# hhcho/sfgwas

Hardware: AMD Instinct MI355X
Metric: pca_power_iter_ring_macs_per_s (higher is better)
Workload: dtype u64 ring words, exact integers: int8 digits on the matrix core for the MAC of all five moduli, fp64-held integers in the encode and key-switch kernels

## Files before the change

include/sfgwas_hip.h:

```cpp
#ifndef SFGWAS_HIP_H
#define SFGWAS_HIP_H
#include <stdint.h>
#include <stddef.h>
#ifdef __cplusplus
extern "C" {
#endif

typedef struct sfg_ctx sfg_ctx;
typedef struct sfg_geno sfg_geno;

int sfg_ctx_create(sfg_ctx **out, int device, int logN, int nq, int np,
                   const uint64_t *moduli, const uint64_t *psi, double scale);
typedef struct sfg_config {
    uint32_t struct_size;
    int mm_group;
    size_t acc_budget_bytes;
    size_t assoc_rotcache_bytes;
    size_t ksw_budget_bytes;
    int enc_batch;
    int upload_blocking;
    const char *mgpu_transport;
    size_t mgpu_cache_bytes;
    const char *rccl_lib;
} sfg_config;
void sfg_config_default(sfg_config *c);
int sfg_ctx_create_ex(sfg_ctx **out, int device, int logN, int nq, int np,
                      const uint64_t *moduli, const uint64_t *psi, double scale, const sfg_config *config );
int sfg_ctx_fork(sfg_ctx *parent, sfg_ctx **out);
void sfg_ctx_destroy(sfg_ctx *ctx);
const char *sfg_last_error(const sfg_ctx *ctx);
int sfg_ctx_synchronize(sfg_ctx *ctx);
int sfg_ctx_release_scratch(sfg_ctx *ctx);
int sfg_ctx_scratch_bytes(const sfg_ctx *ctx, const char *prefix, size_t *bytes);
int sfg_ctx_set_stream(sfg_ctx *ctx, void *hip_stream);
int sfg_ctx_use_own_stream(sfg_ctx *ctx);

int sfg_ctx_load_rotkey(sfg_ctx *ctx, uint64_t galois_el, const uint64_t *key_host, int montgomery_form);
int sfg_ctx_has_rotkey(const sfg_ctx *ctx, uint64_t galois_el);
int sfg_ctx_export_rotkey(sfg_ctx *ctx, uint64_t galois_el, uint64_t *key_host);
uint64_t sfg_galois_for_rotation(const sfg_ctx *ctx, int k_left);

int sfg_malloc(sfg_ctx *ctx, void **dev_ptr, size_t bytes);
int sfg_free(sfg_ctx *ctx, void *dev_ptr);
int sfg_memcpy_h2d(sfg_ctx *ctx, void *dst_dev, const void *src_host, size_t bytes);
int sfg_memcpy_d2h(sfg_ctx *ctx, void *dst_host, const void *src_dev, size_t bytes);
int sfg_memcpy_d2d(sfg_ctx *ctx, void *dst_dev, const void *src_dev, size_t bytes);

int sfg_ntt_rows(sfg_ctx *ctx, uint64_t *rows_dev, int nrows, const int *mod_idx_host);
int sfg_intt_rows(sfg_ctx *ctx, uint64_t *rows_dev, int nrows, const int *mod_idx_host);

int sfg_mac_dev(sfg_ctx *ctx, const uint64_t *rot_dev, const uint64_t *pt_dev, uint64_t *out_dev,
                int K, int R, int Ncols, int L, int accumulate);

int sfg_mac_i8_dev(sfg_ctx *ctx, const uint64_t *rot_dev, const uint64_t *pt_half_dev, uint64_t *out_dev,
                   int K, int R, int Ncols, int L, int accumulate, int pt_form);

int sfg_encode_diags_dev(sfg_ctx *ctx, const int8_t *block_dev, size_t ld, int r, int c, int transposed,
                         int shift0, int nshift, int L, uint64_t *pt_dev);
int sfg_encode_coeffs_host(sfg_ctx *ctx, const double *values_host, int nvec, int64_t *coeffs_host);
int sfg_ctx_encoder_near_ties(sfg_ctx *ctx, unsigned long long *count, int reset);
int sfg_ctx_encoder_resolved(sfg_ctx *ctx, unsigned long long *count);
int sfg_ctx_encoder_unprovable(sfg_ctx *ctx, unsigned long long *count);
int sfg_ctx_encoder_inject_unsafe_for_test(sfg_ctx *ctx, unsigned long long n);
int sfg_encode_vectors_dev(sfg_ctx *ctx, const double *values_host, int nvec, int level, uint64_t *pt_dev);

int sfg_rotate_right_dev(sfg_ctx *ctx, const uint64_t *ct_in_dev, uint64_t *ct_out_dev, int nct, int level,
                         const int *nrot_host);
int sfg_ct_galois_dev(sfg_ctx *ctx, const uint64_t *ct_in_dev, uint64_t *ct_out_dev, int nct, int level, uint64_t galois_el);
int sfg_ct_add_dev(sfg_ctx *ctx, const uint64_t *a_dev, const uint64_t *b_dev, uint64_t *out_dev, int nct, int level);
int sfg_ct_sub_dev(sfg_ctx *ctx, const uint64_t *a_dev, const uint64_t *b_dev, uint64_t *out_dev, int nct, int level);

int sfg_ct_drop_level_dev(sfg_ctx *ctx, const uint64_t *in_dev, uint64_t *out_dev, int nct, int level_in, int level_out);

int sfg_ct_mul_scalar_dev(sfg_ctx *ctx, const uint64_t *ct_dev, const uint64_t *scalars_host, uint64_t *out_dev, int nct, int level);
int sfg_ct_mul_scalar_add_dev(sfg_ctx *ctx, const uint64_t *ct_dev, const uint64_t *scalars_host, uint64_t *acc_dev, int nct, int level);
int sfg_ct_add_scalar_dev(sfg_ctx *ctx, const uint64_t *ct_dev, const uint64_t *scalars_host, uint64_t *out_dev, int nct, int level);
int sfg_ct_add_plain_dev(sfg_ctx *ctx, const uint64_t *ct_dev, const uint64_t *pt_dev, size_t pt_stride, uint64_t *out_dev,
                         int nct, int level);

int sfg_ctx_load_relinkey(sfg_ctx *ctx, const uint64_t *key_host, int montgomery);
int sfg_ct_mulrelin_dev(sfg_ctx *ctx, const uint64_t *a_dev, const uint64_t *b_dev, uint64_t *out_dev, int nct, int level);
int sfg_ct_mul_plain_dev(sfg_ctx *ctx, const uint64_t *ct_dev, const uint64_t *pt_dev, size_t pt_stride, uint64_t *out_dev,
                         int nct, int level);
int sfg_ct_rescale_dev(sfg_ctx *ctx, const uint64_t *in_dev, uint64_t *out_dev, int nct, int level);
int sfg_ct_innersum_dev(sfg_ctx *ctx, const uint64_t *in_dev, int nct, int level, uint64_t *out_dev);

int sfg_geno_upload(sfg_ctx *ctx, const int8_t *geno_host, size_t nrow, size_t ncol, size_t ld, sfg_geno **out);
int sfg_geno_from_device(sfg_ctx *ctx, const int8_t *geno_dev, size_t nrow, size_t ncol, size_t ld, sfg_geno **out);
void sfg_geno_free(sfg_ctx *ctx, sfg_geno *g);
int sfg_geno_create(sfg_ctx *ctx, size_t nrow, size_t ncol, sfg_geno **out);
int sfg_geno_write_rows(sfg_ctx *ctx, sfg_geno *g, size_t row0, size_t nrows, const int8_t *rows_host, size_t ld);
int sfg_geno_compare_rows(sfg_ctx *ctx, const sfg_geno *g, unsigned flags, size_t row0, size_t nrows, const int8_t *rows_host, size_t ld, uint64_t *ndiff);
int sfg_pinned_alloc(sfg_ctx *ctx, void **host_ptr, size_t bytes);
int sfg_pinned_free(sfg_ctx *ctx, void *host_ptr);
int sfg_geno_set_plaintext_cache(sfg_ctx *ctx, const sfg_geno *g, size_t max_bytes);
int sfg_geno_plaintext_cache_stats(sfg_ctx *ctx, const sfg_geno *g, size_t *blocks, size_t *bytes, size_t *hits, size_t *fills);
int sfg_geno_from_bed(sfg_ctx *ctx, const uint8_t *bed_host, size_t bed_bytes, size_t num_sample, size_t num_snp,
                      const uint8_t *row_filter, const uint8_t *col_filter, sfg_geno **out);
int sfg_pgen_dims(sfg_ctx *ctx, const uint8_t *pgen_host, size_t pgen_bytes, size_t *num_sample, size_t *num_variant);
int sfg_geno_from_pgen(sfg_ctx *ctx, const uint8_t *pgen_host, size_t pgen_bytes, size_t v0, size_t v1,
                       const uint8_t *row_filter, const uint8_t *col_filter, sfg_geno **out);
int sfg_pgen_geno_counts(sfg_ctx *ctx, const uint8_t *pgen_host, size_t pgen_bytes, const uint8_t *row_filter, uint32_t *counts_host);
int sfg_geno_pack(sfg_ctx *ctx, const sfg_geno *g, sfg_geno **out);
int sfg_geno_unpack(sfg_ctx *ctx, const sfg_geno *g, sfg_geno **out);
int sfg_geno_dims(const sfg_geno *g, size_t *nrow, size_t *ncol);
int sfg_geno_download(sfg_ctx *ctx, const sfg_geno *g, int8_t *host);
int sfg_geno_transpose(sfg_ctx *ctx, const sfg_geno *g, sfg_geno **out);
int sfg_geno_concat_cols(sfg_ctx *ctx, const sfg_geno *const *parts, int k, sfg_geno **out);
int sfg_geno_colsums(sfg_ctx *ctx, const sfg_geno *g, double *sum_host, double *sqsum_host);

#define SFG_SQUARE 1u
#define SFG_TRANSPOSE 2u
#define SFG_STREAM_DIRECT 4u
int sfg_matmul_resident_dev(sfg_ctx *ctx, const uint64_t *A_dev, int s, int in_level, int max_level,
                            const sfg_geno *g, unsigned flags, uint64_t *out_dev);
int sfg_matmul_from_cache(sfg_ctx *ctx, const uint64_t *A_dev, int s, int in_level, int max_level, const char *cache_prefix, int nbr, uint64_t *out_dev);
int sfg_diagcache_write(sfg_ctx *ctx, const sfg_geno *g, unsigned flags, int max_level, const char *cache_prefix, int *files_written);
int sfg_diagcache_header(sfg_ctx *ctx, const char *cache_prefix, int block_row, uint64_t hdr[6]);
int sfg_matmul_stream(sfg_ctx *ctx, const uint64_t *A_host, int s, int in_level, int max_level,
                      const int8_t *geno_host, size_t nrow, size_t ncol, size_t ld, unsigned flags,
                      uint64_t *out_host, double *sum_host, double *sqsum_host);
int sfg_assoc_stream_bed(sfg_ctx *ctx, const char *bed_path, size_t num_sample, size_t num_snp, const uint8_t *row_filter, const uint8_t *col_filter,
                         size_t batch_snps, const uint64_t *A_dev, int s, int in_level, int max_level, unsigned flags,
                         uint64_t *out_dev, size_t out_ct_capacity, size_t *out_ct, double *sum_host, double *sqsum_host);
int sfg_assoc_pgen(sfg_ctx *ctx, const uint8_t *pgen_host, size_t pgen_bytes, const uint8_t *row_filter, const uint8_t *col_filter, size_t batch_snps,
                   const uint64_t *A_dev, int s, int in_level, int max_level, unsigned flags,
                   uint64_t *out_dev, size_t out_ct_capacity, size_t *out_ct, double *sum_host, double *sqsum_host);
int sfg_assoc_stream_pgen(sfg_ctx *ctx, const char *pgen_path, const uint8_t *row_filter, const uint8_t *col_filter, size_t batch_snps,
                          const uint64_t *A_dev, int s, int in_level, int max_level, unsigned flags,
                          uint64_t *out_dev, size_t out_ct_capacity, size_t *out_ct, double *sum_host, double *sqsum_host);
int sfg_matmul_resident_range_dev(sfg_ctx *ctx, const uint64_t *A_dev, int s, int in_level, int max_level,
                                  const sfg_geno *g, unsigned flags, int blk0, int blk1, uint64_t *out_dev);
int sfg_matmul_accumulate_dev(sfg_ctx *ctx, const uint64_t *A_dev, int s, int in_level, int max_level,
                              const sfg_geno *g, unsigned flags, int b0, int b1, int j0, int j1,
                              int accumulate, uint64_t *acc_dev);
int sfg_matmul_finalize_dev(sfg_ctx *ctx, const uint64_t *acc_dev, int s, int max_level, int ncolb,
                            int g0, int g1, int accumulate, uint64_t *out_dev);
int sfg_matmul_finalize_slots_dev(sfg_ctx *ctx, const uint64_t *acc_dev, int s, int max_level, int ncolb, int acc_giants, int giant_base,
                                  int g0, int g1, int accumulate, uint64_t *out_dev);
int sfg_rotcache_invalidate(sfg_ctx *ctx);
int sfg_rotcache_layout(sfg_ctx *ctx, int s, int max_level, size_t *job_doubles, size_t *tail_doubles);
int sfg_rotcache_build_jobs_dev(sfg_ctx *ctx, const uint64_t *A_dev, int s, int in_level, int max_level, int nbr, int job0, int job1, double *staged_dev);
int sfg_rotcache_scatter_dev(sfg_ctx *ctx, const double *staged_dev, int s, int max_level, int job0, int job1, int row0, int nrows, double *cache_dev);
int sfg_rotcache_build_rows_dev(sfg_ctx *ctx, const uint64_t *A_dev, int s, int in_level, int max_level, int nbr, int b0, int b1, double *cache_dev);
int sfg_matmul_resident_range_rc_dev(sfg_ctx *ctx, const double *cache_dev, int s, int max_level, const sfg_geno *g, unsigned flags,
                                     int blk0, int blk1, uint64_t *out_dev);
int sfg_matmul_accumulate_rc_dev(sfg_ctx *ctx, const double *cache_dev, int s, int max_level, const sfg_geno *g, unsigned flags,
                                 int b0, int b1, int j0, int j1, int accumulate, uint64_t *acc_dev);
int sfg_reduce_rows_dev(sfg_ctx *ctx, uint64_t *rows_dev, size_t nrows_of_L, int L);

typedef struct sfg_mgpu sfg_mgpu;
typedef struct sfg_mgeno sfg_mgeno;
#define SFG_MGPU_ID_BYTES 128
int sfg_mgpu_unique_id(uint8_t *id128);
int sfg_mgpu_create(sfg_mgpu **out, const int *devices, int n, int logN, int nq, int np, const uint64_t *moduli, const uint64_t *psi, double scale);
int sfg_mgpu_create_rank(sfg_mgpu **out, int device, int rank, int world, const uint8_t *id128, int logN, int nq, int np, const uint64_t *moduli,
                         const uint64_t *psi, double scale);
int sfg_mgpu_create_ex(sfg_mgpu **out, const int *devices, int n, int logN, int nq, int np, const uint64_t *moduli, const uint64_t *psi, double scale,
                       const sfg_config *config);
int sfg_mgpu_create_rank_ex(sfg_mgpu **out, int device, int rank, int world, const uint8_t *id128, int logN, int nq, int np, const uint64_t *moduli,
                            const uint64_t *psi, double scale, const sfg_config *config);
void sfg_mgpu_destroy(sfg_mgpu *mg);
const char *sfg_mgpu_last_error(const sfg_mgpu *mg);
int sfg_mgpu_world(const sfg_mgpu *mg);
int sfg_mgpu_nlocal(const sfg_mgpu *mg);
int sfg_mgpu_rank(const sfg_mgpu *mg, int local);
sfg_ctx *sfg_mgpu_ctx(sfg_mgpu *mg, int local);
const char *sfg_mgpu_transport(const sfg_mgpu *mg);
int sfg_mgpu_synchronize(sfg_mgpu *mg);
int sfg_mgpu_comm_info(sfg_mgpu *mg, int local, int *nranks, int *rank);
int sfg_mgpu_preflight(sfg_mgpu *mg, size_t count_per_rank);
int sfg_mgpu_load_rotkey(sfg_mgpu *mg, uint64_t galois_el, const uint64_t *key_host, int montgomery_form);
int sfg_mgpu_load_relinkey(sfg_mgpu *mg, const uint64_t *key_host, int montgomery_form);
int sfg_mgpu_fill_rotkeys_synthetic(sfg_mgpu *mg, const int *rot_left, int nrot, uint64_t seed);
int sfg_mgpu_shard(int world, size_t ncol, int rank, size_t *blk0, size_t *blk1, size_t *col0, size_t *col1);
int sfg_mgpu_geno_upload(sfg_mgpu *mg, const int8_t *geno_host, size_t nrow, size_t ncol, size_t ld, sfg_mgeno **out);
int sfg_mgpu_geno_adopt(sfg_mgpu *mg, size_t nrow, size_t ncol, sfg_geno *const *shards, sfg_mgeno **out);
int sfg_mgpu_geno_synthetic(sfg_mgpu *mg, size_t nrow, size_t ncol, uint64_t seed, int packed, sfg_mgeno **out);
void sfg_mgpu_geno_free(sfg_mgpu *mg, sfg_mgeno *g);
const sfg_geno *sfg_mgpu_geno_shard(const sfg_mgeno *g, int local);
int sfg_mgpu_geno_dims(const sfg_mgeno *g, size_t *nrow, size_t *ncol);
int sfg_mgpu_geno_blocks(const sfg_mgeno *g, int local, size_t *blk0, size_t *blk1);
int sfg_mgpu_geno_set_plaintext_cache(sfg_mgpu *mg, const sfg_mgeno *g, size_t max_bytes_per_rank);
int sfg_mgpu_geno_create(sfg_mgpu *mg, size_t nrow, size_t ncol, sfg_mgeno **out);
int sfg_mgpu_geno_write_rows(sfg_mgpu *mg, sfg_mgeno *g, size_t row0, size_t nrows, const int8_t *rows_host, size_t ld);
int sfg_mgpu_geno_compare_rows(sfg_mgpu *mg, const sfg_mgeno *g, unsigned flags, size_t row0, size_t nrows, const int8_t *rows_host, size_t ld, uint64_t *ndiff);
int sfg_mgpu_matmul_dev(sfg_mgpu *mg, const uint64_t *const *A_dev, int s, int in_level, int max_level, const sfg_mgeno *g, unsigned flags,
                        uint64_t *const *out_dev);
int sfg_mgpu_matmul(sfg_mgpu *mg, const uint64_t *A_host, int s, int in_level, int max_level, const sfg_mgeno *g, unsigned flags, uint64_t *out_host);
int sfg_mgpu_inject_failure_for_test(sfg_mgpu *mg, int local, int phase);
int sfg_mgpu_assoc_stream_bed(sfg_mgpu *mg, const char *bed_path, size_t num_sample, size_t num_snp, const uint8_t *row_filter, const uint8_t *col_filter,
                              size_t batch_snps, const uint64_t *A_host, int s, int in_level, int max_level, unsigned flags,
                              uint64_t *out_host, size_t out_ct_capacity, size_t *out_ct, double *sum_host, double *sqsum_host);
int sfg_mgpu_assoc_stream_pgen(sfg_mgpu *mg, const char *pgen_path, const uint8_t *row_filter, const uint8_t *col_filter, size_t kept_samples,
                               size_t batch_snps, const uint64_t *A_host, int s, int in_level, int max_level, unsigned flags,
                               uint64_t *out_host, size_t out_ct_capacity, size_t *out_ct, double *sum_host, double *sqsum_host);

int sfg_ctx_load_secret_key(sfg_ctx *ctx, const uint64_t *sk_host, int montgomery_form);
int sfg_refresh_gen_shares_dev(sfg_ctx *ctx, const uint64_t *ct_dev, int nct, int level, const uint64_t *crs_dev, const uint64_t *mask_dev, int mask_limbs,
                               const int32_t *e0_dev, const int32_t *e1_dev, uint64_t *h0_dev, uint64_t *h1_dev);
int sfg_refresh_finish_dev(sfg_ctx *ctx, const uint64_t *ct_dev, int nct, int level, const uint64_t *h0agg_dev, const uint64_t *h1agg_dev,
                           const uint64_t *crs_dev, uint64_t *out_dev);

int sfg_refresh_gen_shares_scaled_dev(sfg_ctx *ctx, const uint64_t *ct_dev, int nct, int level, double ct_scale, double target_scale, const uint64_t *crs_dev,
                                      const uint64_t *mask_dev, int mask_limbs, const int32_t *e0_dev, const int32_t *e1_dev, uint64_t *h0_dev, uint64_t *h1_dev);
int sfg_refresh_finish_scaled_dev(sfg_ctx *ctx, const uint64_t *ct_dev, int nct, int level, double ct_scale, double target_scale, const uint64_t *h0agg_dev,
                                  const uint64_t *h1agg_dev, const uint64_t *crs_dev, uint64_t *out_dev);

int sfg_ckks_to_ss_share_dev(sfg_ctx *ctx, const uint64_t *ct_dev, int nct, int level, const uint64_t *mask_dev, int mask_limbs, const int32_t *e0_dev,
                             uint64_t *h0_dev, uint64_t *mask_ntt_dev);

int sfg_ss_mask_dev(sfg_ctx *ctx, int limbs, const uint64_t *modulus_host, const uint64_t *bound_host, const uint64_t *rm_dev, const uint64_t *rand_dev,
                    uint64_t *rm_masked_dev, uint64_t *mask_dev, size_t n);
int sfg_ss_hub_share_dev(sfg_ctx *ctx, int limbs, const uint64_t *modulus_host, const uint64_t *revealed_dev, const uint64_t *mask_dev, uint64_t *share_dev, size_t n);

int sfg_ctx_load_public_key(sfg_ctx *ctx, const uint64_t *pk_host, int montgomery_form);
int sfg_ctx_has_public_key(const sfg_ctx *ctx);
int sfg_encrypt_explicit_dev(sfg_ctx *ctx, const uint64_t *pt_dev, int nct, int level, const int8_t *u_dev, const int32_t *e0_dev, const int32_t *e1_dev,
                             uint64_t *out_dev);
int sfg_ctx_seed_encryptor(sfg_ctx *ctx, const uint8_t *key32);
int sfg_ctx_encryptor_next_index(const sfg_ctx *ctx, uint64_t *next_index);
int sfg_ct_add_fresh_zero_dev(sfg_ctx *ctx, uint64_t *ct_dev, int nct, int level);
int sfg_encrypt_vectors_dev(sfg_ctx *ctx, const double *values_host, int nct, int level, uint64_t *out_dev);
int sfg_encrypt_transcript_for_test(sfg_ctx *ctx, uint64_t first_index, int nct, int8_t *u_dev, int32_t *e0_dev, int32_t *e1_dev);

int sfg_pcks_gen_share_dev(sfg_ctx *ctx, const uint64_t *ct_dev, int nct, int level, const int32_t *e0_dev, const int32_t *e1_dev, uint64_t *h0_dev, uint64_t *h1_dev);
int sfg_pcks_finish_dev(sfg_ctx *ctx, const uint64_t *ct_dev, int nct, int level, const uint64_t *h0agg_dev, uint64_t *pt_dev);
int sfg_decode_vectors(sfg_ctx *ctx, const uint64_t *pt_dev, size_t pt_stride, int nct, int level, double scale, double *re_host, double *im_host);
int sfg_decode_vectors_dev(sfg_ctx *ctx, const uint64_t *pt_dev, size_t pt_stride, int nct, int level, double scale, double *re_dev, double *im_dev);
int sfg_decode_coeffs(sfg_ctx *ctx, const uint64_t *pt_dev, size_t pt_stride, int nct, int level, double scale, double *coeffs_host);
int sfg_pcks_finish_decode(sfg_ctx *ctx, const uint64_t *ct_dev, int nct, int level, double scale, const uint64_t *h0agg_dev, double *re_host, double *im_host);
int sfg_decrypt_vectors(sfg_ctx *ctx, const uint64_t *ct_dev, int nct, int level, double scale, double *re_host, double *im_host);

int sfg_beaver_elem_dev(sfg_ctx *ctx, int pid, int limbs, const uint64_t *modulus_host,
                        const uint64_t *ar_dev, const uint64_t *am_dev, const uint64_t *br_dev, const uint64_t *bm_dev,
                        uint64_t *out_dev, size_t n);
int sfg_beaver_elem(sfg_ctx *ctx, int pid, int limbs, const uint64_t *modulus_host,
                    const uint64_t *ar_host, const uint64_t *am_host, const uint64_t *br_host, const uint64_t *bm_host,
                    uint64_t *out_host, size_t n);
int sfg_beaver_matmul(sfg_ctx *ctx, int pid, int limbs, const uint64_t *modulus_host,
                      const uint64_t *ar_host, const uint64_t *am_host, const uint64_t *br_host, const uint64_t *bm_host,
                      uint64_t *out_host, int m, int k, int n);

int sfg_sketch(sfg_ctx *ctx, const sfg_geno *g, const int32_t *bucket_host, const int8_t *sgn_host, int kp,
               double *sketch_host, uint64_t *xsum_host, uint64_t *x2sum_host);

int sfg_fill_uniform_ct_dev(sfg_ctx *ctx, uint64_t *ct_dev, int nct, int level, uint64_t seed);
int sfg_fill_geno_dev(sfg_ctx *ctx, int8_t *geno_dev, size_t nrow, size_t ncol, uint64_t seed);
int sfg_fill_geno_window_dev(sfg_ctx *ctx, int8_t *geno_dev, size_t nrow, size_t ncol, size_t ld, size_t col0, size_t ncol_global, uint64_t seed);
int sfg_fill_rotkeys_synthetic(sfg_ctx *ctx, const int *rot_left, int nrot, uint64_t seed);

int sfg_ctx_clear_phases(sfg_ctx *ctx);
double sfg_last_phase_ms(const sfg_ctx *ctx, const char *phase);
int sfg_last_phase_launches(const sfg_ctx *ctx, const char *phase);
double sfg_last_phase_bytes(const sfg_ctx *ctx, const char *phase);

#ifdef __cplusplus
}
#endif
#endif
```

sfgwas_amd/capi.py:

```python
import ctypes as C
import os
import numpy as np

_HERE = os.path.dirname(os.path.abspath(__file__))
LIB_PATH = os.environ.get("SFG_LIB_PATH") or os.path.join(_HERE, "lib", "libsfgwas_hip.so")
AB_LIB_PATH = os.path.join(_HERE, "lib_ab", "libsfgwas_hip.so")
DEPLOYMENT_SWITCHES = {"SFG_MM_GROUP", "SFG_MM_ACC_BUDGET_MB", "SFG_ASSOC_ROTCACHE_MB", "SFG_KSW_BUDGET_MB", "SFG_ENC_BATCH", "SFG_UPLOAD_BLOCKING",
                       "SFG_MGPU_TRANSPORT", "SFG_MGPU_CACHE_GB", "SFG_RCCL_LIB", "SFG_ENABLE_TEST_HOOKS",
                       "SFG_TEST_SCRATCH_OOM", "SFG_TEST_TIE_BAND_LOG2", "SFG_MGPU_FORCE_COLLECTIVES"}


def ab_lib():
    import subprocess
    subprocess.check_call(["make", "-C", os.path.join(_HERE, "csrc"), "ab", "-j8"], stdout=subprocess.DEVNULL)
    return AB_LIB_PATH


def env_for(switches):
    e = {k: str(v) for k, v in switches.items()}
    if any(k.startswith("SFG_") and k not in DEPLOYMENT_SWITCHES for k in e):
        e["SFG_LIB_PATH"] = ab_lib()
    return e


class SfgConfig(C.Structure):
    _fields_ = [("struct_size", C.c_uint32), ("mm_group", C.c_int), ("acc_budget_bytes", C.c_size_t), ("assoc_rotcache_bytes", C.c_size_t),
                ("ksw_budget_bytes", C.c_size_t), ("enc_batch", C.c_int), ("upload_blocking", C.c_int), ("mgpu_transport", C.c_char_p),
                ("mgpu_cache_bytes", C.c_size_t), ("rccl_lib", C.c_char_p)]

    def __init__(self, **kw):
        super().__init__()
        self.struct_size = C.sizeof(SfgConfig)
        for k, v in kw.items():
            setattr(self, k, v)

u64p = C.POINTER(C.c_uint64)
_lib = None

SFG_SQUARE = 1
SFG_TRANSPOSE = 2
SFG_STREAM_DIRECT = 4


class SfgError(RuntimeError):
    pass


def _sig(L):
    vp, i, u64, d, sz = C.c_void_p, C.c_int, C.c_uint64, C.c_double, C.c_size_t
    S = {
        "sfg_ctx_create": (i, [C.POINTER(vp), i, i, i, i, u64p, u64p, d]),
        "sfg_ctx_create_ex": (i, [C.POINTER(vp), i, i, i, i, u64p, u64p, d, vp]),
        "sfg_config_default": (None, [vp]),
        "sfg_mgpu_create_ex": (i, [C.POINTER(vp), C.POINTER(i), i, i, i, i, u64p, u64p, d, vp]),
        "sfg_mgpu_create_rank_ex": (i, [C.POINTER(vp), i, i, i, vp, i, i, i, u64p, u64p, d, vp]),
        "sfg_ctx_fork": (i, [vp, C.POINTER(vp)]),
        "sfg_ctx_destroy": (None, [vp]),
        "sfg_last_error": (C.c_char_p, [vp]),
        "sfg_ctx_synchronize": (i, [vp]),
        "sfg_ctx_set_stream": (i, [vp, vp]),
        "sfg_ctx_release_scratch": (i, [vp]),
        "sfg_ctx_scratch_bytes": (i, [vp, C.c_char_p, C.POINTER(C.c_size_t)]),
        "sfg_rotcache_invalidate": (i, [vp]),
        "sfg_ctx_use_own_stream": (i, [vp]),
        "sfg_ctx_encoder_inject_unsafe_for_test": (i, [vp, C.c_ulonglong]),
        "sfg_ctx_encoder_resolved": (i, [vp, C.POINTER(C.c_ulonglong)]),
        "sfg_ctx_encoder_unprovable": (i, [vp, C.POINTER(C.c_ulonglong)]),
        "sfg_ctx_load_rotkey": (i, [vp, u64, u64p, i]),
        "sfg_ctx_load_secret_key": (i, [vp, u64p, i]),
        "sfg_ctx_load_public_key": (i, [vp, u64p, i]),
        "sfg_ctx_has_public_key": (i, [vp]),
        "sfg_ctx_seed_encryptor": (i, [vp, C.c_char_p]),
        "sfg_ctx_encryptor_next_index": (i, [vp, C.POINTER(u64)]),
        "sfg_encrypt_explicit_dev": (i, [vp, vp, i, i, vp, vp, vp, vp]),
        "sfg_ct_add_fresh_zero_dev": (i, [vp, vp, i, i]),
        "sfg_encrypt_vectors_dev": (i, [vp, C.POINTER(d), i, i, vp]),
        "sfg_encrypt_transcript_for_test": (i, [vp, u64, i, vp, vp, vp]),
        "sfg_pcks_gen_share_dev": (i, [vp, vp, i, i, vp, vp, vp, vp]),
        "sfg_pcks_finish_dev": (i, [vp, vp, i, i, vp, vp]),
        "sfg_decode_vectors": (i, [vp, vp, sz, i, i, d, vp, vp]),
        "sfg_decode_vectors_dev": (i, [vp, vp, sz, i, i, d, vp, vp]),
        "sfg_decode_coeffs": (i, [vp, vp, sz, i, i, d, vp]),
        "sfg_pcks_finish_decode": (i, [vp, vp, i, i, d, vp, vp, vp]),
        "sfg_decrypt_vectors": (i, [vp, vp, i, i, d, vp, vp]),
        "sfg_ct_galois_dev": (i, [vp, vp, vp, i, i, u64]),
        "sfg_ct_mul_scalar_add_dev": (i, [vp, vp, u64p, vp, i, i]),
        "sfg_refresh_gen_shares_dev": (i, [vp, vp, i, i, vp, vp, i, vp, vp, vp, vp]),
        "sfg_refresh_finish_dev": (i, [vp, vp, i, i, vp, vp, vp, vp]),
        "sfg_refresh_gen_shares_scaled_dev": (i, [vp, vp, i, i, d, d, vp, vp, i, vp, vp, vp, vp]),
        "sfg_refresh_finish_scaled_dev": (i, [vp, vp, i, i, d, d, vp, vp, vp, vp]),
        "sfg_ckks_to_ss_share_dev": (i, [vp, vp, i, i, vp, i, vp, vp, vp]),
        "sfg_geno_pack": (i, [vp, vp, C.POINTER(vp)]),
        "sfg_geno_unpack": (i, [vp, vp, C.POINTER(vp)]),
        "sfg_assoc_stream_bed": (i, [vp, C.c_char_p, sz, sz, vp, vp, sz, vp, i, i, i, C.c_uint, vp, sz, C.POINTER(sz), vp, vp]),
        "sfg_assoc_stream_pgen": (i, [vp, C.c_char_p, vp, vp, sz, vp, i, i, i, C.c_uint, vp, sz, C.POINTER(sz), vp, vp]),
        "sfg_assoc_pgen": (i, [vp, vp, sz, vp, vp, sz, vp, i, i, i, C.c_uint, vp, sz, C.POINTER(sz), vp, vp]),
        "sfg_ctx_has_rotkey": (i, [vp, u64]),
        "sfg_ctx_export_rotkey": (i, [vp, u64, u64p]),
        "sfg_galois_for_rotation": (u64, [vp, i]),
        "sfg_malloc": (i, [vp, C.POINTER(vp), sz]),
        "sfg_free": (i, [vp, vp]),
        "sfg_memcpy_h2d": (i, [vp, vp, vp, sz]),
        "sfg_memcpy_d2h": (i, [vp, vp, vp, sz]),
        "sfg_memcpy_d2d": (i, [vp, vp, vp, sz]),
        "sfg_ct_drop_level_dev": (i, [vp, vp, vp, i, i, i]),
        "sfg_ntt_rows": (i, [vp, vp, i, C.POINTER(i)]),
        "sfg_intt_rows": (i, [vp, vp, i, C.POINTER(i)]),
        "sfg_mac_dev": (i, [vp, vp, vp, vp, i, i, i, i, i]),
        "sfg_mac_i8_dev": (i, [vp, vp, vp, vp, i, i, i, i, i, i]),
        "sfg_encode_diags_dev": (i, [vp, vp, sz, i, i, i, i, i, i, vp]),
        "sfg_encode_coeffs_host": (i, [vp, C.POINTER(d), i, C.POINTER(C.c_int64)]),
        "sfg_encode_vectors_dev": (i, [vp, C.POINTER(d), i, i, vp]),
        "sfg_ctx_encoder_near_ties": (i, [vp, C.POINTER(C.c_ulonglong), i]),
        "sfg_rotate_right_dev": (i, [vp, vp, vp, i, i, C.POINTER(i)]),
        "sfg_ct_add_dev": (i, [vp, vp, vp, vp, i, i]),
        "sfg_ct_sub_dev": (i, [vp, vp, vp, vp, i, i]),
        "sfg_ct_mul_scalar_dev": (i, [vp, vp, u64p, vp, i, i]),
        "sfg_ct_add_scalar_dev": (i, [vp, vp, u64p, vp, i, i]),
        "sfg_ct_add_plain_dev": (i, [vp, vp, vp, sz, vp, i, i]),
        "sfg_ctx_load_relinkey": (i, [vp, u64p, i]),
        "sfg_ct_mulrelin_dev": (i, [vp, vp, vp, vp, i, i]),
        "sfg_ct_mul_plain_dev": (i, [vp, vp, vp, sz, vp, i, i]),
        "sfg_ct_rescale_dev": (i, [vp, vp, vp, i, i]),
        "sfg_ct_innersum_dev": (i, [vp, vp, i, i, vp]),
        "sfg_geno_upload": (i, [vp, vp, sz, sz, sz, C.POINTER(vp)]),
        "sfg_geno_from_device": (i, [vp, vp, sz, sz, sz, C.POINTER(vp)]),
        "sfg_geno_free": (None, [vp, vp]),
        "sfg_geno_create": (i, [vp, sz, sz, C.POINTER(vp)]),
        "sfg_geno_write_rows": (i, [vp, vp, sz, sz, vp, sz]),
        "sfg_geno_compare_rows": (i, [vp, vp, C.c_uint, sz, sz, vp, sz, u64p]),
        "sfg_pinned_alloc": (i, [vp, C.POINTER(vp), sz]),
        "sfg_pinned_free": (i, [vp, vp]),
        "sfg_geno_set_plaintext_cache": (i, [vp, vp, C.c_size_t]),
        "sfg_geno_plaintext_cache_stats": (i, [vp, vp, C.POINTER(C.c_size_t), C.POINTER(C.c_size_t), C.POINTER(C.c_size_t), C.POINTER(C.c_size_t)]),
        "sfg_geno_from_bed": (i, [vp, vp, sz, sz, sz, vp, vp, C.POINTER(vp)]),
        "sfg_geno_dims": (i, [vp, C.POINTER(sz), C.POINTER(sz)]),
        "sfg_pgen_dims": (i, [vp, vp, sz, C.POINTER(sz), C.POINTER(sz)]),
        "sfg_geno_from_pgen": (i, [vp, vp, sz, sz, sz, vp, vp, C.POINTER(vp)]),
        "sfg_pgen_geno_counts": (i, [vp, vp, sz, vp, vp]),
        "sfg_geno_download": (i, [vp, vp, vp]),
        "sfg_geno_transpose": (i, [vp, vp, C.POINTER(vp)]),
        "sfg_geno_concat_cols": (i, [vp, C.POINTER(vp), i, C.POINTER(vp)]),
        "sfg_geno_colsums": (i, [vp, vp, C.POINTER(d), C.POINTER(d)]),
        "sfg_matmul_resident_dev": (i, [vp, vp, i, i, i, vp, C.c_uint, vp]),
        "sfg_matmul_from_cache": (i, [vp, vp, i, i, i, C.c_char_p, i, vp]),
        "sfg_diagcache_header": (i, [vp, C.c_char_p, i, u64p]),
        "sfg_diagcache_write": (i, [vp, vp, C.c_uint, i, C.c_char_p, C.POINTER(C.c_int)]),
        "sfg_matmul_stream": (i, [vp, u64p, i, i, i, vp, sz, sz, sz, C.c_uint, u64p, C.POINTER(d), C.POINTER(d)]),
        "sfg_matmul_resident_range_dev": (i, [vp, vp, i, i, i, vp, C.c_uint, i, i, vp]),
        "sfg_matmul_accumulate_dev": (i, [vp, vp, i, i, i, vp, C.c_uint, i, i, i, i, i, vp]),
        "sfg_matmul_finalize_dev": (i, [vp, vp, i, i, i, i, i, i, vp]),
        "sfg_matmul_finalize_slots_dev": (i, [vp, vp, i, i, i, i, i, i, i, i, vp]),
        "sfg_reduce_rows_dev": (i, [vp, vp, sz, i]),
        "sfg_rotcache_layout": (i, [vp, i, i, C.POINTER(sz), C.POINTER(sz)]),
        "sfg_rotcache_build_jobs_dev": (i, [vp, vp, i, i, i, i, i, i, vp]),
        "sfg_rotcache_scatter_dev": (i, [vp, vp, i, i, i, i, i, i, vp]),
        "sfg_rotcache_build_rows_dev": (i, [vp, vp, i, i, i, i, i, i, vp]),
        "sfg_matmul_resident_range_rc_dev": (i, [vp, vp, i, i, vp, C.c_uint, i, i, vp]),
        "sfg_matmul_accumulate_rc_dev": (i, [vp, vp, i, i, vp, C.c_uint, i, i, i, i, i, vp]),
        "sfg_beaver_elem_dev": (i, [vp, i, i, u64p, vp, vp, vp, vp, vp, sz]),
        "sfg_ss_mask_dev": (i, [vp, i, u64p, u64p, vp, vp, vp, vp, sz]),
        "sfg_ss_hub_share_dev": (i, [vp, i, u64p, vp, vp, vp, sz]),
        "sfg_beaver_elem": (i, [vp, i, i, u64p, u64p, u64p, u64p, u64p, u64p, sz]),
        "sfg_beaver_matmul": (i, [vp, i, i, u64p, u64p, u64p, u64p, u64p, u64p, i, i, i]),
        "sfg_sketch": (i, [vp, vp, C.POINTER(C.c_int32), C.POINTER(C.c_int8), i, C.POINTER(d), u64p, u64p]),
        "sfg_fill_uniform_ct_dev": (i, [vp, vp, i, i, u64]),
        "sfg_fill_geno_dev": (i, [vp, vp, sz, sz, u64]),
        "sfg_fill_geno_window_dev": (i, [vp, vp, sz, sz, sz, sz, sz, u64]),
        "sfg_fill_rotkeys_synthetic": (i, [vp, C.POINTER(i), i, u64]),
        "sfg_mgpu_unique_id": (i, [vp]),
        "sfg_mgpu_create": (i, [C.POINTER(vp), C.POINTER(i), i, i, i, i, u64p, u64p, d]),
        "sfg_mgpu_create_rank": (i, [C.POINTER(vp), i, i, i, vp, i, i, i, u64p, u64p, d]),
        "sfg_mgpu_destroy": (None, [vp]),
        "sfg_mgpu_last_error": (C.c_char_p, [vp]),
        "sfg_mgpu_world": (i, [vp]),
        "sfg_mgpu_nlocal": (i, [vp]),
        "sfg_mgpu_rank": (i, [vp, i]),
        "sfg_mgpu_ctx": (vp, [vp, i]),
        "sfg_mgpu_transport": (C.c_char_p, [vp]),
        "sfg_mgpu_synchronize": (i, [vp]),
        "sfg_mgpu_load_rotkey": (i, [vp, u64, u64p, i]),
        "sfg_mgpu_load_relinkey": (i, [vp, u64p, i]),
        "sfg_mgpu_fill_rotkeys_synthetic": (i, [vp, C.POINTER(i), i, u64]),
        "sfg_mgpu_shard": (i, [i, sz, i, C.POINTER(sz), C.POINTER(sz), C.POINTER(sz), C.POINTER(sz)]),
        "sfg_mgpu_geno_upload": (i, [vp, vp, sz, sz, sz, C.POINTER(vp)]),
        "sfg_mgpu_geno_adopt": (i, [vp, sz, sz, C.POINTER(vp), C.POINTER(vp)]),
        "sfg_mgpu_geno_create": (i, [vp, sz, sz, C.POINTER(vp)]),
        "sfg_mgpu_geno_write_rows": (i, [vp, vp, sz, sz, vp, sz]),
        "sfg_mgpu_geno_compare_rows": (i, [vp, vp, C.c_uint, sz, sz, vp, sz, u64p]),
        "sfg_mgpu_comm_info": (i, [vp, i, C.POINTER(i), C.POINTER(i)]),
        "sfg_mgpu_preflight": (i, [vp, sz]),
        "sfg_mgpu_geno_synthetic": (i, [vp, sz, sz, u64, i, C.POINTER(vp)]),
        "sfg_mgpu_geno_free": (None, [vp, vp]),
        "sfg_mgpu_geno_shard": (vp, [vp, i]),
        "sfg_mgpu_geno_dims": (i, [vp, C.POINTER(sz), C.POINTER(sz)]),
        "sfg_mgpu_geno_blocks": (i, [vp, i, C.POINTER(sz), C.POINTER(sz)]),
        "sfg_mgpu_geno_set_plaintext_cache": (i, [vp, vp, sz]),
        "sfg_mgpu_matmul_dev": (i, [vp, C.POINTER(vp), i, i, i, vp, C.c_uint, C.POINTER(vp)]),
        "sfg_mgpu_matmul": (i, [vp, u64p, i, i, i, vp, C.c_uint, u64p]),
        "sfg_mgpu_inject_failure_for_test": (i, [vp, i, i]),
        "sfg_mgpu_assoc_stream_bed": (i, [vp, C.c_char_p, sz, sz, vp, vp, sz, u64p, i, i, i, C.c_uint, u64p, sz, C.POINTER(sz), vp, vp]),
        "sfg_mgpu_assoc_stream_pgen": (i, [vp, C.c_char_p, vp, vp, sz, sz, u64p, i, i, i, C.c_uint, u64p, sz, C.POINTER(sz), vp, vp]),
        "sfg_ctx_clear_phases": (i, [vp]),
        "sfg_last_phase_ms": (d, [vp, C.c_char_p]),
        "sfg_last_phase_launches": (i, [vp, C.c_char_p]),
        "sfg_last_phase_bytes": (d, [vp, C.c_char_p]),
    }
    for name, (res, args) in S.items():
        fn = getattr(L, name)
        fn.restype, fn.argtypes = res, args
    return list(S.keys())


EXPORTS = []


def lib():
    global _lib, EXPORTS
    if _lib is None:
        if not os.path.exists(LIB_PATH):
            raise SfgError(f"{LIB_PATH} is missing: run `python -c 'import __graft_entry__ as g; g.build()'` "
                           "(there is no CPU fallback for the HIP path)")
        _lib = C.CDLL(LIB_PATH)
        EXPORTS = _sig(_lib)
    return _lib


def p64(a):
    assert a.dtype == np.uint64 and a.flags.c_contiguous
    return a.ctypes.data_as(u64p)


class Context:

    def __init__(self, q, p, scale=2.0 ** 34, logN=14, device=0, psi=None, config=None):
        L = lib()
        self.q, self.p = list(q), list(p)
        self.nq, self.np_ = len(q), len(p)
        self.N, self.slots = 1 << logN, (1 << logN) // 2
        mods = np.array(self.q + self.p, dtype=np.uint64)
        h = C.c_void_p()
        ps = None if psi is None else p64(np.array(psi, dtype=np.uint64))
        if config is None:
            rc = L.sfg_ctx_create(C.byref(h), device, logN, self.nq, self.np_, p64(mods), ps, float(scale))
        else:
            rc = L.sfg_ctx_create_ex(C.byref(h), device, logN, self.nq, self.np_, p64(mods), ps, float(scale), C.byref(config))
        if rc:
            raise SfgError("sfg_ctx_create: " + L.sfg_last_error(None).decode())
        self.h = h
        self.beta = (self.nq + self.np_ - 1) // self.np_

    def close(self):
        if getattr(self, "h", None):
            lib().sfg_ctx_destroy(self.h)
            self.h = None

    def __del__(self):
        try:
            self.close()
        except Exception:
            pass

    def check(self, rc, what):
        if rc:
            raise SfgError(f"{what}: {lib().sfg_last_error(self.h).decode()}")

    def malloc(self, nbytes):
        p = C.c_void_p()
        self.check(lib().sfg_malloc(self.h, C.byref(p), nbytes), "sfg_malloc")
        return p

    def free(self, p):
        self.check(lib().sfg_free(self.h, p), "sfg_free")

    def to_device(self, arr):
        arr = np.ascontiguousarray(arr)
        p = self.malloc(arr.nbytes)
        self.check(lib().sfg_memcpy_h2d(self.h, p, arr.ctypes.data_as(C.c_void_p), arr.nbytes), "h2d")
        return p

    def to_host(self, p, shape, dtype):
        out = np.empty(shape, dtype=dtype)
        self.check(lib().sfg_memcpy_d2h(self.h, out.ctypes.data_as(C.c_void_p), p, out.nbytes), "d2h")
        return out

    def sync(self):
        self.check(lib().sfg_ctx_synchronize(self.h), "sync")

    def ntt_rows(self, rows, mod_idx, inverse=False):
        rows = np.ascontiguousarray(rows, dtype=np.uint64)
        n = rows.shape[0]
        mi = (C.c_int * n)(*[int(x) for x in mod_idx])
        d = self.to_device(rows)
        fn = lib().sfg_intt_rows if inverse else lib().sfg_ntt_rows
        self.check(fn(self.h, d, n, mi), "ntt_rows")
        out = self.to_host(d, rows.shape, np.uint64)
        self.free(d)
        return out

    def load_rotkey(self, galois, key, montgomery=False):
        key = np.ascontiguousarray(key, dtype=np.uint64)
        self.check(lib().sfg_ctx_load_rotkey(self.h, int(galois), p64(key), int(montgomery)), "load_rotkey")

    def export_rotkey(self, galois):
        key = np.zeros((self.beta, 2, self.nq + self.np_, self.N), dtype=np.uint64)
        self.check(lib().sfg_ctx_export_rotkey(self.h, int(galois), p64(key)), "export_rotkey")
        return key

    def load_secret_key(self, sk_rows, montgomery=False):
        sk_rows = np.ascontiguousarray(sk_rows, dtype=np.uint64)
        assert sk_rows.shape == (self.nq, self.N)
        self.check(lib().sfg_ctx_load_secret_key(self.h, p64(sk_rows), int(montgomery)), "load_secret_key")

    def refresh_gen_shares(self, cts, level, crs, mask_limbs, e0, e1, scales=None):
        nct, W = cts.shape[0], mask_limbs.shape[-1]
        d = [self.to_device(np.ascontiguousarray(a)) for a in (cts, crs, mask_limbs, e0.astype(np.int32), e1.astype(np.int32))]
        h0, h1 = self.malloc(nct * (level + 1) * self.N * 8), self.malloc(nct * self.nq * self.N * 8)
        if scales is None:
            self.check(lib().sfg_refresh_gen_shares_dev(self.h, d[0], nct, level, d[1], d[2], W, d[3], d[4], h0, h1), "refresh_gen_shares")
        else:
            self.check(lib().sfg_refresh_gen_shares_scaled_dev(self.h, d[0], nct, level, float(scales[0]), float(scales[1]), d[1], d[2], W, d[3], d[4], h0, h1),
                       "refresh_gen_shares_scaled")
        out = self.to_host(h0, (nct, level + 1, self.N), np.uint64), self.to_host(h1, (nct, self.nq, self.N), np.uint64)
        for p_ in d + [h0, h1]:
            self.free(p_)
        return out

    def ckks_to_ss_share(self, cts, level, mask_limbs, e0):
        nct, W = cts.shape[0], mask_limbs.shape[-1]
        d = [self.to_device(np.ascontiguousarray(a)) for a in (cts, mask_limbs, e0.astype(np.int32))]
        h0, mk = self.malloc(nct * (level + 1) * self.N * 8), self.malloc(nct * (level + 1) * self.N * 8)
        self.check(lib().sfg_ckks_to_ss_share_dev(self.h, d[0], nct, level, d[1], W, d[2], h0, mk), "ckks_to_ss_share")
        out = self.to_host(h0, (nct, level + 1, self.N), np.uint64), self.to_host(mk, (nct, level + 1, self.N), np.uint64)
        for p_ in d + [h0, mk]:
            self.free(p_)
        return out

    def refresh_finish(self, cts, level, h0agg, h1agg, crs, scales=None):
        nct = cts.shape[0]
        d = [self.to_device(np.ascontiguousarray(a)) for a in (cts, h0agg, h1agg, crs)]
        o = self.malloc(nct * 2 * self.nq * self.N * 8)
        if scales is None:
            self.check(lib().sfg_refresh_finish_dev(self.h, d[0], nct, level, d[1], d[2], d[3], o), "refresh_finish")
        else:
            self.check(lib().sfg_refresh_finish_scaled_dev(self.h, d[0], nct, level, float(scales[0]), float(scales[1]), d[1], d[2], d[3], o), "refresh_finish_scaled")
        out = self.to_host(o, (nct, 2, self.nq, self.N), np.uint64)
        for p_ in d + [o]:
            self.free(p_)
        return out

    def fork(self):
        h = C.c_void_p()
        self.check(lib().sfg_ctx_fork(self.h, C.byref(h)), "sfg_ctx_fork")
        child = Context.__new__(Context)
        child.__dict__.update({k: v for k, v in self.__dict__.items()})
        child.h = h
        return child

    def encoder_near_ties(self, reset=False):
        n = C.c_ulonglong()
        self.check(lib().sfg_ctx_encoder_near_ties(self.h, C.byref(n), int(reset)), "encoder_near_ties")
        return n.value

    def galois(self, k):
        return lib().sfg_galois_for_rotation(self.h, k)

    def phase_ms(self, name):
        return lib().sfg_last_phase_ms(self.h, name.encode())


def _ctx_mac(self, rot, pt, L, out_init=None):
    rot = np.ascontiguousarray(rot, dtype=np.uint64)
    pt = np.ascontiguousarray(pt, dtype=np.uint64)
    K, R = rot.shape[0], rot.shape[1]
    Ncols = pt.shape[1]
    assert rot.shape[2] == L and pt.shape[2] == L and pt.shape[0] == K
    d_rot, d_pt = self.to_device(rot), self.to_device(pt)
    if out_init is not None:
        d_out = self.to_device(np.ascontiguousarray(out_init, dtype=np.uint64))
    else:
        d_out = self.malloc(Ncols * R * L * self.N * 8)
    self.check(lib().sfg_mac_dev(self.h, d_rot, d_pt, d_out, K, R, Ncols, L, int(out_init is not None)), "sfg_mac_dev")
    out = self.to_host(d_out, (Ncols, R, L, self.N), np.uint64)
    for p in (d_rot, d_pt, d_out):
        self.free(p)
    return out


Context.mac = _ctx_mac


def _ctx_mac_i8(self, rot, pt_half, L, K=None, out_init=None, pt_form=0):
    rot = np.ascontiguousarray(rot, dtype=np.uint64)
    pt_half = np.ascontiguousarray(pt_half, dtype=np.uint64)
    P, R = rot.shape[0], rot.shape[1]
    Ncols = pt_half.shape[1]
    K = P if K is None else K
    assert rot.shape[2] == L and pt_half.shape[2] == L and pt_half.shape[0] == P and pt_half.shape[3] == self.N // 2 and K >= P
    bufs = []
    for arr in (rot, pt_half):
        sl = arr.nbytes // P
        d = self.malloc(sl * K)
        self.check(lib().sfg_memcpy_h2d(self.h, d, arr.ctypes.data_as(C.c_void_p), arr.nbytes), "h2d")
        filled = P
        while filled < K:
            n = min(filled, K - filled)
            self.check(lib().sfg_memcpy_d2d(self.h, C.c_void_p(d.value + filled * sl), d, n * sl), "d2d")
            filled += n
        bufs.append(d)
    if out_init is not None:
        d_out = self.to_device(np.ascontiguousarray(out_init, dtype=np.uint64))
    else:
        d_out = self.malloc(Ncols * R * L * self.N * 8)
    try:
        self.check(lib().sfg_mac_i8_dev(self.h, bufs[0], bufs[1], d_out, K, R, Ncols, L, int(out_init is not None), pt_form), "sfg_mac_i8_dev")
        out = self.to_host(d_out, (Ncols, R, L, self.N), np.uint64)
    finally:
        for p_ in bufs + [d_out]:
            self.free(p_)
    return out


Context.mac_i8 = _ctx_mac_i8


def _ctx_encode_diags(self, block, shift0, nshift, L, transposed=False):
    block = np.ascontiguousarray(block, dtype=np.int8)
    r, c = block.shape
    if transposed:
        r, c = c, r
    d_blk = self.to_device(block)
    d_pt = self.malloc(nshift * L * self.N * 8)
    self.check(lib().sfg_encode_diags_dev(self.h, d_blk, block.shape[1], r, c, int(transposed), shift0, nshift, L, d_pt), "sfg_encode_diags_dev")
    out = self.to_host(d_pt, (nshift, L, self.N), np.uint64)
    self.free(d_blk)
    self.free(d_pt)
    return out


Context.encode_diags = _ctx_encode_diags


def _ctx_rotate_right(self, cts, level, nrots):
    cts = np.ascontiguousarray(cts, dtype=np.uint64)
    nct = cts.shape[0]
    d_in = self.to_device(cts)
    d_out = self.malloc(cts.nbytes)
    arr = (C.c_int * nct)(*[int(x) for x in nrots])
    self.check(lib().sfg_rotate_right_dev(self.h, d_in, d_out, nct, level, arr), "sfg_rotate_right_dev")
    out = self.to_host(d_out, cts.shape, np.uint64)
    self.free(d_in)
    self.free(d_out)
    return out


Context.rotate_right = _ctx_rotate_right


def _ctx_matmul_stream(self, A, in_level, max_level, geno, flags=0, want_sums=False):
    A = np.ascontiguousarray(A, dtype=np.uint64)
    geno = np.ascontiguousarray(geno, dtype=np.int8)
    s = A.shape[0]
    nrow, ncol = geno.shape
    lrow, lcol = (ncol, nrow) if flags & SFG_TRANSPOSE else (nrow, ncol)
    nbr, m_ct = (lrow - 1) // self.slots + 1, (lcol - 1) // self.slots + 1
    assert A.shape[1] == nbr, (A.shape, nbr)
    out = np.zeros((s, m_ct, 2, max_level, self.N), dtype=np.uint64)
    sm = np.zeros(ncol) if want_sums else None
    sq = np.zeros(ncol) if want_sums else None
    dp = C.POINTER(C.c_double)
    self.check(lib().sfg_matmul_stream(self.h, p64(A), s, in_level, max_level, geno.ctypes.data_as(C.c_void_p), nrow, ncol, ncol, flags,
                                       p64(out), sm.ctypes.data_as(dp) if want_sums else None, sq.ctypes.data_as(dp) if want_sums else None),
               "sfg_matmul_stream")
    return out, sm, sq


Context.matmul_stream = _ctx_matmul_stream


def random_rotkey(ctx_or_ring_moduli, beta, N, seed):
    rnd = np.random.default_rng(seed)
    mods = ctx_or_ring_moduli
    k = np.zeros((beta, 2, len(mods), N), dtype=np.uint64)
    for m, q in enumerate(mods):
        k[:, :, m, :] = rnd.integers(0, q, (beta, 2, N), dtype=np.uint64)
    return k


def _ctx_evalop(self, name, level, *arrays, out_level=None, extra=()):
    devs = [self.to_device(np.ascontiguousarray(a, dtype=np.uint64)) for a in arrays]
    nct = arrays[0].shape[0]
    ol_ = level if out_level is None else out_level
    out = self.malloc(nct * 2 * (ol_ + 1) * self.N * 8)
    fn = getattr(lib(), name)
    if name in ("sfg_ct_mul_plain_dev", "sfg_ct_add_plain_dev"):
        self.check(fn(self.h, devs[0], devs[1], extra[0], out, nct, level), name)
    elif name in ("sfg_ct_mul_scalar_dev", "sfg_ct_add_scalar_dev"):
        self.check(fn(self.h, devs[0], p64(np.ascontiguousarray(extra[0], dtype=np.uint64)), out, nct, level), name)
    elif name == "sfg_ct_rescale_dev":
        self.check(fn(self.h, devs[0], out, nct, level), name)
    else:
        self.check(fn(self.h, devs[0], devs[1], out, nct, level), name)
    res = self.to_host(out, (nct, 2, ol_ + 1, self.N), np.uint64)
    for d_ in devs + [out]:
        self.free(d_)
    return res


def _ctx_innersum(self, cts, level):
    cts = np.ascontiguousarray(cts, dtype=np.uint64)
    d_in = self.to_device(cts)
    out = self.malloc(2 * (level + 1) * self.N * 8)
    self.check(lib().sfg_ct_innersum_dev(self.h, d_in, cts.shape[0], level, out), "innersum")
    res = self.to_host(out, (2, level + 1, self.N), np.uint64)
    self.free(d_in); self.free(out)
    return res


def _ctx_load_relinkey(self, key, montgomery=False):
    key = np.ascontiguousarray(key, dtype=np.uint64)
    self.check(lib().sfg_ctx_load_relinkey(self.h, p64(key), int(montgomery)), "load_relinkey")


Context.evalop = _ctx_evalop
Context.innersum = _ctx_innersum
Context.load_relinkey = _ctx_load_relinkey


def _ctx_geno_to_host(self, g):
    nr, nc = C.c_size_t(), C.c_size_t()
    lib().sfg_geno_dims(g, C.byref(nr), C.byref(nc))
    out = np.empty((nr.value, nc.value), dtype=np.int8)
    self.check(lib().sfg_geno_download(self.h, g, out.ctypes.data_as(C.c_void_p)), "geno_download")
    return out


def _ctx_geno_from_bed(self, bed, num_sample, num_snp, row_filter=None, col_filter=None):
    bed = np.ascontiguousarray(bed, dtype=np.uint8)
    rf = None if row_filter is None else np.ascontiguousarray(row_filter, dtype=np.uint8)
    cf = None if col_filter is None else np.ascontiguousarray(col_filter, dtype=np.uint8)
    g = C.c_void_p()
    self.check(lib().sfg_geno_from_bed(self.h, bed.ctypes.data_as(C.c_void_p), bed.size, num_sample, num_snp,
                                       None if rf is None else rf.ctypes.data_as(C.c_void_p),
                                       None if cf is None else cf.ctypes.data_as(C.c_void_p), C.byref(g)), "geno_from_bed")
    return g


def _ctx_geno_from_pgen(self, img, v0=0, v1=0, row_filter=None, col_filter=None):
    img = np.ascontiguousarray(img, dtype=np.uint8)
    rf = None if row_filter is None else np.ascontiguousarray(row_filter, dtype=np.uint8)
    cf = None if col_filter is None else np.ascontiguousarray(col_filter, dtype=np.uint8)
    g = C.c_void_p()
    self.check(lib().sfg_geno_from_pgen(self.h, img.ctypes.data_as(C.c_void_p), img.size, v0, v1,
                                        None if rf is None else rf.ctypes.data_as(C.c_void_p),
                                        None if cf is None else cf.ctypes.data_as(C.c_void_p), C.byref(g)), "geno_from_pgen")
    return g


def _ctx_pgen_geno_counts(self, img, row_filter=None):
    img = np.ascontiguousarray(img, dtype=np.uint8)
    ns, nv = C.c_size_t(), C.c_size_t()
    self.check(lib().sfg_pgen_dims(self.h, img.ctypes.data_as(C.c_void_p), img.size, C.byref(ns), C.byref(nv)), "pgen_dims")
    rf = None if row_filter is None else np.ascontiguousarray(row_filter, dtype=np.uint8)
    out = np.empty((6, nv.value), dtype=np.uint32)
    self.check(lib().sfg_pgen_geno_counts(self.h, img.ctypes.data_as(C.c_void_p), img.size, None if rf is None else rf.ctypes.data_as(C.c_void_p),
                                          out.ctypes.data_as(C.c_void_p)), "pgen_geno_counts")
    return out


Context.geno_to_host = _ctx_geno_to_host
Context.geno_from_bed = _ctx_geno_from_bed
Context.geno_from_pgen = _ctx_geno_from_pgen
Context.pgen_geno_counts = _ctx_pgen_geno_counts


def _ctx_encode_vectors(self, values, level):
    values = np.ascontiguousarray(values, dtype=np.float64)
    nvec = values.shape[0]
    out = self.malloc(nvec * (level + 1) * self.N * 8)
    self.check(lib().sfg_encode_vectors_dev(self.h, values.ctypes.data_as(C.POINTER(C.c_double)), nvec, level, out), "encode_vectors")
    res = self.to_host(out, (nvec, level + 1, self.N), np.uint64)
    self.free(out)
    return res


Context.encode_vectors = _ctx_encode_vectors


def _ctx_load_public_key(self, pk_rows, montgomery=False):
    pk_rows = np.ascontiguousarray(pk_rows, dtype=np.uint64)
    assert pk_rows.shape == (2, self.nq + self.np_, self.N)
    self.check(lib().sfg_ctx_load_public_key(self.h, p64(pk_rows), int(montgomery)), "load_public_key")


def _ctx_has_public_key(self):
    return bool(lib().sfg_ctx_has_public_key(self.h))


def _ctx_seed_encryptor(self, key32):
    key32 = bytes(key32)
    if len(key32) != 32:
        raise ValueError("the encryptor key is 32 bytes")
    self.check(lib().sfg_ctx_seed_encryptor(self.h, key32), "seed_encryptor")


def _ctx_encryptor_next_index(self):
    n = C.c_uint64()
    self.check(lib().sfg_ctx_encryptor_next_index(self.h, C.byref(n)), "encryptor_next_index")
    return n.value


def _ctx_encrypt_explicit(self, pt, level, u, e0, e1):
    u, e0, e1 = (np.ascontiguousarray(u, dtype=np.int8), np.ascontiguousarray(e0, dtype=np.int32), np.ascontiguousarray(e1, dtype=np.int32))
    nct = u.shape[0]
    assert u.shape == e0.shape == e1.shape == (nct, self.N)
    d = [DevArray.from_host(self, a) for a in (u, e0, e1)]
    dpt = None
    if pt is not None:
        pt = np.ascontiguousarray(pt, dtype=np.uint64)
        assert pt.shape == (nct, level + 1, self.N)
        dpt = DevArray.from_host(self, pt)
    out = DevArray(self, (nct, 2, level + 1, self.N))
    try:
        self.check(lib().sfg_encrypt_explicit_dev(self.h, None if dpt is None else dpt.p, nct, level, d[0].p, d[1].p, d[2].p, out.p), "encrypt_explicit")
        return out.host()
    finally:
        for a in d + [out] + ([dpt] if dpt is not None else []):
            a.free()


def _ctx_add_fresh_zero(self, ct_dev, level):
    nct = int(np.prod(ct_dev.shape[:-3])) if len(ct_dev.shape) > 3 else 1
    assert ct_dev.shape[-3:] == (2, level + 1, self.N)
    self.check(lib().sfg_ct_add_fresh_zero_dev(self.h, ct_dev.p, nct, level), "add_fresh_zero")
    return ct_dev


def _ctx_encrypt_vectors(self, values, level):
    values = np.ascontiguousarray(values, dtype=np.float64)
    nct = values.shape[0]
    out = DevArray(self, (max(nct, 1), 2, level + 1, self.N))
    rc = lib().sfg_encrypt_vectors_dev(self.h, values.ctypes.data_as(C.POINTER(C.c_double)), nct, level, out.p)
    if rc:
        out.free()
    self.check(rc, "encrypt_vectors")
    return out


def _ctx_encrypt_transcript(self, first_index, nct):
    d = [DevArray(self, (max(nct, 1), self.N), t) for t in (np.int8, np.int32, np.int32)]
    try:
        self.check(lib().sfg_encrypt_transcript_for_test(self.h, int(first_index), nct, d[0].p, d[1].p, d[2].p), "encrypt_transcript")
        return tuple(a.host() for a in d)
    finally:
        for a in d:
            a.free()


Context.load_public_key = _ctx_load_public_key
Context.has_public_key = _ctx_has_public_key
Context.seed_encryptor = _ctx_seed_encryptor
Context.encryptor_next_index = _ctx_encryptor_next_index
Context.encrypt_explicit = _ctx_encrypt_explicit
Context.add_fresh_zero = _ctx_add_fresh_zero
Context.encrypt_vectors = _ctx_encrypt_vectors
Context.encrypt_transcript = _ctx_encrypt_transcript


def _dev_ptr(self, a, dtype, shape=None):
    if isinstance(a, DevArray):
        return a.p, None
    a = np.ascontiguousarray(a, dtype=dtype)
    assert shape is None or a.shape == shape, (a.shape, shape)
    d = DevArray.from_host(self, a)
    return d.p, d


def _ctx_pcks_gen_share(self, cts, level, e0, e1=None):
    nct = int(cts.shape[0])
    keep = []
    try:
        pc, t = _dev_ptr(self, cts, np.uint64, (nct, 2, level + 1, self.N)); keep.append(t)
        p0, t = _dev_ptr(self, e0, np.int32, (nct, self.N)); keep.append(t)
        p1 = None
        if e1 is not None:
            p1, t = _dev_ptr(self, e1, np.int32, (nct, self.N)); keep.append(t)
        h0 = DevArray(self, (nct, level + 1, self.N)); keep.append(h0)
        h1 = None
        if e1 is not None:
            h1 = DevArray(self, (nct, level + 1, self.N)); keep.append(h1)
        self.check(lib().sfg_pcks_gen_share_dev(self.h, pc, nct, level, p0, p1, h0.p, None if h1 is None else h1.p), "pcks_gen_share")
        return h0.host(), (None if h1 is None else h1.host())
    finally:
        for a in keep:
            if a is not None:
                a.free()


def _ctx_pcks_finish(self, cts, level, h0agg, scale=None, want_imag=False):
    nct = int(cts.shape[0])
    keep = []
    try:
        pc, t = _dev_ptr(self, cts, np.uint64, (nct, 2, level + 1, self.N)); keep.append(t)
        ph, t = _dev_ptr(self, h0agg, np.uint64, (nct, level + 1, self.N)); keep.append(t)
        if scale is None:
            pt = DevArray(self, (nct, level + 1, self.N)); keep.append(pt)
            self.check(lib().sfg_pcks_finish_dev(self.h, pc, nct, level, ph, pt.p), "pcks_finish")
            return pt.host()
        re = np.empty((nct, self.slots)); im = np.empty((nct, self.slots)) if want_imag else None
        self.check(lib().sfg_pcks_finish_decode(self.h, pc, nct, level, float(scale), ph, re.ctypes.data_as(C.c_void_p),
                                                None if im is None else im.ctypes.data_as(C.c_void_p)), "pcks_finish_decode")
        return (re, im) if want_imag else re
    finally:
        for a in keep:
            if a is not None:
                a.free()


def _ctx_decode_vectors(self, pt, level, scale, want_imag=False, stride=None):
    nct = int(pt.shape[0])
    p, t = _dev_ptr(self, pt, np.uint64)
    try:
        re = np.empty((nct, self.slots)); im = np.empty((nct, self.slots)) if want_imag else None
        self.check(lib().sfg_decode_vectors(self.h, p, (level + 1) * self.N if stride is None else int(stride), nct, level, float(scale),
                                            re.ctypes.data_as(C.c_void_p), None if im is None else im.ctypes.data_as(C.c_void_p)), "decode_vectors")
        return (re, im) if want_imag else re
    finally:
        if t is not None:
            t.free()


def _ctx_decode_coeffs(self, pt, level, scale, stride=None):
    nct = int(pt.shape[0])
    p, t = _dev_ptr(self, pt, np.uint64)
    try:
        out = np.empty((nct, self.N))
        self.check(lib().sfg_decode_coeffs(self.h, p, (level + 1) * self.N if stride is None else int(stride), nct, level, float(scale),
                                           out.ctypes.data_as(C.c_void_p)), "decode_coeffs")
        return out
    finally:
        if t is not None:
            t.free()


def _ctx_decrypt_vectors(self, cts, level, scale, want_imag=False):
    nct = int(np.prod(cts.shape[:-3]))
    p, t = _dev_ptr(self, cts, np.uint64)
    try:
        re = np.empty((nct, self.slots)); im = np.empty((nct, self.slots)) if want_imag else None
        self.check(lib().sfg_decrypt_vectors(self.h, p, nct, level, float(scale), re.ctypes.data_as(C.c_void_p),
                                             None if im is None else im.ctypes.data_as(C.c_void_p)), "decrypt_vectors")
        return (re, im) if want_imag else re
    finally:
        if t is not None:
            t.free()


Context.pcks_gen_share = _ctx_pcks_gen_share
Context.pcks_finish = _ctx_pcks_finish
Context.decode_vectors = _ctx_decode_vectors
Context.decode_coeffs = _ctx_decode_coeffs
Context.decrypt_vectors = _ctx_decrypt_vectors


class DevArray:

    def __init__(self, ctx, shape, dtype=np.uint64):
        self.ctx, self.shape, self.dtype = ctx, tuple(int(x) for x in shape), np.dtype(dtype)
        self.nbytes = int(np.prod(self.shape)) * self.dtype.itemsize
        self.p = ctx.malloc(max(self.nbytes, 8))

    @classmethod
    def from_host(cls, ctx, arr):
        arr = np.ascontiguousarray(arr)
        d = cls(ctx, arr.shape, arr.dtype)
        ctx.check(lib().sfg_memcpy_h2d(ctx.h, d.p, arr.ctypes.data_as(C.c_void_p), arr.nbytes), "h2d")
        return d

    def host(self):
        return self.ctx.to_host(self.p, self.shape, self.dtype)

    def host_slice(self, index):
        index = index if isinstance(index, tuple) else (index,)
        sub = self.shape[len(index):]
        off = 0
        for k, i in enumerate(index):
            off += int(i) * int(np.prod(self.shape[k + 1:]))
        out = np.empty(sub, dtype=self.dtype)
        src = C.c_void_p(self.p.value + off * self.dtype.itemsize)
        self.ctx.check(lib().sfg_memcpy_d2h(self.ctx.h, out.ctypes.data_as(C.c_void_p), src, out.nbytes), "d2h")
        return out

    def free(self):
        if self.p is not None:
            self.ctx.free(self.p)
            self.p = None


def _ctx_geno_upload(self, geno):
    geno = np.ascontiguousarray(geno, dtype=np.int8)
    g = C.c_void_p()
    self.check(lib().sfg_geno_upload(self.h, geno.ctypes.data_as(C.c_void_p), geno.shape[0], geno.shape[1], geno.shape[1], C.byref(g)), "geno_upload")
    return g


def _ctx_geno_free(self, g):
    lib().sfg_geno_free(self.h, g)


def _ctx_geno_create(self, nrow, ncol):
    g = C.c_void_p()
    self.check(lib().sfg_geno_create(self.h, nrow, ncol, C.byref(g)), "geno_create")
    return g


def _ctx_geno_write_rows(self, g, row0, rows, ld=None):
    rows = np.ascontiguousarray(rows, dtype=np.int8)
    self.check(lib().sfg_geno_write_rows(self.h, g, row0, rows.shape[0], rows.ctypes.data_as(C.c_void_p), ld or rows.shape[1]), "geno_write_rows")


def _ctx_geno_compare_rows(self, g, flags, row0, rows):
    rows = np.ascontiguousarray(rows, dtype=np.int8)
    nd = np.zeros(1, dtype=np.uint64)
    self.check(lib().sfg_geno_compare_rows(self.h, g, flags, row0, rows.shape[0], rows.ctypes.data_as(C.c_void_p), rows.shape[1], p64(nd)), "geno_compare_rows")
    return int(nd[0])


def _ctx_fill_uniform_cts(self, nct, level, seed):
    d = DevArray(self, (nct, 2, level + 1, self.N))
    self.check(lib().sfg_fill_uniform_ct_dev(self.h, d.p, nct, level, seed), "fill_uniform_ct")
    return d


def _ctx_fill_geno(self, nrow, ncol, seed):
    d = DevArray(self, (nrow, ncol), np.int8)
    self.check(lib().sfg_fill_geno_dev(self.h, d.p, nrow, ncol, seed), "fill_geno")
    g = C.c_void_p()
    self.check(lib().sfg_geno_from_device(self.h, d.p, nrow, ncol, ncol, C.byref(g)), "geno_from_device")
    return d, g


def _ctx_matmul_resident(self, A_dev, s, in_level, max_level, g, flags=0, blk=None):
    nr, nc = C.c_size_t(), C.c_size_t()
    lib().sfg_geno_dims(g, C.byref(nr), C.byref(nc))
    lcol = nr.value if flags & SFG_TRANSPOSE else nc.value
    m_ct = (lcol - 1) // self.slots + 1
    if blk is None:
        out = DevArray(self, (s, m_ct, 2, max_level, self.N))
        self.check(lib().sfg_matmul_resident_dev(self.h, A_dev.p, s, in_level, max_level, g, flags, out.p), "matmul_resident")
    else:
        m_out = m_ct if flags & SFG_TRANSPOSE else blk[1] - blk[0]
        out = DevArray(self, (s, m_out, 2, max_level, self.N))
        self.check(lib().sfg_matmul_resident_range_dev(self.h, A_dev.p, s, in_level, max_level, g, flags, blk[0], blk[1], out.p), "matmul_resident_range")
    return out


def _ctx_matmul_accumulate(self, A_dev, s, in_level, max_level, g, flags, b0, b1, j0, j1, acc=None):
    d = 91
    accumulate = acc is not None
    if acc is None:
        acc = DevArray(self, (j1 - j0, d, s, 2, max_level, self.N))
    self.check(lib().sfg_matmul_accumulate_dev(self.h, A_dev.p, s, in_level, max_level, g, flags, b0, b1, j0, j1, int(accumulate), acc.p), "matmul_accumulate")
    return acc


def _ctx_matmul_finalize(self, acc, s, max_level, ncolb, g0, g1, out=None):
    accumulate = out is not None
    if out is None:
        out = DevArray(self, (s, ncolb, 2, max_level, self.N))
    self.check(lib().sfg_matmul_finalize_dev(self.h, acc.p, s, max_level, ncolb, g0, g1, int(accumulate), out.p), "matmul_finalize")
    return out


Context.geno_upload = _ctx_geno_upload
Context.geno_free = _ctx_geno_free
Context.geno_create = _ctx_geno_create
Context.geno_write_rows = _ctx_geno_write_rows
Context.geno_compare_rows = _ctx_geno_compare_rows
Context.fill_uniform_cts = _ctx_fill_uniform_cts
Context.fill_geno = _ctx_fill_geno
Context.matmul_resident = _ctx_matmul_resident
Context.matmul_accumulate = _ctx_matmul_accumulate
Context.matmul_finalize = _ctx_matmul_finalize


class MultiGpu:

    def __init__(self, q, p, devices=None, scale=2.0 ** 34, logN=14, rank=None, world=None, uid=None, device=0, config=None):
        L = lib()
        self.q, self.p = list(q), list(p)
        self.nq, self.np_ = len(q), len(p)
        self.N, self.slots = 1 << logN, (1 << logN) // 2
        mods = np.array(self.q + self.p, dtype=np.uint64)
        h = C.c_void_p()
        cfgp = None if config is None else C.byref(config)
        if uid is None:
            devs = (C.c_int * len(devices))(*devices)
            rc = L.sfg_mgpu_create_ex(C.byref(h), devs, len(devices), logN, self.nq, self.np_, p64(mods), None, float(scale), cfgp)
        else:
            buf = (C.c_uint8 * 128).from_buffer_copy(bytes(uid))
            rc = L.sfg_mgpu_create_rank_ex(C.byref(h), device, rank, world, buf, logN, self.nq, self.np_, p64(mods), None, float(scale), cfgp)
        if rc:
            raise SfgError("sfg_mgpu_create: " + L.sfg_mgpu_last_error(None).decode())
        self.h = h
        self.world, self.nlocal = L.sfg_mgpu_world(h), L.sfg_mgpu_nlocal(h)
        self.transport = L.sfg_mgpu_transport(h).decode()
        self.ctx = []
        for i in range(self.nlocal):
            c = Context.__new__(Context)
            c.__dict__.update(q=self.q, p=self.p, nq=self.nq, np_=self.np_, N=self.N, slots=self.slots, beta=(self.nq + self.np_ - 1) // self.np_)
            c.h = C.c_void_p(L.sfg_mgpu_ctx(h, i))
            c.close = lambda: None
            self.ctx.append(c)
        self.ranks = [L.sfg_mgpu_rank(h, i) for i in range(self.nlocal)]

    @staticmethod
    def unique_id():
        buf = (C.c_uint8 * 128)()
        if lib().sfg_mgpu_unique_id(buf):
            raise SfgError("sfg_mgpu_unique_id: " + lib().sfg_mgpu_last_error(None).decode())
        return bytes(buf)

    def check(self, rc, what):
        if rc:
            raise SfgError(f"{what}: {lib().sfg_mgpu_last_error(self.h).decode()}")

    def close(self):
        if getattr(self, "h", None):
            for c in self.ctx:
                c.h = None
            lib().sfg_mgpu_destroy(self.h)
            self.h = None

    def sync(self):
        self.check(lib().sfg_mgpu_synchronize(self.h), "sfg_mgpu_synchronize")

    def fill_rotkeys_synthetic(self, rots_left, seed):
        arr = (C.c_int * len(rots_left))(*rots_left)
        self.check(lib().sfg_mgpu_fill_rotkeys_synthetic(self.h, arr, len(rots_left), seed), "sfg_mgpu_fill_rotkeys_synthetic")

    def load_rotkey(self, galois, key, montgomery=False):
        key = np.ascontiguousarray(key, dtype=np.uint64)
        self.check(lib().sfg_mgpu_load_rotkey(self.h, int(galois), p64(key), int(montgomery)), "sfg_mgpu_load_rotkey")

    def geno_upload(self, geno):
        geno = np.ascontiguousarray(geno, dtype=np.int8)
        g = C.c_void_p()
        self.check(lib().sfg_mgpu_geno_upload(self.h, geno.ctypes.data_as(C.c_void_p), geno.shape[0], geno.shape[1], geno.shape[1], C.byref(g)), "sfg_mgpu_geno_upload")
        return g

    def geno_create(self, nrow, ncol):
        g = C.c_void_p()
        self.check(lib().sfg_mgpu_geno_create(self.h, nrow, ncol, C.byref(g)), "sfg_mgpu_geno_create")
        return g

    def geno_write_rows(self, g, row0, rows):
        rows = np.ascontiguousarray(rows, dtype=np.int8)
        self.check(lib().sfg_mgpu_geno_write_rows(self.h, g, row0, rows.shape[0], rows.ctypes.data_as(C.c_void_p), rows.shape[1]), "sfg_mgpu_geno_write_rows")

    def geno_compare_rows(self, g, flags, row0, rows):
        rows = np.ascontiguousarray(rows, dtype=np.int8)
        nd = np.zeros(1, dtype=np.uint64)
        self.check(lib().sfg_mgpu_geno_compare_rows(self.h, g, flags, row0, rows.shape[0], rows.ctypes.data_as(C.c_void_p), rows.shape[1], p64(nd)), "sfg_mgpu_geno_compare_rows")
        return int(nd[0])

    def preflight(self, count_per_rank=4096):
        self.check(lib().sfg_mgpu_preflight(self.h, count_per_rank), "sfg_mgpu_preflight")

    def comm_info(self, local=0):
        n, r = C.c_int(), C.c_int()
        self.check(lib().sfg_mgpu_comm_info(self.h, local, C.byref(n), C.byref(r)), "sfg_mgpu_comm_info")
        return n.value, r.value

    def geno_synthetic(self, nrow, ncol, seed, packed=False):
        g = C.c_void_p()
        self.check(lib().sfg_mgpu_geno_synthetic(self.h, nrow, ncol, seed, int(packed), C.byref(g)), "sfg_mgpu_geno_synthetic")
        return g

    def geno_free(self, g):
        lib().sfg_mgpu_geno_free(self.h, g)

    def geno_blocks(self, g, local):
        b0, b1 = C.c_size_t(), C.c_size_t()
        lib().sfg_mgpu_geno_blocks(g, local, C.byref(b0), C.byref(b1))
        return b0.value, b1.value

    def matmul_dev(self, A, s, in_level, max_level, g, flags, out):
        n = self.nlocal
        pa = (C.c_void_p * n)(*[a.p for a in A])
        po = (C.c_void_p * n)(*[o.p for o in out])
        self.check(lib().sfg_mgpu_matmul_dev(self.h, pa, s, in_level, max_level, g, flags, po), "sfg_mgpu_matmul_dev")

    def inject_failure_for_test(self, local, phase):
        self.check(lib().sfg_mgpu_inject_failure_for_test(self.h, local, phase), "sfg_mgpu_inject_failure_for_test")

    def matmul(self, A_host, s, in_level, max_level, g, flags=0):
        A_host = np.ascontiguousarray(A_host, dtype=np.uint64)
        nr, nc = C.c_size_t(), C.c_size_t()
        lib().sfg_mgpu_geno_dims(g, C.byref(nr), C.byref(nc))
        ncols = ((nr.value if flags & SFG_TRANSPOSE else nc.value) - 1) // self.slots + 1
        out = np.zeros((s, ncols, 2, max_level, self.N), dtype=np.uint64)
        self.check(lib().sfg_mgpu_matmul(self.h, p64(A_host), s, in_level, max_level, g, flags, p64(out)), "sfg_mgpu_matmul")
        return out
```

sfgwas_amd/csrc/common.hpp:

```cpp
#pragma once
#include <hip/hip_runtime.h>
#include <cstdint>
#include <cstdio>
#include <cstring>
#include <string>
#include <vector>
#include <map>
#include <set>
#include "../../include/sfgwas_hip.h"

typedef unsigned long long u64;
typedef unsigned __int128 u128;

constexpr int SFG_LOGN = 14;
constexpr int SFG_N = 1 << SFG_LOGN;
constexpr int SFG_SLOTS = SFG_N / 2;
constexpr int SFG_D = 91;
constexpr int SFG_MAXMOD = 16;
constexpr unsigned long long SFG_I8_BIG_QMAX = 0x7F7F7F7F7F80ULL;

struct ModConst {
    double q, qinv;
    double ninv, ninv_q;
    u64 qi;
};

struct RotKey {
    u64 *key_dev = nullptr;
    uint16_t *index_dev = nullptr;
};

struct PhaseStat { double ms = 0; int launches = 0; double bytes = 0; };
struct PendingEvent { hipEvent_t e0, e1; std::string name; int launches; double bytes; };

struct sfg_geno {
    const int8_t *dev = nullptr;
    size_t nrow = 0, ncol = 0, ld = 0;
    bool owned = false;
    bool packed = false;
    struct PtcEntry { double *slot; bool transposed; };
    mutable std::map<uint64_t, PtcEntry> ptc;
    mutable size_t ptc_budget = 0, ptc_used = 0;
    mutable double *ptc_arena = nullptr;
    mutable uint32_t *ptc_perm = nullptr;
    mutable const void *ptc_owner = nullptr;
    mutable size_t ptc_hits = 0, ptc_fills = 0;
};

struct SfgConfig {
    int mm_group = 8;
    bool mm_group_auto = true;
    size_t acc_budget = 24ULL << 30;
    size_t assoc_cache_budget = 160ULL << 30;
    size_t ksw_budget = 4ULL << 30;
    int enc_batch = 2048;
    bool upload_blocking = false;
    bool test_hooks = false;
    std::string test_scratch_oom;
    double tie_band = 0x1p-50;
    bool mac_i8_big = true;
    bool mac_reg = false;
    bool mac_bc = true;
    bool mac_i8 = true;
    bool mac_i8_nolds = true;
    bool mac_i8_ring = true;
    int mac_i8_waves = 12;
    bool mac_i8_wg1 = false;
    int mac_wc = 1;
    bool no_overlap = true;
    bool ntt_fwd_full = false;
    bool ntt_half_full = false;
    bool pt_compact = true;
    bool pt_kmajor = true;
    int pt_ride = 192;
    int i8_mover_depth_ride = 1, i8_mover_nt_ride = 1;
    bool mac_plain_pt = false;
    bool assoc_trace = false;
};
constexpr size_t SFG_I8_KEEP_RESERVE = 80ULL << 30;

struct SfgShared {
    int device = 0;
    int logN = SFG_LOGN, N = SFG_N, nq = 0, np = 0, nmod = 0, beta = 0;
    double scale = 0;
    u64 q[SFG_MAXMOD] = {0}, psi[SFG_MAXMOD] = {0};
    double *tw_fwd = nullptr;
    double *tw_inv = nullptr;
    double2 *pack_fwd = nullptr;
    double2 *pack_inv = nullptr;
    ModConst *modc = nullptr;
    ModConst modc_host[SFG_MAXMOD];
    void *enc_tables = nullptr;
    void *zeros_dev = nullptr;
    u64 *sk_dev = nullptr;
    u64 *pk_dev = nullptr;
    uint32_t enc_key[8] = {0, 0, 0, 0, 0, 0, 0, 0}; uint32_t *enc_key_dev = nullptr; bool enc_seeded = false;
    u64 enc_next = 0;
    std::map<u64, RotKey> rotkeys;
    SfgConfig cfg;
    int refs = 1;
};

struct sfg_ctx {
    SfgShared *sh = nullptr;
    bool is_fork = false;
    int device = 0;
    int logN = SFG_LOGN, N = SFG_N, nq = 0, np = 0, nmod = 0, beta = 0;
    double scale = 0;
    u64 q[SFG_MAXMOD] = {0}, psi[SFG_MAXMOD] = {0};
    double *tw_fwd = nullptr, *tw_inv = nullptr;
    double2 *pack_fwd = nullptr, *pack_inv = nullptr;
    ModConst *modc = nullptr;
    ModConst modc_host[SFG_MAXMOD];
    SfgConfig cfg;
    unsigned ntt_plain_seq = 0;
    struct I8Slot { const void *src = nullptr; u64 sig[8] = {0, 0, 0, 0, 0, 0, 0, 0}; u64 last_use = 0; };
    static constexpr int I8_SLOTS = 16;
    u64 i8_gen = 1, i8_clock = 0; I8Slot i8_slot[2][I8_SLOTS];
    hipStream_t own_stream = nullptr, stream = nullptr;
    hipStream_t user_stream = nullptr;
    hipStream_t aux_stream = nullptr;
    unsigned char *pin = nullptr; size_t pin_bytes = 0, pin_head = 0;
    hipStream_t coll_stream = nullptr;
    hipEvent_t ev_pipe[4] = {nullptr, nullptr, nullptr, nullptr};
    std::vector<hipEvent_t> ev_pool; size_t ev_next = 0;
    std::map<int, void *> ksw_cache;
    void *ws = nullptr; size_t ws_bytes = 0;
    std::map<std::string, std::pair<void *, size_t>> pool;
    std::map<std::string, std::pair<void *, size_t>> host_pool;
    std::map<std::string, unsigned long long> pool_epoch;
    unsigned long long api_epoch = 0; int api_depth = 0;
    int scratch_oom_seen = 0;
    std::vector<PendingEvent> pending;
    std::string err;
    std::map<std::string, PhaseStat> phases;
    std::set<const sfg_geno *> ptc_genos;
    bool test_hooks = false;
    void *tie_count_dev = nullptr;
    hipStream_t main_stream() const { return user_stream ? user_stream : own_stream; }
    std::map<u64, RotKey> &rotkeys() { return sh->rotkeys; }
    const std::map<u64, RotKey> &rotkeys() const { return sh->rotkeys; }
    void *enc_tables() const { return sh->enc_tables; }
    void *zeros_dev() const { return sh->zeros_dev; }
};

int sfg_sync_all(sfg_ctx *ctx);
int sfg_encoder_check(sfg_ctx *ctx);
void sfg_ptc_detach_all(sfg_ctx *ctx);
void sfg_ptc_invalidate_all(sfg_ctx *ctx);

int encrypt_set_attrs(sfg_ctx *ctx);
int sfg_rows_from_montgomery(sfg_ctx *ctx, unsigned long long *rows_dev, size_t nrows, int nmod);
void sfg_encrypt_destroy(SfgShared *sh);

extern thread_local std::string g_create_error;

#define SFG_FAIL(ctx, ...) do { char _b[512]; snprintf(_b, sizeof _b, __VA_ARGS__); (ctx)->err = _b; return 1; } while (0)
#ifdef SFG_AB
#include "ab/ab.hpp"
#endif
#define SFG_HIP(ctx, call) do { hipError_t _e = (call); if (_e != hipSuccess) { char _b[512]; \
    snprintf(_b, sizeof _b, "HIP call failed: %s (%s:%d)", hipGetErrorString(_e), __FILE__, __LINE__); (ctx)->err = _b; return 1; } } while (0)
#define SFG_TRY(expr) do { int _rc = (expr); if (_rc) return _rc; } while (0)

int sfg_ws_reserve(sfg_ctx *ctx, size_t bytes);

static inline u64 h_mulmod(u64 a, u64 b, u64 q) { return (u64)(((u128)a * b) % q); }
static inline u64 h_powmod(u64 a, u64 e, u64 q) { u64 r = 1 % q; a %= q; while (e) { if (e & 1) r = h_mulmod(r, a, q); a = h_mulmod(a, a, q); e >>= 1; } return r; }
static inline u64 h_invmod(u64 a, u64 q) { return h_powmod(a, q - 2, q); }
static inline uint32_t h_brev(uint32_t x, int bits) { uint32_t r = 0; for (int i = 0; i < bits; i++) { r = (r << 1) | (x & 1); x >>= 1; } return r; }

int sfg_upload_small(sfg_ctx *ctx, void *dst_dev, const void *src_host, size_t bytes);
struct ApiScope {
    sfg_ctx *c;
    explicit ApiScope(sfg_ctx *c_) : c(c_) { if (c->api_depth++ == 0) c->api_epoch++; }
    ~ApiScope() { c->api_depth--; }
};
struct AuxScope {
    sfg_ctx *c; hipStream_t saved;
    explicit AuxScope(sfg_ctx *c_, bool on = true) : c(c_), saved(c_->stream) { if (on) c->stream = c->aux_stream; }
    ~AuxScope() { c->stream = saved; }
};
int sfg_stream_after(sfg_ctx *ctx, hipStream_t waiter, hipStream_t signaller);
int sfg_scratch(sfg_ctx *ctx, const char *name, size_t bytes, void **out);
int sfg_host_scratch(sfg_ctx *ctx, const char *name, size_t bytes, void **out);
void sfg_phases_resolve(sfg_ctx *ctx);

struct PhaseTimer {
    sfg_ctx *ctx; const char *name; hipEvent_t e0, e1; bool on;
    PhaseTimer(sfg_ctx *c, const char *n, bool enable = true) : ctx(c), name(n), on(enable) {
        if (on) { (void)hipEventCreate(&e0); (void)hipEventCreate(&e1); (void)hipEventRecord(e0, ctx->stream); }
    }
    void stop(int launches = 1, double bytes = 0) {
        if (!on) return;
        (void)hipEventRecord(e1, ctx->stream);
        ctx->pending.push_back(PendingEvent{e0, e1, name, launches, bytes});
        on = false;
        if (ctx->pending.size() > 4096) sfg_phases_resolve(ctx);
    }
    ~PhaseTimer() { stop(0); }
};

constexpr u64 PACKED_ZERO = 0ULL;
#ifdef __HIPCC__
__device__ __host__ __forceinline__ u64 pack_limbs(u64 w) {
    return (w & 0xFFF) | (((w >> 12) & 0xFFF) << 16) | ((w >> 24) << 32);
}

__device__ __forceinline__ double mulmod_lazy(double x, double w, double wq, double q) {
    double qh = __builtin_rint(x * wq);
    double h = x * w;
    double l = __builtin_fma(x, w, -h);
    double r = __builtin_fma(-qh, q, h);
    return r + l;
}
__device__ __forceinline__ double mulmod_lazy_q(double x, double w, double q, double qinv) {
    double h = x * w;
    double qh = __builtin_rint(h * qinv);
    double l = __builtin_fma(x, w, -h);
    double r = __builtin_fma(-qh, q, h);
    return r + l;
}
__device__ __forceinline__ double canon(double x, double q, double qinv) {
    const double r = __builtin_fma(-__builtin_floor(x * qinv), q, x);
    return r == q ? 0.0 : r;
}
__device__ __forceinline__ double canon_le(double x, double q, double qinv) {
    return __builtin_fma(-__builtin_floor(x * qinv), q, x);
}
__device__ __forceinline__ double pred(double x, double q, double qinv) {
    double qh = __builtin_rint(x * qinv);
    return __builtin_fma(-qh, q, x);
}
__device__ __forceinline__ double u64_to_f64(u64 x) {
    return __longlong_as_double((long long)(x | 0x4330000000000000ULL)) - 4503599627370496.0;
}
__device__ __forceinline__ u64 f64_to_u64(double x) {
    return (u64)__double_as_longlong(x + 4503599627370496.0) & 0x000FFFFFFFFFFFFFULL;
}
__device__ __forceinline__ void bytes_tr4(unsigned w0, unsigned w1, unsigned w2, unsigned w3, unsigned (&o)[4]) {
    const unsigned p0 = __builtin_amdgcn_perm(w1, w0, 0x05010400u), p1 = __builtin_amdgcn_perm(w1, w0, 0x07030602u);
    const unsigned q0 = __builtin_amdgcn_perm(w3, w2, 0x05010400u), q1 = __builtin_amdgcn_perm(w3, w2, 0x07030602u);
    o[0] = __builtin_amdgcn_perm(q0, p0, 0x05040100u); o[1] = __builtin_amdgcn_perm(q0, p0, 0x07060302u);
    o[2] = __builtin_amdgcn_perm(q1, p1, 0x05040100u); o[3] = __builtin_amdgcn_perm(q1, p1, 0x07060302u);
}
__device__ __forceinline__ int sq_sum4_i8(int w) {
    const int sq = __builtin_amdgcn_sdot4(w, w, 0, false);
    if (sq < 128) return sq;
    int s = 0;
#pragma unroll
    for (int k = 0; k < 4; k++) { const int x = (int)(int8_t)(w >> (8 * k)); s += (int)(int8_t)(x * x); }
    return s;
}
__device__ __forceinline__ u64 pack_limbs_f64(double x) {
    const u64 b = (u64)__double_as_longlong(x + 4503599627370496.0);
    const unsigned lo = (unsigned)b, hi = (unsigned)(b >> 32);
    const unsigned x01 = ((lo << 4) & 0x0FFF0000u) | (lo & 0xFFFu);
    const unsigned x2 = __builtin_amdgcn_alignbit(hi, lo, 24) & 0xFFFu;
    return ((u64)x2 << 32) | x01;
}
__device__ __forceinline__ u64 d_mulmod_u64(u64 a, u64 b, u64 q) {
    u64 hi = __umul64hi(a, b), lo = a * b;
    u64 r = hi % q;
    for (int i = 63; i >= 0; i--) { u64 top = r >> 63; r = (r << 1) | ((lo >> i) & 1); if (top || r >= q) r -= q; }
    return r;
}
__device__ __forceinline__ u64 splitmix_at(u64 seed, u64 idx) {
    u64 z = seed + 0x9E3779B97F4A7C15ULL * (idx + 1);
    z = (z ^ (z >> 30)) * 0xBF58476D1CE4E5B9ULL;
    z = (z ^ (z >> 27)) * 0x94D049BB133111EBULL;
    return z ^ (z >> 31);
}
#endif
```

sfgwas_amd/csrc/ctx.hip:

```cpp
#include "common.hpp"

thread_local std::string g_create_error;

static u64 derive_psi(u64 q, int logN) {
    u64 phi = q - 1, n = phi; std::vector<u64> fac;
    for (u64 p = 2; p * p <= n; p += (p == 2 ? 1 : 2)) if (n % p == 0) { fac.push_back(p); while (n % p == 0) n /= p; }
    if (n > 1) fac.push_back(n);
    for (u64 g = 2;; g++) {
        bool ok = true;
        for (u64 f : fac) if (h_powmod(g, phi / f, q) == 1) { ok = false; break; }
        if (ok) return h_powmod(g, phi >> (logN + 1), q);
    }
}

int sfg_encoder_init(sfg_ctx *ctx);
void sfg_encoder_destroy(SfgShared *sh);
int sfg_kernel_attrs_init(sfg_ctx *ctx);
int mac_bc_set_attrs(sfg_ctx *ctx);
int ntt_set_attrs(sfg_ctx *ctx);
int encode_set_attrs(sfg_ctx *ctx);
int decrypt_set_attrs(sfg_ctx *ctx);
int mac_i8_set_attrs(sfg_ctx *ctx);

static void apply_public_config(SfgConfig &c, const sfg_config *pc) {
    if (!pc || pc->struct_size < sizeof(uint32_t) * 2) return;
    const size_t have = pc->struct_size;
#define SFG_CFG_HAS(f) (have >= offsetof(sfg_config, f) + sizeof(pc->f))
    if (SFG_CFG_HAS(mm_group) && pc->mm_group > 0) { c.mm_group = pc->mm_group; c.mm_group_auto = false; }
    if (SFG_CFG_HAS(acc_budget_bytes) && pc->acc_budget_bytes) c.acc_budget = pc->acc_budget_bytes;
    if (SFG_CFG_HAS(assoc_rotcache_bytes) && pc->assoc_rotcache_bytes) c.assoc_cache_budget = pc->assoc_rotcache_bytes == SIZE_MAX ? 0 : pc->assoc_rotcache_bytes;
    if (SFG_CFG_HAS(ksw_budget_bytes) && pc->ksw_budget_bytes) c.ksw_budget = std::max<size_t>(pc->ksw_budget_bytes, 16ULL << 20);
    if (SFG_CFG_HAS(enc_batch) && pc->enc_batch > 0) c.enc_batch = std::min(std::max(pc->enc_batch, 64), 8192);
    if (SFG_CFG_HAS(upload_blocking) && pc->upload_blocking) c.upload_blocking = true;
#undef SFG_CFG_HAS
}
static void read_config(SfgConfig &c, const sfg_config *pc) {
    auto env = [](const char *n) { return getenv(n); };
    apply_public_config(c, pc);
    if (const char *e = env("SFG_MM_GROUP")) { c.mm_group = atoi(e); if (c.mm_group < 1) c.mm_group = 1; c.mm_group_auto = false; }
    if (const char *e = env("SFG_MM_ACC_BUDGET_MB")) c.acc_budget = (size_t)atoll(e) << 20;
    if (const char *e = env("SFG_ASSOC_ROTCACHE_MB")) c.assoc_cache_budget = (size_t)atoll(e) << 20;
    if (const char *e = env("SFG_KSW_BUDGET_MB")) { c.ksw_budget = (size_t)atoll(e) << 20; if (c.ksw_budget < (16ULL << 20)) c.ksw_budget = 16ULL << 20; }
    if (const char *e = env("SFG_ENC_BATCH")) { c.enc_batch = atoi(e); if (c.enc_batch < 64) c.enc_batch = 64; if (c.enc_batch > 8192) c.enc_batch = 8192; }
    if (env("SFG_UPLOAD_BLOCKING")) c.upload_blocking = true;
    if (const char *e = env("SFG_ENABLE_TEST_HOOKS")) c.test_hooks = atoi(e) == 1;
    if (c.test_hooks) {
        if (const char *e = env("SFG_TEST_SCRATCH_OOM")) c.test_scratch_oom = e;
        if (const char *e = env("SFG_TEST_TIE_BAND_LOG2")) c.tie_band = ldexp(1.0, atoi(e));
    }
#ifdef SFG_AB
    ab_read_config(c);
#endif
}

static void ctx_bind_shared(sfg_ctx *ctx, SfgShared *sh) {
    ctx->sh = sh; ctx->device = sh->device; ctx->logN = sh->logN; ctx->N = sh->N; ctx->nq = sh->nq; ctx->np = sh->np; ctx->nmod = sh->nmod;
    ctx->beta = sh->beta; ctx->scale = sh->scale; ctx->cfg = sh->cfg; ctx->test_hooks = sh->cfg.test_hooks;
    memcpy(ctx->q, sh->q, sizeof sh->q); memcpy(ctx->psi, sh->psi, sizeof sh->psi); memcpy(ctx->modc_host, sh->modc_host, sizeof sh->modc_host);
    ctx->tw_fwd = sh->tw_fwd; ctx->tw_inv = sh->tw_inv; ctx->pack_fwd = sh->pack_fwd; ctx->pack_inv = sh->pack_inv; ctx->modc = sh->modc;
}
static const char *ctx_exec_init(sfg_ctx *ctx) {
    if (hipSetDevice(ctx->device) != hipSuccess) return "hipSetDevice failed";
    if (hipStreamCreateWithFlags(&ctx->own_stream, hipStreamNonBlocking) != hipSuccess) return "hipStreamCreate failed";
    ctx->stream = ctx->own_stream;
    {
        int lo = 0, hi = 0; (void)hipDeviceGetStreamPriorityRange(&lo, &hi);
        if (hipStreamCreateWithPriority(&ctx->aux_stream, hipStreamNonBlocking, lo) != hipSuccess) return "hipStreamCreate failed";
    }
    if (hipStreamCreateWithFlags(&ctx->coll_stream, hipStreamNonBlocking) != hipSuccess) return "hipStreamCreate failed";
    for (int i = 0; i < 4; i++) if (hipEventCreateWithFlags(&ctx->ev_pipe[i], hipEventDisableTiming) != hipSuccess) return "hipEventCreate failed";
    ctx->pin_bytes = 64u << 20;
    if (hipHostMalloc((void **)&ctx->pin, ctx->pin_bytes, hipHostMallocDefault) != hipSuccess) return "hipHostMalloc failed";
    if (hipMalloc(&ctx->tie_count_dev, 32) != hipSuccess || hipMemset(ctx->tie_count_dev, 0, 32) != hipSuccess) return "hipMalloc failed";
    return nullptr;
}

extern "C" void sfg_config_default(sfg_config *c) { if (c) { memset(c, 0, sizeof *c); c->struct_size = (uint32_t)sizeof *c; } }
extern "C" int sfg_ctx_create(sfg_ctx **out, int device, int logN, int nq, int np,
                              const uint64_t *moduli, const uint64_t *psi, double scale) {
    return sfg_ctx_create_ex(out, device, logN, nq, np, moduli, psi, scale, nullptr);
}
extern "C" int sfg_ctx_create_ex(sfg_ctx **out, int device, int logN, int nq, int np,
                                 const uint64_t *moduli, const uint64_t *psi, double scale, const sfg_config *config) {
    if (!out) { g_create_error = "null result pointer"; return 1; }
    *out = nullptr;
    if (logN != SFG_LOGN) { g_create_error = "only logN = 14 (PN14QP438) is built into this library"; return 1; }
    if (nq < 1 || np < 1 || nq + np > SFG_MAXMOD) { g_create_error = "bad modulus counts"; return 1; }
    int ndev = 0;
    if (hipGetDeviceCount(&ndev) != hipSuccess || ndev == 0) { g_create_error = "no HIP device: libsfgwas_hip has no CPU fallback"; return 1; }
    if (device < 0 || device >= ndev) { g_create_error = "bad device index"; return 1; }
    sfg_ctx *ctx = new sfg_ctx();
    SfgShared *sh = new SfgShared();
    ctx->sh = sh; ctx->device = device;
    sh->device = device; sh->nq = nq; sh->np = np; sh->nmod = nq + np; sh->beta = (nq + np - 1) / np; sh->scale = scale;
    read_config(sh->cfg, config);
    auto fail = [&](const char *m) { std::string msg = m; sfg_ctx_destroy(ctx); g_create_error = msg; return 1; };
    if (const char *e = ctx_exec_init(ctx)) return fail(e);
    const int N = SFG_N;
    std::vector<double> twf((size_t)sh->nmod * N), twi((size_t)sh->nmod * N);
    for (int m = 0; m < sh->nmod; m++) {
        u64 q = moduli[m];
        if (q >= (1ULL << 47) || (q - 1) % (2ULL * N)) return fail("modulus must be < 2^47 (exact fp64 arithmetic: 14 lazy NTT stages stay below 2^51) and == 1 mod 2N");
        sh->q[m] = q;
        if (m < nq && q > SFG_I8_BIG_QMAX) sh->cfg.mac_i8_big = false;
        sh->psi[m] = psi ? psi[m] : derive_psi(q, logN);
        if (h_powmod(sh->psi[m], N, q) != q - 1) return fail("psi is not a primitive 2N-th root of unity");
        u64 psi_inv = h_invmod(sh->psi[m], q), p = 1, pi = 1;
        for (int k = 0; k < N; k++) {
            uint32_t b = h_brev((uint32_t)k, logN);
            twf[(size_t)m * N + b] = (double)p;
            twi[(size_t)m * N + b] = (double)pi;
            p = h_mulmod(p, sh->psi[m], q); pi = h_mulmod(pi, psi_inv, q);
        }
        ModConst &mc = sh->modc_host[m];
        mc.q = (double)q; mc.qinv = 1.0 / (double)q; mc.qi = q;
        u64 ninv = h_invmod((u64)N, q);
        mc.ninv = (double)ninv; mc.ninv_q = (double)ninv / (double)q;
    }
    auto build_pack = [&](const std::vector<double> &tw, std::vector<double2> &pk) {
        pk.assign((size_t)sh->nmod * (N / 2), make_double2(0, 0));
        for (int m = 0; m < sh->nmod; m++) {
            const double *t = tw.data() + (size_t)m * N;
            for (int p = 0; p < N / 16; p++) {
                double e[16]; int k = 0;
                e[k++] = t[1024 + p];
                for (int g = 0; g < 2; g++) e[k++] = t[2048 + 2 * p + g];
                for (int g = 0; g < 4; g++) e[k++] = t[4096 + 4 * p + g];
                for (int g = 0; g < 8; g++) e[k++] = t[8192 + 8 * p + g];
                e[k++] = 0.0;
                for (int i = 0; i < 8; i++) pk[(size_t)m * (N / 2) + (size_t)(p >> 6) * 512 + (size_t)i * 64 + (p & 63)] = make_double2(e[2 * i], e[2 * i + 1]);
            }
        }
    };
    std::vector<double2> pkf, pki; build_pack(twf, pkf); build_pack(twi, pki);
    if (hipMalloc(&sh->tw_fwd, twf.size() * sizeof(double)) != hipSuccess || hipMalloc(&sh->tw_inv, twi.size() * sizeof(double)) != hipSuccess ||
        hipMalloc(&sh->pack_fwd, pkf.size() * sizeof(double2)) != hipSuccess || hipMalloc(&sh->pack_inv, pki.size() * sizeof(double2)) != hipSuccess ||
        hipMalloc(&sh->modc, sizeof(ModConst) * SFG_MAXMOD) != hipSuccess || hipMalloc(&sh->zeros_dev, 512) != hipSuccess) return fail("hipMalloc of tables failed");
    if (hipMemcpy(sh->tw_fwd, twf.data(), twf.size() * sizeof(double), hipMemcpyHostToDevice) != hipSuccess ||
        hipMemcpy(sh->tw_inv, twi.data(), twi.size() * sizeof(double), hipMemcpyHostToDevice) != hipSuccess ||
        hipMemcpy(sh->pack_fwd, pkf.data(), pkf.size() * sizeof(double2), hipMemcpyHostToDevice) != hipSuccess ||
        hipMemcpy(sh->pack_inv, pki.data(), pki.size() * sizeof(double2), hipMemcpyHostToDevice) != hipSuccess ||
        hipMemcpy(sh->modc, sh->modc_host, sizeof(ModConst) * SFG_MAXMOD, hipMemcpyHostToDevice) != hipSuccess ||
        hipMemset(sh->zeros_dev, 0, 512) != hipSuccess) return fail("table upload failed");
    {
        u64 pz[32]; for (int i = 0; i < 32; i++) pz[i] = PACKED_ZERO;
        if (hipMemcpy((char *)sh->zeros_dev + 256, pz, 256, hipMemcpyHostToDevice) != hipSuccess) return fail("table upload failed");
    }
    ctx_bind_shared(ctx, sh);
    if (sfg_encoder_init(ctx)) { std::string e = ctx->err; return fail(e.c_str()); }
    if (mac_bc_set_attrs(ctx) || ntt_set_attrs(ctx) || encode_set_attrs(ctx) || mac_i8_set_attrs(ctx) || encrypt_set_attrs(ctx) || decrypt_set_attrs(ctx)) { std::string e = ctx->err; return fail(e.c_str()); }
    *out = ctx;
    return 0;
}

extern "C" int sfg_ctx_fork(sfg_ctx *parent, sfg_ctx **out) {
    *out = nullptr;
    sfg_ctx *ctx = new sfg_ctx();
    ctx->is_fork = true;
    ctx_bind_shared(ctx, parent->sh);
    __atomic_add_fetch(&parent->sh->refs, 1, __ATOMIC_ACQ_REL);
    if (const char *e = ctx_exec_init(ctx)) { parent->err = std::string("sfg_ctx_fork: ") + e; sfg_ctx_destroy(ctx); return 1; }
    *out = ctx;
    return 0;
}

extern "C" void sfg_ctx_destroy(sfg_ctx *ctx) {
    if (!ctx) return;
    (void)hipSetDevice(ctx->device);
    if (ctx->own_stream) (void)hipStreamSynchronize(ctx->own_stream);
    if (ctx->aux_stream) (void)hipStreamSynchronize(ctx->aux_stream);
    if (ctx->coll_stream) (void)hipStreamSynchronize(ctx->coll_stream);
    if (ctx->user_stream) (void)hipStreamSynchronize(ctx->user_stream);
    sfg_phases_resolve(ctx);
    sfg_ptc_detach_all(ctx);
    for (auto &kv : ctx->ksw_cache) (void)hipFree(kv.second);
    for (auto &kv : ctx->host_pool) (void)hipHostFree(kv.second.first);
    for (auto &kv : ctx->pool) (void)hipFree(kv.second.first);
    (void)hipFree(ctx->ws); (void)hipFree(ctx->tie_count_dev);
    if (ctx->own_stream) (void)hipStreamDestroy(ctx->own_stream);
    if (ctx->aux_stream) (void)hipStreamDestroy(ctx->aux_stream);
    if (ctx->coll_stream) (void)hipStreamDestroy(ctx->coll_stream);
    if (ctx->pin) (void)hipHostFree(ctx->pin);
    for (hipEvent_t e : ctx->ev_pool) (void)hipEventDestroy(e);
    for (int i = 0; i < 4; i++) if (ctx->ev_pipe[i]) (void)hipEventDestroy(ctx->ev_pipe[i]);
    SfgShared *sh = ctx->sh;
    if (sh && __atomic_sub_fetch(&sh->refs, 1, __ATOMIC_ACQ_REL) == 0) {
        for (auto &kv : sh->rotkeys) { (void)hipFree(kv.second.key_dev); (void)hipFree(kv.second.index_dev); }
        sfg_encoder_destroy(sh);
        sfg_encrypt_destroy(sh);
        (void)hipFree(sh->tw_fwd); (void)hipFree(sh->tw_inv); (void)hipFree(sh->pack_fwd); (void)hipFree(sh->pack_inv); (void)hipFree(sh->modc); (void)hipFree(sh->zeros_dev); (void)hipFree(sh->sk_dev);
        delete sh;
    }
    delete ctx;
}

extern "C" const char *sfg_last_error(const sfg_ctx *ctx) { return ctx ? ctx->err.c_str() : g_create_error.c_str(); }

extern "C" int sfg_ctx_synchronize(sfg_ctx *ctx) {
    SFG_HIP(ctx, hipSetDevice(ctx->device));
    SFG_TRY(sfg_sync_all(ctx));
    return sfg_encoder_check(ctx);
}
extern "C" int sfg_ctx_set_stream(sfg_ctx *ctx, void *s) {
    if (!s) SFG_FAIL(ctx, "sfg_ctx_set_stream: a NULL handle is HIP's default stream - create an explicit (non-default) stream, or call sfg_ctx_use_own_stream");
    ctx->user_stream = (hipStream_t)s; ctx->stream = ctx->main_stream(); return 0;
}
extern "C" int sfg_ctx_use_own_stream(sfg_ctx *ctx) { ctx->user_stream = nullptr; ctx->stream = ctx->main_stream(); return 0; }
int sfg_sync_all(sfg_ctx *ctx) {
    SFG_HIP(ctx, hipStreamSynchronize(ctx->stream));
    if (ctx->user_stream && ctx->user_stream != ctx->stream) SFG_HIP(ctx, hipStreamSynchronize(ctx->user_stream));
    if (ctx->own_stream && ctx->own_stream != ctx->stream) SFG_HIP(ctx, hipStreamSynchronize(ctx->own_stream));
    if (ctx->aux_stream && ctx->aux_stream != ctx->stream) SFG_HIP(ctx, hipStreamSynchronize(ctx->aux_stream));
    if (ctx->coll_stream && ctx->coll_stream != ctx->stream) SFG_HIP(ctx, hipStreamSynchronize(ctx->coll_stream));
    return 0;
}

int sfg_upload_small(sfg_ctx *ctx, void *dst_dev, const void *src_host, size_t bytes) {
    if (!bytes) return 0;
    const size_t need = (bytes + 255) & ~(size_t)255;
    if (ctx->cfg.upload_blocking || need > ctx->pin_bytes / 4) {
        SFG_HIP(ctx, hipStreamSynchronize(ctx->stream));
        SFG_HIP(ctx, hipMemcpy(dst_dev, src_host, bytes, hipMemcpyHostToDevice));
        return 0;
    }
    if (ctx->pin_head + need > ctx->pin_bytes) {
        SFG_TRY(sfg_sync_all(ctx));
        ctx->pin_head = 0;
    }
    unsigned char *slot = ctx->pin + ctx->pin_head; ctx->pin_head += need;
    memcpy(slot, src_host, bytes);
    SFG_HIP(ctx, hipMemcpyAsync(dst_dev, slot, bytes, hipMemcpyHostToDevice, ctx->stream));
    return 0;
}
int sfg_stream_after(sfg_ctx *ctx, hipStream_t waiter, hipStream_t signaller) {
    if (waiter == signaller) return 0;
    if (ctx->ev_pool.size() < 64) { hipEvent_t e; SFG_HIP(ctx, hipEventCreateWithFlags(&e, hipEventDisableTiming)); ctx->ev_pool.push_back(e); ctx->ev_next = ctx->ev_pool.size() - 1; }
    hipEvent_t e = ctx->ev_pool[ctx->ev_next]; ctx->ev_next = (ctx->ev_next + 1) % ctx->ev_pool.size();
    SFG_HIP(ctx, hipEventRecord(e, signaller));
    SFG_HIP(ctx, hipStreamWaitEvent(waiter, e, 0));
    return 0;
}

int sfg_ws_reserve(sfg_ctx *ctx, size_t bytes) {
    if (bytes <= ctx->ws_bytes) return 0;
    SFG_TRY(sfg_sync_all(ctx));
    if (ctx->ws) SFG_HIP(ctx, hipFree(ctx->ws));
    ctx->ws = nullptr; ctx->ws_bytes = 0;
    SFG_HIP(ctx, hipMalloc(&ctx->ws, bytes));
    ctx->ws_bytes = bytes;
    return 0;
}

extern "C" int sfg_ctx_release_scratch(sfg_ctx *ctx);
extern "C" int sfg_malloc(sfg_ctx *ctx, void **p, size_t bytes) {
    SFG_HIP(ctx, hipSetDevice(ctx->device));
    hipError_t err = hipMalloc(p, bytes);
    if (err == hipErrorOutOfMemory && ctx->api_depth == 0 && !ctx->pool.empty()) {
        (void)hipGetLastError();
        SFG_TRY(sfg_ctx_release_scratch(ctx));
        err = hipMalloc(p, bytes);
    }
    SFG_HIP(ctx, err);
    return 0;
}
extern "C" int sfg_free(sfg_ctx *ctx, void *p) { SFG_HIP(ctx, hipSetDevice(ctx->device)); SFG_HIP(ctx, hipStreamSynchronize(ctx->stream)); SFG_HIP(ctx, hipFree(p)); return 0; }
extern "C" int sfg_memcpy_h2d(sfg_ctx *ctx, void *d, const void *s, size_t n) {
    SFG_HIP(ctx, hipSetDevice(ctx->device)); SFG_HIP(ctx, hipMemcpyAsync(d, s, n, hipMemcpyHostToDevice, ctx->stream)); SFG_HIP(ctx, hipStreamSynchronize(ctx->stream)); return 0;
}
extern "C" int sfg_memcpy_d2h(sfg_ctx *ctx, void *d, const void *s, size_t n) {
    SFG_HIP(ctx, hipSetDevice(ctx->device)); SFG_HIP(ctx, hipMemcpyAsync(d, s, n, hipMemcpyDeviceToHost, ctx->stream)); SFG_HIP(ctx, hipStreamSynchronize(ctx->stream));
    return sfg_encoder_check(ctx);
}

void sfg_phases_resolve(sfg_ctx *ctx) {
    if (ctx->pending.empty()) return;
    (void)hipEventSynchronize(ctx->pending.back().e1);
    for (auto &p : ctx->pending) {
        float ms = 0; (void)hipEventSynchronize(p.e1); (void)hipEventElapsedTime(&ms, p.e0, p.e1);
        auto &st = ctx->phases[p.name]; st.ms += ms; st.launches += p.launches; st.bytes += p.bytes;
        (void)hipEventDestroy(p.e0); (void)hipEventDestroy(p.e1);
    }
    ctx->pending.clear();
}
int sfg_scratch(sfg_ctx *ctx, const char *name, size_t bytes, void **out) {
    auto &e = ctx->pool[name];
    ctx->pool_epoch[name] = ctx->api_epoch;
    bool inject = false;
    if (ctx->test_hooks && !ctx->cfg.test_scratch_oom.empty() && ctx->api_depth > 0) {
        const std::string &t = ctx->cfg.test_scratch_oom; const size_t c = t.rfind(':');
        if (t.compare(0, c, name) == 0 && strlen(name) == (c == std::string::npos ? t.size() : c))
            inject = ++ctx->scratch_oom_seen == (c == std::string::npos ? 1 : atoi(t.c_str() + c + 1));
    }
    if (e.second < bytes || inject) {
        SFG_TRY(sfg_sync_all(ctx));
        if (e.first) SFG_HIP(ctx, hipFree(e.first));
        e.first = nullptr; e.second = 0;
        hipError_t err = inject ? hipErrorOutOfMemory : hipMalloc(&e.first, bytes);
        if (err != hipSuccess && ctx->api_depth > 0) {
            (void)hipGetLastError();
            bool freed_rot_copy = false;
            for (auto it = ctx->pool.begin(); it != ctx->pool.end();) {
                if (it->first != name && it->second.first && ctx->pool_epoch[it->first] < ctx->api_epoch) {
                    if (it->first.rfind("mi8.A", 0) == 0) freed_rot_copy = true;
                    (void)hipFree(it->second.first); ctx->pool_epoch.erase(it->first); it = ctx->pool.erase(it);
                } else ++it;
            }
            if (freed_rot_copy) { for (int b = 0; b < 2; b++) for (int i = 0; i < sfg_ctx::I8_SLOTS; i++) ctx->i8_slot[b][i] = sfg_ctx::I8Slot(); ctx->i8_gen++; }
            auto &e2 = ctx->pool[name];
            err = hipMalloc(&e2.first, bytes);
            if (err != hipSuccess) { e2.first = nullptr; e2.second = 0; SFG_FAIL(ctx, "out of device memory: %zu bytes for scratch buffer '%s' (after returning the buffers of earlier calls)", bytes, name); }
            e2.second = bytes; *out = e2.first;
            return 0;
        }
        if (err != hipSuccess) { e.first = nullptr; SFG_FAIL(ctx, "out of device memory: %zu bytes for scratch buffer '%s' (sfg_ctx_release_scratch returns the grown pools)", bytes, name); }
        e.second = bytes;
    }
    *out = e.first;
    return 0;
}
extern "C" int sfg_ctx_release_scratch(sfg_ctx *ctx) {
    SFG_HIP(ctx, hipSetDevice(ctx->device));
    SFG_TRY(sfg_sync_all(ctx));
    for (auto &kv : ctx->pool) (void)hipFree(kv.second.first);
    ctx->pool.clear(); ctx->pool_epoch.clear();
    for (auto &kv : ctx->host_pool) (void)hipHostFree(kv.second.first);
    ctx->host_pool.clear();
    for (int b = 0; b < 2; b++) for (int i = 0; i < sfg_ctx::I8_SLOTS; i++) ctx->i8_slot[b][i] = sfg_ctx::I8Slot();
    ctx->i8_gen++;
    return 0;
}
int sfg_host_scratch(sfg_ctx *ctx, const char *name, size_t bytes, void **out) {
    auto &e = ctx->host_pool[name];
    if (e.second < bytes) {
        if (e.first) { SFG_TRY(sfg_sync_all(ctx)); SFG_HIP(ctx, hipHostFree(e.first)); }
        e.first = nullptr; e.second = 0;
        SFG_HIP(ctx, hipHostMalloc(&e.first, bytes, hipHostMallocDefault));
        e.second = bytes;
    }
    *out = e.first;
    return 0;
}
extern "C" int sfg_ctx_scratch_bytes(const sfg_ctx *ctx, const char *prefix, size_t *bytes) {
    size_t n = 0; const std::string pre = prefix ? prefix : "";
    for (const auto &kv : ctx->pool) if (kv.second.first && kv.first.rfind(pre, 0) == 0) n += kv.second.second;
    if (bytes) *bytes = n;
    return 0;
}
extern "C" int sfg_rotcache_invalidate(sfg_ctx *ctx) { ctx->i8_gen++; return 0; }
extern "C" int sfg_ctx_clear_phases(sfg_ctx *ctx) { sfg_phases_resolve(ctx); ctx->phases.clear(); return 0; }
extern "C" double sfg_last_phase_ms(const sfg_ctx *ctx, const char *phase) {
    sfg_phases_resolve(const_cast<sfg_ctx *>(ctx));
    auto it = ctx->phases.find(phase); return it == ctx->phases.end() ? -1.0 : it->second.ms;
}
extern "C" double sfg_last_phase_bytes(const sfg_ctx *ctx, const char *phase) {
    sfg_phases_resolve(const_cast<sfg_ctx *>(ctx));
    auto it = ctx->phases.find(phase); return it == ctx->phases.end() ? -1.0 : it->second.bytes;
}
extern "C" int sfg_last_phase_launches(const sfg_ctx *ctx, const char *phase) {
    sfg_phases_resolve(const_cast<sfg_ctx *>(ctx));
    auto it = ctx->phases.find(phase); return it == ctx->phases.end() ? -1 : it->second.launches;
}

extern "C" uint64_t sfg_galois_for_rotation(const sfg_ctx *ctx, int k) {
    const u64 M = 2ULL * SFG_N; int n = SFG_SLOTS; k %= n; if (k < 0) k += n;
    u64 g = 1; for (int i = 0; i < k; i++) g = (g * 5) % M; return g;
}
extern "C" int sfg_ctx_has_rotkey(const sfg_ctx *ctx, uint64_t g) { return ctx->rotkeys().count(g) ? 1 : 0; }

extern "C" int sfg_ctx_export_rotkey(sfg_ctx *ctx, uint64_t g, uint64_t *key_host) {
    SFG_HIP(ctx, hipSetDevice(ctx->device));
    auto it = ctx->rotkeys().find(g);
    if (it == ctx->rotkeys().end()) SFG_FAIL(ctx, "export_rotkey: no key loaded for galois element %llu", (unsigned long long)g);
    const size_t words = (size_t)ctx->beta * 2 * ctx->nmod * SFG_N;
    SFG_HIP(ctx, hipMemcpyAsync(key_host, it->second.key_dev, words * 8, hipMemcpyDeviceToHost, ctx->stream));
    SFG_HIP(ctx, hipStreamSynchronize(ctx->stream));
    return 0;
}

__global__ void k_from_montgomery(u64 *rows, int nmod, const ModConst *modc, size_t total_rows) {
    size_t row = blockIdx.y; int m = (int)(row % nmod); u64 q = modc[m].qi;
    __shared__ u64 r64inv;
    if (threadIdx.x == 0) {
        u64 r = ((~0ULL) % q + 1) % q;
        u64 e = q - 2, base = r, acc = 1;
        while (e) { if (e & 1) acc = d_mulmod_u64(acc, base, q); base = d_mulmod_u64(base, base, q); e >>= 1; }
        r64inv = acc;
    }
    __syncthreads();
    u64 *p = rows + row * SFG_N;
    for (int x = blockIdx.x * blockDim.x + threadIdx.x; x < SFG_N; x += gridDim.x * blockDim.x) p[x] = d_mulmod_u64(p[x], r64inv, q);
}

int sfg_rows_from_montgomery(sfg_ctx *ctx, u64 *rows_dev, size_t nrows, int nmod) {
    dim3 grid(8, (unsigned)nrows);
    hipLaunchKernelGGL(k_from_montgomery, grid, dim3(256), 0, ctx->stream, rows_dev, nmod, ctx->modc, nrows);
    SFG_HIP(ctx, hipGetLastError());
    return 0;
}
extern "C" int sfg_ctx_load_secret_key(sfg_ctx *ctx, const uint64_t *sk_host, int mont) {
    SFG_HIP(ctx, hipSetDevice(ctx->device));
    const size_t words = (size_t)ctx->nq * SFG_N;
    if (!ctx->sh->sk_dev) SFG_HIP(ctx, hipMalloc(&ctx->sh->sk_dev, words * 8));
    SFG_HIP(ctx, hipMemcpyAsync(ctx->sh->sk_dev, sk_host, words * 8, hipMemcpyHostToDevice, ctx->stream));
    if (mont) {
        dim3 grid(8, (unsigned)ctx->nq);
        hipLaunchKernelGGL(k_from_montgomery, grid, dim3(256), 0, ctx->stream, ctx->sh->sk_dev, ctx->nq, ctx->modc, (size_t)grid.y);
    }
    SFG_HIP(ctx, hipStreamSynchronize(ctx->stream));
    return 0;
}

extern "C" int sfg_ctx_load_rotkey(sfg_ctx *ctx, uint64_t g, const uint64_t *key_host, int mont) {
    SFG_HIP(ctx, hipSetDevice(ctx->device));
    const int N = SFG_N; size_t words = (size_t)ctx->beta * 2 * ctx->nmod * N;
    RotKey rk;
    auto it = ctx->rotkeys().find(g);
    if (it != ctx->rotkeys().end()) rk = it->second;
    else { SFG_HIP(ctx, hipMalloc(&rk.key_dev, words * 8)); SFG_HIP(ctx, hipMalloc(&rk.index_dev, N * sizeof(uint16_t))); }
    SFG_HIP(ctx, hipMemcpyAsync(rk.key_dev, key_host, words * 8, hipMemcpyHostToDevice, ctx->stream));
    if (mont) {
        dim3 grid(8, (unsigned)((size_t)ctx->beta * 2 * ctx->nmod));
        hipLaunchKernelGGL(k_from_montgomery, grid, dim3(256), 0, ctx->stream, rk.key_dev, ctx->nmod, ctx->modc, (size_t)grid.y);
    }
    std::vector<uint16_t> idx(N); u64 mask = 2ULL * N - 1;
    for (int i = 0; i < N; i++) { u64 t1 = 2ULL * h_brev((uint32_t)i, SFG_LOGN) + 1; u64 t2 = ((g * t1 & mask) - 1) >> 1; idx[i] = (uint16_t)h_brev((uint32_t)t2, SFG_LOGN); }
    SFG_HIP(ctx, hipMemcpyAsync(rk.index_dev, idx.data(), N * sizeof(uint16_t), hipMemcpyHostToDevice, ctx->stream));
    SFG_HIP(ctx, hipStreamSynchronize(ctx->stream));
    ctx->rotkeys()[g] = rk;
    return 0;
}
```

sfgwas_amd/csrc/ddfft.hpp:

```cpp
#pragma once
#include "common.hpp"
#include <cmath>
#include <type_traits>

struct dd { double hi, lo; };
__host__ __device__ static inline dd dd_make(double h, double l) { dd r; r.hi = h; r.lo = l; return r; }
__host__ __device__ static inline dd dd_quick(double a, double b) { double s = a + b; return dd_make(s, b - (s - a)); }
__host__ __device__ static inline dd dd_two_sum(double a, double b) { double s = a + b, bb = s - a; return dd_make(s, (a - (s - bb)) + (b - bb)); }
__host__ __device__ static inline dd dd_add(dd a, dd b) { dd s = dd_two_sum(a.hi, b.hi); s.lo += a.lo + b.lo; return dd_quick(s.hi, s.lo); }
__host__ __device__ static inline dd dd_neg(dd a) { return dd_make(-a.hi, -a.lo); }
__host__ __device__ static inline dd dd_add_lazy(dd a, dd b) { dd s = dd_two_sum(a.hi, b.hi); s.lo += a.lo + b.lo; return s; }
__host__ __device__ static inline dd dd_sub_lazy(dd a, dd b) { dd s = dd_two_sum(a.hi, -b.hi); s.lo += a.lo - b.lo; return s; }
__host__ __device__ static inline dd dd_sub(dd a, dd b) { return dd_add(a, dd_neg(b)); }
__host__ __device__ static inline dd dd_mul(dd a, dd b) {
    double p = a.hi * b.hi, e = fma(a.hi, b.hi, -p);
    e = fma(a.hi, b.lo, e); e = fma(a.lo, b.hi, e);
    return dd_quick(p, e);
}
__host__ __device__ static inline dd dd_mul_d(dd a, double b) {
    double p = a.hi * b, e = fma(a.hi, b, -p);
    e = fma(a.lo, b, e);
    return dd_quick(p, e);
}
static inline dd dd_add_acc(dd a, dd b) {
    dd s = dd_two_sum(a.hi, b.hi), t = dd_two_sum(a.lo, b.lo);
    s.lo += t.hi; s = dd_quick(s.hi, s.lo); s.lo += t.lo; return dd_quick(s.hi, s.lo);
}
struct cdd { dd re, im; };
__host__ __device__ static inline cdd cdd_mul(cdd a, cdd b) {
    cdd r; r.re = dd_sub(dd_mul(a.re, b.re), dd_mul(a.im, b.im)); r.im = dd_add(dd_mul(a.re, b.im), dd_mul(a.im, b.re)); return r;
}

constexpr int ENC_H = SFG_SLOTS / 2;
constexpr int ENC_TW = 16384;
constexpr int ENC_TB_P512 = 0, ENC_TB_P64 = ENC_TB_P512 + 7 * 512, ENC_TB_P8 = ENC_TB_P64 + 7 * 64;
constexpr int ENC_TB_RLEN = ENC_H / 2 + 1;
constexpr int ENC_TB_RW = ENC_TB_P8 + 7 * 8, ENC_TB_RZ = ENC_TB_RW + ENC_TB_RLEN, ENC_TB_RZ2 = ENC_TB_RZ + ENC_TB_RLEN;
constexpr int ENC_TB_SIZE = ENC_TB_RZ2 + ENC_TB_RLEN;

struct EncTables {
    double4 *tb = nullptr;
    uint16_t *tinv = nullptr;
    double2 *costab = nullptr;
    int sexp = -1;
    double4 *dec = nullptr;
};

static inline void dd_sincos_small(dd theta, dd &s, dd &c) {
    dd t2 = dd_mul(theta, theta);
    dd term = theta; s = theta;
    for (int k = 1; k < 14; k++) {
        term = dd_mul(term, t2); term = dd_mul_d(term, -1.0);
        double den = (double)(2 * k) * (double)(2 * k + 1);
        dd q; q.hi = term.hi / den; double rem = fma(-q.hi, den, term.hi); q.lo = (rem + term.lo) / den; term = dd_quick(q.hi, q.lo);
        s = dd_add_acc(s, term);
    }
    term = dd_make(1.0, 0.0); c = term;
    for (int k = 1; k < 14; k++) {
        term = dd_mul(term, t2); term = dd_mul_d(term, -1.0);
        double den = (double)(2 * k - 1) * (double)(2 * k);
        dd q; q.hi = term.hi / den; double rem = fma(-q.hi, den, term.hi); q.lo = (rem + term.lo) / den; term = dd_quick(q.hi, q.lo);
        c = dd_add_acc(c, term);
    }
}

__device__ __forceinline__ int padj(int j) { return j ^ ((j >> 3) & 31); }
__device__ __forceinline__ int padj_fin(int j) { return j ^ ((j >> 5) & 15); }

__device__ __forceinline__ dd dd_dot2(dd a, dd w, dd b, dd x, double sgn) {
    const double p1 = a.hi * w.hi, e1 = fma(a.hi, w.hi, -p1);
    const double bh = sgn * b.hi, bl = sgn * b.lo;
    const double p2 = bh * x.hi, e2 = fma(bh, x.hi, -p2);
    dd s = dd_two_sum(p1, p2);
    double lo = e1 + e2;
    lo = fma(a.hi, w.lo, lo); lo = fma(a.lo, w.hi, lo);
    lo = fma(bh, x.lo, lo); lo = fma(bl, x.hi, lo);
    return dd_quick(s.hi, s.lo + lo);
}
constexpr double GRID_M = 3145728.0;
__device__ __forceinline__ dd grid_split(double p, double e) { const double h = (p + GRID_M) - GRID_M; return dd_make(h, (p - h) + e); }
template <bool GRID> __device__ __forceinline__ dd fx_add(dd a, dd b) { return GRID ? dd_make(a.hi + b.hi, a.lo + b.lo) : dd_add_lazy(a, b); }
template <bool GRID> __device__ __forceinline__ dd fx_sub(dd a, dd b) { return GRID ? dd_make(a.hi - b.hi, a.lo - b.lo) : dd_sub_lazy(a, b); }
template <bool GRID> __device__ __forceinline__ dd fx_mul(dd a, dd b) {
    double p = a.hi * b.hi, e = fma(a.hi, b.hi, -p);
    e = fma(a.hi, b.lo, e); e = fma(a.lo, b.hi, e);
    return GRID ? grid_split(p, e) : dd_quick(p, e);
}
template <bool GRID> __device__ __forceinline__ dd fx_dot2(dd a, dd w, dd b, dd x, double sgn) {
    const double p1 = a.hi * w.hi, e1 = fma(a.hi, w.hi, -p1);
    const double bh = sgn * b.hi, bl = sgn * b.lo;
    const double p2 = bh * x.hi, e2 = fma(bh, x.hi, -p2);
    if (GRID) {
        const double h1 = (p1 + GRID_M) - GRID_M, h2 = (p2 + GRID_M) - GRID_M;
        double lo = (p1 - h1) + (p2 - h2);
        lo += e1 + e2;
        lo = fma(a.hi, w.lo, lo); lo = fma(a.lo, w.hi, lo);
        lo = fma(bh, x.lo, lo); lo = fma(bl, x.hi, lo);
        return dd_make(h1 + h2, lo);
    }
    dd s = dd_two_sum(p1, p2);
    double lo = e1 + e2;
    lo = fma(a.hi, w.lo, lo); lo = fma(a.lo, w.hi, lo);
    lo = fma(bh, x.lo, lo); lo = fma(bl, x.hi, lo);
    return dd_quick(s.hi, s.lo + lo);
}
#ifndef SFG_ENC_DIAG
#define SFG_ENC_DIAG 0
#endif
__device__ __forceinline__ void tw_at(const double4 *tab, int idx, dd &wr, dd &wi) {
    if (SFG_ENC_DIAG & 1) { wr = dd_make(0.7 + idx * 1e-9, 1e-18); wi = dd_make(0.3 - idx * 1e-9, 2e-18); return; }
    const double4 w = tab[idx];
    wr = dd_make(w.x, w.y); wi = dd_make(w.z, w.w);
}
template <int S, bool GRID>
__device__ __forceinline__ void dif_radix8(dd (&xr)[8], dd (&xi)[8], const double4 *tab, int t) {
    const dd rs = dd_make(7.071067811865475727e-01, -4.833646656726456726e-17);
    dd ur[4], ui[4], dr[4], di[4];
#pragma unroll
    for (int i = 0; i < 4; i++) {
        ur[i] = fx_add<GRID>(xr[i], xr[i + 4]); ui[i] = fx_add<GRID>(xi[i], xi[i + 4]);
        dr[i] = fx_sub<GRID>(xr[i], xr[i + 4]); di[i] = fx_sub<GRID>(xi[i], xi[i + 4]);
    }
    {
        dd a = dr[1], b = di[1];
        dr[1] = fx_mul<GRID>(fx_add<GRID>(a, b), rs); di[1] = fx_mul<GRID>(fx_sub<GRID>(b, a), rs);
    }
    {
        dd a = dr[2]; dr[2] = di[2]; di[2] = dd_neg(a);
    }
    {
        dd a = dr[3], b = di[3];
        dr[3] = fx_mul<GRID>(fx_sub<GRID>(b, a), rs); di[3] = dd_neg(fx_mul<GRID>(fx_add<GRID>(a, b), rs));
    }
    auto quad = [&](dd (&hr)[4], dd (&hi)[4], int o) {
        dd p0r = fx_add<GRID>(hr[0], hr[2]), p0i = fx_add<GRID>(hi[0], hi[2]);
        dd p1r = fx_add<GRID>(hr[1], hr[3]), p1i = fx_add<GRID>(hi[1], hi[3]);
        dd q0r = fx_sub<GRID>(hr[0], hr[2]), q0i = fx_sub<GRID>(hi[0], hi[2]);
        dd t1r = fx_sub<GRID>(hr[1], hr[3]), t1i = fx_sub<GRID>(hi[1], hi[3]);
        dd q1r = t1i, q1i = dd_neg(t1r);
        xr[o + 0] = fx_add<GRID>(p0r, p1r); xi[o + 0] = fx_add<GRID>(p0i, p1i);
        xr[o + 1] = fx_sub<GRID>(p0r, p1r); xi[o + 1] = fx_sub<GRID>(p0i, p1i);
        xr[o + 2] = fx_add<GRID>(q0r, q1r); xi[o + 2] = fx_add<GRID>(q0i, q1i);
        xr[o + 3] = fx_sub<GRID>(q0r, q1r); xi[o + 3] = fx_sub<GRID>(q0i, q1i);
    };
    quad(ur, ui, 0);
    quad(dr, di, 4);
    if (S > 1) {
#pragma unroll
        for (int r = 1; r < 8; r++) {
            if (SFG_ENC_DIAG & 8) continue;
            dd wr, wi; tw_at(tab, (r - 1) * S + t, wr, wi);
            const dd pr = fx_dot2<GRID>(xr[r], wr, xi[r], wi, -1.0), pi = fx_dot2<GRID>(xr[r], wi, xi[r], wr, 1.0);
            xr[r] = pr; xi[r] = pi;
        }
    }
}
```

sfgwas_amd/csrc/encode.hip:

```cpp
#include "common.hpp"
#include "kernels.hpp"
#include "i8_move.hpp"
#include "ddfft.hpp"



int sfg_encoder_init(sfg_ctx *ctx) {
    EncTables *et = new EncTables();
    ctx->sh->enc_tables = et;
    const int n = SFG_SLOTS; const u64 M = 2ULL * SFG_N;
    dd pi = dd_make(3.141592653589793116e+00, 1.224646799147353207e-16);
    dd theta = dd_make(pi.hi / 16384.0, pi.lo / 16384.0);
    dd s1, c1; dd_sincos_small(theta, s1, c1);
    std::vector<cdd> z(ENC_TW + 1);
    z[0].re = dd_make(1, 0); z[0].im = dd_make(0, 0);
    z[1].re = c1; z[1].im = dd_neg(s1);
    for (int k = 2; k <= ENC_TW; k++) z[k] = (k & 1) ? cdd_mul(z[k - 1], z[1]) : cdd_mul(z[k / 2], z[k / 2]);
    z[ENC_TW].re = dd_make(-1, 0); z[ENC_TW].im = dd_make(0, 0);
    z[ENC_TW / 2].re = dd_make(0, 0); z[ENC_TW / 2].im = dd_make(-1, 0);
    auto zat = [&](int idx) {
        const bool neg = idx > ENC_TW; const cdd w = z[neg ? idx - ENC_TW : idx]; const double sg = neg ? -1.0 : 1.0;
        return make_double4(sg * w.re.hi, sg * w.re.lo, sg * w.im.hi, sg * w.im.lo);
    };
    std::vector<double4> tb(ENC_TB_SIZE);
    {
        const int E[8] = {0, 4, 2, 6, 1, 5, 3, 7};
        const int S3[3] = {512, 64, 8}, off[3] = {ENC_TB_P512, ENC_TB_P64, ENC_TB_P8};
        for (int k = 0; k < 3; k++) for (int r = 1; r < 8; r++) for (int t = 0; t < S3[k]; t++) tb[off[k] + (r - 1) * S3[k] + t] = zat(E[r] * t * (4096 / S3[k]));
        const double son = ctx->sh->scale / (double)n;
        auto scaled = [&](int idx) {
            const double4 w = zat(idx); const dd re = dd_mul_d(dd_make(w.x, w.y), son), im = dd_mul_d(dd_make(w.z, w.w), son);
            return make_double4(re.hi, re.lo, im.hi, im.lo);
        };
        for (int c = 0; c < ENC_TB_RLEN; c++) { { const double4 w = zat(4 * c); tb[ENC_TB_RW + c] = make_double4(0.5 * w.x, 0.5 * w.y, 0.5 * w.z, 0.5 * w.w); } tb[ENC_TB_RZ + c] = scaled(c); tb[ENC_TB_RZ2 + c] = scaled(ENC_H - c); }
    }
    {
        std::vector<double4> dt(2 * ENC_H);
        for (int c = 0; c < ENC_H; c++) {
            const double4 a = zat(c), b = zat(4 * c);
            dt[c] = make_double4(0.5 * a.x, 0.5 * a.y, -0.5 * a.z, -0.5 * a.w); dt[ENC_H + c] = make_double4(b.x, b.y, -b.z, -b.w);
        }
        SFG_HIP(ctx, hipMalloc(&et->dec, dt.size() * sizeof(double4)));
        SFG_HIP(ctx, hipMemcpy(et->dec, dt.data(), dt.size() * sizeof(double4), hipMemcpyHostToDevice));
    }
    std::vector<uint16_t> tinv(n);
    u64 g = 1;
    for (int t = 0; t < n; t++) { tinv[((g - 1) / 4) % n] = (uint16_t)t; g = (g * 5) % M; }
    {
        std::vector<double2> ct(ENC_TW / 2 + 1);
        for (int k = 0; k <= ENC_TW / 2; k++) ct[k] = make_double2(z[k].re.hi, z[k].re.lo);
        SFG_HIP(ctx, hipMalloc(&et->costab, ct.size() * sizeof(double2)));
        SFG_HIP(ctx, hipMemcpy(et->costab, ct.data(), ct.size() * sizeof(double2), hipMemcpyHostToDevice));
        int e = 0; const double son = std::frexp(ctx->sh->scale / (double)n, &e);
        et->sexp = (son == 0.5 && e - 1 >= 0 && e - 1 <= 40) ? e - 1 : -1;
    }
    SFG_HIP(ctx, hipMalloc(&et->tb, tb.size() * sizeof(double4)));
    SFG_HIP(ctx, hipMalloc(&et->tinv, n * sizeof(uint16_t)));
    SFG_HIP(ctx, hipMemcpy(et->tb, tb.data(), tb.size() * sizeof(double4), hipMemcpyHostToDevice));
    SFG_HIP(ctx, hipMemcpy(et->tinv, tinv.data(), n * sizeof(uint16_t), hipMemcpyHostToDevice));
    return 0;
}
void sfg_encoder_destroy(SfgShared *sh) {
    EncTables *et = (EncTables *)sh->enc_tables;
    if (!et) return;
    (void)hipFree(et->tb); (void)hipFree(et->tinv); (void)hipFree(et->costab); (void)hipFree(et->dec);
    delete et; sh->enc_tables = nullptr;
}

constexpr int SK_T = 128, SK_U = 2 * SK_T - 1, SK_PITCH = 144, SK_PITCH_T = 272;
constexpr int SK_LDS = SK_U * SK_PITCH > SK_T * SK_PITCH_T ? SK_U * SK_PITCH : SK_T * SK_PITCH_T;
__device__ __forceinline__ unsigned sk_clean(unsigned w, int square) {
    const unsigned t = w & 0x80808080u;
    w &= ~((t << 1) - (t >> 7));
    if (square) {
        unsigned o = 0;
#pragma unroll
        for (int k = 0; k < 4; k++) { const unsigned v = (w >> (8 * k)) & 0xFFu; o |= ((v * v) & 0xFFu) << (8 * k); }
        w = o;
    }
    return w;
}
template <bool TR>
__global__ void __launch_bounds__(256) k_skew(const int8_t *blk, size_t ld, int r, int c, int square, int8_t *D) {
    __shared__ __attribute__((aligned(16))) int8_t tile[SK_LDS];
    const int n = SFG_SLOTS, tid = threadIdx.x;
    const int J0 = blockIdx.x * SK_T, S0 = blockIdx.y * SK_T;
    auto load4 = [&](const int8_t *src, int nvalid) -> unsigned {
        if (nvalid >= 4 && ((uintptr_t)src & 3) == 0) return *reinterpret_cast<const unsigned *>(src);
        unsigned w = 0;
#pragma unroll
        for (int k = 0; k < 4; k++) if (k < nvalid) w |= (unsigned)(uint8_t)src[k] << (8 * k);
        return w;
    };
    auto load16 = [&](const int8_t *src, int nvalid) -> uint4 {
        if (nvalid >= 16 && ((uintptr_t)src & 15) == 0) return *reinterpret_cast<const uint4 *>(src);
        return make_uint4(load4(src, nvalid), load4(src + 4, nvalid - 4), load4(src + 8, nvalid - 8), load4(src + 12, nvalid - 12));
    };
    if (!TR) {
        const int x = tid & 7;
        for (int u = tid >> 3; u < SK_U; u += 32) {
            int i = S0 + J0 + u; if (i >= n) i -= n;
            const int j = J0 + 16 * x;
            const uint4 w = i < r ? load16(blk + (size_t)i * ld + j, c - j) : make_uint4(0, 0, 0, 0);
            *reinterpret_cast<uint4 *>(tile + u * SK_PITCH + 16 * x) = w;
        }
    } else {
        const int x = tid & 15;
        for (int jj = tid >> 4; jj < SK_T; jj += 16) {
            const int u = 16 * x;
            int i = S0 + J0 + u; if (i >= n) i -= n;
            const int j = J0 + jj;
            const uint4 w = j < c ? load16(blk + (size_t)j * ld + i, r - i) : make_uint4(0, 0, 0, 0);
            *reinterpret_cast<uint4 *>(tile + jj * SK_PITCH_T + u) = w;
        }
    }
    __syncthreads();
    const int q = tid & 31;
#pragma unroll
    for (int it = 0; it < 4; it++) {
        const int s0 = 4 * ((tid >> 5) + 8 * it);
        unsigned out[4];
        if (!TR) {
            unsigned W[7], E[6];
#pragma unroll
            for (int k = 0; k < 7; k++) W[k] = *reinterpret_cast<const unsigned *>(tile + (s0 + 4 * q + k) * SK_PITCH + 4 * q);
#pragma unroll
            for (int k = 0; k < 6; k++) E[k] = __builtin_amdgcn_perm(W[k + 1], W[k], 0x07020500u);
#pragma unroll
            for (int m = 0; m < 4; m++) out[m] = __builtin_amdgcn_perm(E[m + 2], E[m], 0x07060100u);
        } else {
            unsigned V[4];
#pragma unroll
            for (int t = 0; t < 4; t++) {
                const unsigned *rowp = reinterpret_cast<const unsigned *>(tile + (4 * q + t) * SK_PITCH_T + s0 + 4 * q);
                V[t] = t ? __builtin_amdgcn_alignbyte(rowp[1], rowp[0], (unsigned)t) : rowp[0];
            }
            const unsigned P0 = __builtin_amdgcn_perm(V[1], V[0], 0x05010400u), P1 = __builtin_amdgcn_perm(V[1], V[0], 0x07030602u);
            const unsigned Q0 = __builtin_amdgcn_perm(V[3], V[2], 0x05010400u), Q1 = __builtin_amdgcn_perm(V[3], V[2], 0x07030602u);
            out[0] = __builtin_amdgcn_perm(Q0, P0, 0x05040100u); out[1] = __builtin_amdgcn_perm(Q0, P0, 0x07060302u);
            out[2] = __builtin_amdgcn_perm(Q1, P1, 0x05040100u); out[3] = __builtin_amdgcn_perm(Q1, P1, 0x07060302u);
        }
#pragma unroll
        for (int m = 0; m < 4; m++) *reinterpret_cast<unsigned *>(D + (size_t)(S0 + s0 + m) * n + J0 + 4 * q) = sk_clean(out[m], square);
    }
}

__device__ __forceinline__ dd dd_dot2_raw(dd a, dd w, dd b, dd x, double sgn) {
    const double p1 = a.hi * w.hi, e1 = fma(a.hi, w.hi, -p1);
    const double bh = sgn * b.hi, bl = sgn * b.lo;
    const double p2 = bh * x.hi, e2 = fma(bh, x.hi, -p2);
    dd s = dd_two_sum(p1, p2);
    double lo = e1 + e2;
    lo = fma(a.hi, w.lo, lo); lo = fma(a.lo, w.hi, lo);
    lo = fma(bh, x.lo, lo); lo = fma(bl, x.hi, lo);
    return dd_make(s.hi, s.lo + lo);
}
__device__ __forceinline__ void cdd_mul_ip(dd &re, dd &im, dd wr, dd wi) {
    const dd r = dd_dot2(re, wr, im, wi, -1.0), i = dd_dot2(re, wi, im, wr, 1.0);
    re = r; im = i;
}

template <bool EXACT_TIES>
__device__ __forceinline__ double dd_round_away(dd x, unsigned &near_tie, double band, bool &inside) {
    double nn = __builtin_rint(x.hi);
    double diff = (x.hi - nn) + x.lo;
    if (!EXACT_TIES) {
        const double tie_dist = __builtin_fabs(__builtin_fabs(diff) - 0.5);
        inside = tie_dist < band;
        near_tie += (tie_dist < 0x1p-40 ? 1u : 0u);
        return nn + __builtin_rint(diff);
    }
    const double k = __builtin_rint(diff), e = diff - k, b = nn + k;
    const double tie_dist = __builtin_fabs(__builtin_fabs(e) - 0.5);
    inside = tie_dist < band;
    near_tie += (tie_dist < 0x1p-40 ? 1u : 0u);
    const bool up = (e == 0.5) & (b >= 0), dn = (e == -0.5) & (b <= 0);
    return b + (up ? 1.0 : 0.0) - (dn ? 1.0 : 0.0);
}

__device__ __noinline__ bool enc_tie_resolve(const int8_t *row, const uint16_t *tinv, int nrot, const double2 *costab, int sexp, int j, double *out) {
    const int n = SFG_SLOTS;
    __int128 sa = 0, sb = 0, sc = 0;
    for (int m = 0; m < n; m++) {
        int t = (int)tinv[m] - nrot; t += t < 0 ? n : 0;
        const int v = (int)row[t];
        if (!v) continue;
        unsigned k = ((4u * (unsigned)m + 1u) * (unsigned)j) & 32767u;
        if (k > 16384u) k = 32768u - k;
        const bool neg = k > 8192u; if (neg) k = 16384u - k;
        const double2 cv = costab[k];
        const double x = cv.x * 0x1p20, a = __builtin_rint(x), r1 = x - a;
        const double y = r1 * 0x1p40, bq = __builtin_rint(y), r2 = y - bq;
        const double cq = __builtin_rint(r2 * 0x1p40 + cv.y * 0x1p100);
        const long long sv = neg ? -(long long)v : (long long)v;
        sa += (__int128)(sv * (long long)a); sb += (__int128)(sv * (long long)bq); sc += (__int128)(sv * (long long)cq);
    }
    const __int128 T = (sa << 80) + (sb << 40) + sc;
    const int sh = 100 - sexp;
    const __int128 q = T >> sh, rem = T - (q << sh), half = (__int128)1 << (sh - 1);
    const __int128 dist = rem > half ? rem - half : half - rem;
    if (dist <= ((__int128)1 << (sh - 62))) return false;
    *out = (double)((long long)q + (rem > half ? 1 : 0));
    return true;
}

constexpr unsigned long long ENC_DOM_NONFINITE = 1, ENC_DOM_RANGE = 2;
constexpr size_t ENC_LDS_BYTES = (size_t)2 * ENC_H * 8;
template <bool F64IN>
__global__ void __launch_bounds__(512, 4) k_fft_encode(const void *Dv, int shift0, const double4 *tb, const uint16_t *tinv,
                                                      double *pc_out, unsigned long long *tie_count, const double2 *costab, int sexp, double band, double band_rel) {
    unsigned near_tie = 0;
    extern __shared__ double lds[];
    double *RE = lds, *IM = lds + ENC_H;
    const int n = SFG_SLOTS, h = ENC_H, tid = threadIdx.x;
    const int shift = shift0 + blockIdx.x;
    const int nrot = F64IN ? 0 : SFG_D * (shift / SFG_D);
    const int8_t *row = (const int8_t *)Dv + (size_t)shift * n;
    const double *rowd = (const double *)Dv + (size_t)shift * n;
    int8_t *rowl = reinterpret_cast<int8_t *>(lds);
    if (!F64IN) reinterpret_cast<uint4 *>(rowl)[tid] = reinterpret_cast<const uint4 *>(row)[tid];
    __syncthreads();
    dd xr[8], xi[8], yr[8], yi[8];
    auto exchange = [&](dd (&sr)[8], dd (&si)[8], dd (&dr)[8], dd (&di)[8], auto widx, auto ridx, auto wave, bool entry_barrier) {
        constexpr bool WAVE = decltype(wave)::value;
        auto sync = [&]() { if (WAVE) __builtin_amdgcn_fence(__ATOMIC_ACQ_REL, "wavefront"); else __syncthreads(); };
        if (SFG_ENC_DIAG & 4) { for (int k = 0; k < 8; k++) { dr[k] = sr[k]; di[k] = si[k]; } return; }
        if (entry_barrier) __syncthreads(); else sync();
#pragma unroll
        for (int k = 0; k < 8; k++) { const int p = padj(widx(k)); RE[p] = sr[k].hi; IM[p] = si[k].hi; }
        sync();
#pragma unroll
        for (int k = 0; k < 8; k++) { const int p = padj(ridx(k)); dr[k].hi = RE[p]; di[k].hi = IM[p]; }
        sync();
#pragma unroll
        for (int k = 0; k < 8; k++) { const int p = padj(widx(k)); RE[p] = sr[k].lo; IM[p] = si[k].lo; }
        sync();
#pragma unroll
        for (int k = 0; k < 8; k++) { const int p = padj(ridx(k)); dr[k].lo = RE[p]; di[k].lo = IM[p]; }
    };
    const std::false_type wg_wide; const std::true_type wave_local;
#pragma unroll
    for (int a = 0; a < 8; a++) {
        const int m = a * 512 + tid;
        int t0 = (int)tinv[2 * m] - nrot, t1 = (int)tinv[2 * m + 1] - nrot;
        t0 += t0 < 0 ? n : 0; t1 += t1 < 0 ? n : 0;
        if (F64IN) { xr[a] = dd_make(rowd[t0], 0.0); xi[a] = dd_make(rowd[t1], 0.0); }
        else { xr[a] = dd_make((double)rowl[t0], 0.0); xi[a] = dd_make((double)rowl[t1], 0.0); }
    }
    bool out_of_domain = false;
    if (F64IN) {
        double s = 0.0;
#pragma unroll
        for (int a = 0; a < 8; a++) s += __builtin_fabs(xr[a].hi) + __builtin_fabs(xi[a].hi);
#pragma unroll
        for (int o = 32; o > 0; o >>= 1) s += __shfl_xor(s, o);
        if ((tid & 63) == 0) lds[tid >> 6] = s;
        __syncthreads();
        s = 0.0;
#pragma unroll
        for (int w = 0; w < 8; w++) s += lds[w];
        if (!__builtin_isfinite(s)) { if (tid == 0) atomicOr(tie_count + 3, ENC_DOM_NONFINITE); }
        else band = __builtin_fmax(band, s * band_rel);
    }
    dif_radix8<512, !F64IN>(xr, xi, tb + ENC_TB_P512, tid);
    {
        const int cd = tid & 63, ar = tid >> 6;
        exchange(xr, xi, yr, yi, [&](int a) { return a * 512 + tid; }, [&](int b) { return ar * 512 + b * 64 + cd; }, wg_wide, true);
        dif_radix8<64, !F64IN>(yr, yi, tb + ENC_TB_P64, cd);
        const int d = tid & 7, ab = tid >> 3;
        exchange(yr, yi, xr, xi, [&](int b) { return ar * 512 + b * 64 + cd; }, [&](int c) { return ab * 64 + c * 8 + d; }, wave_local, true);
        dif_radix8<8, !F64IN>(xr, xi, tb + ENC_TB_P8, d);
        exchange(xr, xi, yr, yi, [&](int c) { return ab * 64 + c * 8 + d; }, [&](int d4) { return tid * 8 + d4; }, wave_local, false);
        dif_radix8<1, !F64IN>(yr, yi, tb, 0);
    }
    double *pc = pc_out + (size_t)blockIdx.x * n;
    const int cbase = (int)(__brev((unsigned)tid) >> 23);
    dd Ar[5], Ai[5], Br[5], Bi[5];
    const int npair = tid == 0 ? 5 : 4;
    __syncthreads();
#pragma unroll
    for (int d4 = 0; d4 < 8; d4++) { const int p = padj_fin((int)((__brev((unsigned)d4) >> 29) << 9) | cbase); RE[p] = yr[d4].hi; IM[p] = yi[d4].hi; }
    __syncthreads();
#pragma unroll
    for (int i = 0; i < 5; i++) if (i < npair) {
        const int c = tid + 512 * i, pa = padj_fin(c), pb = padj_fin((h - c) & (h - 1));
        Ar[i].hi = RE[pa]; Ai[i].hi = IM[pa]; Br[i].hi = RE[pb]; Bi[i].hi = -IM[pb];
    }
    __syncthreads();
#pragma unroll
    for (int d4 = 0; d4 < 8; d4++) { const int p = padj_fin((int)((__brev((unsigned)d4) >> 29) << 9) | cbase); RE[p] = yr[d4].lo; IM[p] = yi[d4].lo; }
    __syncthreads();
#pragma unroll
    for (int i = 0; i < 5; i++) if (i < npair) {
        const int c = tid + 512 * i, pa = padj_fin(c), pb = padj_fin((h - c) & (h - 1));
        Ar[i].lo = RE[pa]; Ai[i].lo = IM[pa]; Br[i].lo = RE[pb]; Bi[i].lo = -IM[pb];
    }
    int tie_j = -1; unsigned tie_n = 0;
    auto note = [&](int j) { tie_j = j; tie_n++; };
    auto recomb = [&](int c, dd Ar, dd Ai, dd Br, dd Bi) {
        constexpr bool GRID = !F64IN;
        auto radd = [](dd a, dd b) { return GRID ? dd_make(a.hi + b.hi, a.lo + b.lo) : dd_add(a, b); };
        auto rsub = [](dd a, dd b) { return GRID ? dd_make(a.hi - b.hi, a.lo - b.lo) : dd_sub(a, b); };
        auto half = [](dd a) { return dd_make(a.hi * 0.5, a.lo * 0.5); };
        if (SFG_ENC_DIAG & 2) { pc[c] = Ar.hi; if (c > 0) pc[n - c] = Ai.hi; if (c < h / 2) { pc[h - c] = Br.hi; pc[n - (h - c)] = Bi.hi; } return; }
        const bool nt = SFG_ENC_DIAG & 16;
        const double4 wo = nt ? make_double4(0.7 + c * 1e-9, 1e-18, 0.3, 1e-18) : tb[ENC_TB_RW + c];
        const double4 zc = nt ? make_double4(0.6 + c * 1e-9, 1e-18, 0.4, 1e-18) : tb[ENC_TB_RZ + c];
        dd Xr = half(radd(Ar, Br)), Xi = half(radd(Ai, Bi));
        dd Dr = rsub(Ar, Br), Di = rsub(Ai, Bi);
        dd Or = Di, Oi = dd_neg(Dr);
        dd wor = dd_make(wo.x, wo.y), woi = dd_make(wo.z, wo.w);
        dd Yr = fx_dot2<GRID>(Or, wor, Oi, woi, -1.0), Yi = fx_dot2<GRID>(Or, woi, Oi, wor, 1.0);
        {
            dd Wr = radd(Xr, Yr), Wi = radd(Xi, Yi);
            dd zr = dd_make(zc.x, zc.y), zi = dd_make(zc.z, zc.w);
            dd wr = dd_dot2_raw(Wr, zr, Wi, zi, -1.0), wi = dd_dot2_raw(Wr, zi, Wi, zr, 1.0);
            bool in0, in1 = false;
            pc[c] = dd_round_away<F64IN>(wr, near_tie, band, in0);
            if (c > 0) pc[n - c] = -dd_round_away<F64IN>(wi, near_tie, band, in1);
            if (F64IN) out_of_domain |= !(__builtin_fabs(wr.hi) < 0x1p53) | !(__builtin_fabs(wi.hi) < 0x1p53);
            if (in0) note(c);
            if (in1) note(n - c);
        }
        if (c < h / 2) {
            const int cc = h - c;
            const double4 zh = nt ? make_double4(0.5 + c * 1e-9, 1e-18, 0.45, 1e-18) : tb[ENC_TB_RZ2 + c];
            dd Wr = rsub(Xr, Yr), Wi = dd_neg(rsub(Xi, Yi));
            dd zr = dd_make(zh.x, zh.y), zi = dd_make(zh.z, zh.w);
            dd wr = dd_dot2_raw(Wr, zr, Wi, zi, -1.0), wi = dd_dot2_raw(Wr, zi, Wi, zr, 1.0);
            bool in0, in1 = false;
            pc[cc] = dd_round_away<F64IN>(wr, near_tie, band, in0);
            if (cc < h) pc[n - cc] = -dd_round_away<F64IN>(wi, near_tie, band, in1);
            if (F64IN) out_of_domain |= !(__builtin_fabs(wr.hi) < 0x1p53) | !(__builtin_fabs(wi.hi) < 0x1p53);
            if (in0) note(cc);
            if (in1) note(n - cc);
        }
    };
#pragma unroll
    for (int i = 0; i < 4; i++) recomb(tid + 512 * i, Ar[i], Ai[i], Br[i], Bi[i]);
    if (tid == 0) recomb(h / 2, Ar[4], Ai[4], Br[4], Bi[4]);
    if (F64IN && __syncthreads_or(out_of_domain ? 1 : 0)) {
        if (tid == 0) atomicOr(tie_count + 3, ENC_DOM_RANGE);
        return;
    }
    if (tie_n) {
        unsigned unproven = tie_n - 1, resolved = 0;
        double v;
#ifndef SFG_ENC_NO_RESOLVE
        if (!F64IN && sexp >= 0 && enc_tie_resolve(row, tinv, nrot, costab, sexp, tie_j, &v)) { pc[tie_j] = v; resolved = 1; } else
#endif
            unproven++;
        if (resolved) atomicAdd(tie_count + 2, 1ULL);
        if (unproven) atomicAdd(tie_count + 1, (unsigned long long)unproven);
    }
    if (near_tie) atomicAdd(tie_count, (unsigned long long)near_tie);
}

static double enc_band_rel(const sfg_ctx *ctx) { return std::ldexp(ctx->sh->scale / (double)SFG_SLOTS, -88); }
static int enc_domain_check(sfg_ctx *ctx, const char *who) {
    unsigned long long f = 0;
    SFG_HIP(ctx, hipMemcpy(&f, (unsigned long long *)ctx->tie_count_dev + 3, 8, hipMemcpyDeviceToHost));
    if (f & ENC_DOM_NONFINITE) SFG_FAIL(ctx, "%s: a slot value is not finite (NaN or inf): outside the encoder's domain", who);
    if (f & ENC_DOM_RANGE) SFG_FAIL(ctx, "%s: a coefficient |Delta * w_c| reaches 2^53: outside the encoder's domain (the rounded integers must be exact doubles)", who);
    return 0;
}

static int enc_pc_scratch(sfg_ctx *ctx, size_t nplain, double **pc) {
    return sfg_scratch(ctx, "enc.pc", nplain * SFG_SLOTS * sizeof(double), (void **)pc);
}
int encode_set_attrs(sfg_ctx *ctx) {
    SFG_HIP(ctx, hipFuncSetAttribute((const void *)k_fft_encode<false>, hipFuncAttributeMaxDynamicSharedMemorySize, (int)ENC_LDS_BYTES));
    SFG_HIP(ctx, hipFuncSetAttribute((const void *)k_fft_encode<true>, hipFuncAttributeMaxDynamicSharedMemorySize, (int)ENC_LDS_BYTES));
    return 0;
}

int launch_skew(sfg_ctx *ctx, const int8_t *blk, size_t ld, int r, int c, int transposed, int square, int8_t *D) {
    if (transposed) hipLaunchKernelGGL(k_skew<true>, dim3(SFG_SLOTS / SK_T, SFG_SLOTS / SK_T), dim3(256), 0, ctx->stream, blk, ld, r, c, square, D);
    else hipLaunchKernelGGL(k_skew<false>, dim3(SFG_SLOTS / SK_T, SFG_SLOTS / SK_T), dim3(256), 0, ctx->stream, blk, ld, r, c, square, D);
    SFG_HIP(ctx, hipGetLastError());
    return 0;
}

int encode_rows_launches(const sfg_ctx *ctx, int nshift) { const int B = ctx->cfg.enc_batch; return (nshift + B - 1) / B; }
int launch_encode_rows(sfg_ctx *ctx, const int8_t *D, int shift0, int nshift, int L, u64 *pt, bool half_rows, int G, int g, unsigned packed_mask, const PcCache *pcache, PtRide *ride) {
    EncTables *et = (EncTables *)ctx->enc_tables();
    const size_t lds_bytes = ENC_LDS_BYTES;
    const int BATCH = ctx->cfg.enc_batch;
    const int cmode = pcache && pcache->slot && half_rows && G > 0 ? pcache->mode : 0;
    double *pc = nullptr;
    if (!cmode) SFG_TRY(enc_pc_scratch(ctx, (size_t)(nshift < BATCH ? nshift : BATCH), &pc));
    for (int s0 = 0; s0 < nshift; s0 += BATCH) {
        const int nb = nshift - s0 < BATCH ? nshift - s0 : BATCH;
        if (cmode == 1) pc = pcache->slot + (size_t)(shift0 + s0) * SFG_SLOTS;
        if (cmode <= 1) {
            PhaseTimer t(ctx, "encode", false);
            hipLaunchKernelGGL(k_fft_encode<false>, dim3(nb), dim3(512), lds_bytes, ctx->stream, (const void *)D, shift0 + s0, et->tb, et->tinv, pc, (unsigned long long *)ctx->tie_count_dev, et->costab, et->sexp, ctx->cfg.tie_band, 0.0);
            SFG_HIP(ctx, hipGetLastError());
        }
        if (cmode == 2) pc = pcache->slot + (size_t)(shift0 + s0) * SFG_SLOTS;
        const bool sampled = half_rows && G > 0 && (ctx->ntt_plain_seq++ & 15) == 0;
        const bool riding = half_rows && G > 0 && ride && ride->on && ride->next < ride->total();
        PhaseTimer tn(ctx, riding ? "ntt_plain_ride" : "ntt_plain", sampled);
        if (half_rows && G > 0) { PhaseStat &all = ctx->phases[riding ? "ntt_ride_all" : "ntt_plain_all"]; all.launches += 1; }
        if (half_rows && G > 0) {
            MoveJob mj; const MoveJob *mv = nullptr; double moved = 0;
            if (ride && ride->on && ride->next < ride->total()) {
                mj = ride->job; mj.first = ride->next; mj.count = std::min(ride->per, ride->total() - ride->next); ride->next += mj.count; mv = &mj;
                const unsigned hi = mj.first + mj.count, n5 = mj.n5, in5 = mj.first < n5 ? std::min(hi, n5) - mj.first : 0u;
                moved = in5 * ride->item_bytes5 + (mj.count - in5) * ride->item_bytes6;
                if (sampled) { PhaseStat &ps = ctx->phases["pt_ride"]; ps.launches += 1; ps.bytes += moved; }
            }
            PanelMap pm{G, g, shift0 + s0, packed_mask};
            if (packed_mask & PT_KMAJOR) pm.K = G * SFG_D;
            if (cmode == 3) SFG_TRY(launch_ntt_plain_half(ctx, pcache->slot, pt, nb, L, pm, pcache->perm, mv));
            else SFG_TRY(launch_ntt_plain_half(ctx, pc, pt, nb, L, pm, nullptr, mv));
        }
        else if (half_rows) { PanelMap pm{0, 0, 0}; SFG_TRY(launch_ntt_plain_half(ctx, pc, pt + (size_t)s0 * L * (SFG_N / 2), nb, L, pm)); }
        else SFG_TRY(launch_ntt_plain(ctx, pc, pt + (size_t)s0 * L * SFG_N, nb, L));
        if (sampled) {
            double wr = 0; for (int l = 0; l < L; l++) wr += ((packed_mask >> 31) && ((packed_mask >> l) & 1u)) ? 5.0 : ((packed_mask >> 30) & 1u) ? 6.0 : 8.0;
            tn.stop(1, (double)nb * (SFG_N / 2) * (8.0 + wr));
        }
    }
    return 0;
}

extern "C" int sfg_encode_diags_dev(sfg_ctx *ctx, const int8_t *block, size_t ld, int r, int c, int transposed,
                                    int shift0, int nshift, int L, uint64_t *pt) {
    SFG_HIP(ctx, hipSetDevice(ctx->device));
    if (r < 1 || c < 1 || r > SFG_SLOTS || c > SFG_SLOTS) SFG_FAIL(ctx, "sfg_encode_diags: block dims out of range");
    if (shift0 < 0 || nshift < 0 || shift0 + nshift > SFG_SLOTS) SFG_FAIL(ctx, "sfg_encode_diags: shift range out of range");
    if (L < 1 || L > ctx->nq) SFG_FAIL(ctx, "sfg_encode_diags: L out of range");
    int8_t *skew = nullptr;
    SFG_TRY(sfg_scratch(ctx, "enc.skew", (size_t)SFG_SLOTS * SFG_SLOTS, (void **)&skew));
    SFG_TRY(launch_skew(ctx, block, ld, r, c, transposed, 0, skew));
    u64 *half = nullptr;
    SFG_TRY(sfg_scratch(ctx, "enc.half", (size_t)nshift * L * (SFG_N / 2) * 8, (void **)&half));
    SFG_TRY(launch_encode_rows(ctx, skew, shift0, nshift, L, half, true));
    return launch_expand_half(ctx, half, (u64 *)pt, (size_t)nshift * L);
}

extern "C" int sfg_encode_coeffs_host(sfg_ctx *ctx, const double *values_host, int nvec, int64_t *coeffs_host) {
    SFG_HIP(ctx, hipSetDevice(ctx->device));
    if (nvec <= 0) return 0;
    EncTables *et = (EncTables *)ctx->enc_tables();
    const size_t n = SFG_SLOTS, lds_bytes = ENC_LDS_BYTES;
    double *dv = nullptr; double *dpc = nullptr;
    SFG_HIP(ctx, hipMalloc(&dv, (size_t)nvec * n * 8));
    if (hipMalloc(&dpc, (size_t)nvec * n * 8) != hipSuccess) { (void)hipFree(dv); SFG_FAIL(ctx, "encode_coeffs: out of device memory"); }
    std::vector<double> pc((size_t)nvec * n);
    int rc = 0;
    if (hipMemcpyAsync(dv, values_host, (size_t)nvec * n * 8, hipMemcpyHostToDevice, ctx->stream) != hipSuccess) rc = 1;
    if (!rc && hipMemsetAsync((unsigned long long *)ctx->tie_count_dev + 3, 0, 8, ctx->stream) != hipSuccess) rc = 1;
    if (!rc) {
        hipLaunchKernelGGL(k_fft_encode<true>, dim3(nvec), dim3(512), lds_bytes, ctx->stream, (const void *)dv, 0, et->tb, et->tinv, dpc, (unsigned long long *)ctx->tie_count_dev, et->costab, -1, ctx->cfg.tie_band, enc_band_rel(ctx));
        if (hipGetLastError() != hipSuccess) rc = 1;
    }
    if (!rc && hipMemcpyAsync(pc.data(), dpc, (size_t)nvec * n * 8, hipMemcpyDeviceToHost, ctx->stream) != hipSuccess) rc = 1;
    (void)hipStreamSynchronize(ctx->stream); (void)hipFree(dv); (void)hipFree(dpc);
    if (rc) SFG_FAIL(ctx, "encode_coeffs: device operation failed");
    SFG_TRY(enc_domain_check(ctx, "encode_coeffs"));
    for (int v = 0; v < nvec; v++) {
        const double *h = pc.data() + (size_t)v * n; int64_t *o = coeffs_host + (size_t)v * SFG_N;
        for (size_t c = 0; c < n; c++) o[c] = (int64_t)h[c];
        o[n] = 0;
        for (size_t c = 1; c < n; c++) o[n + c] = -(int64_t)h[n - c];
    }
    return 0;
}

extern "C" int sfg_encode_vectors_dev(sfg_ctx *ctx, const double *values_host, int nvec, int level, uint64_t *pt_dev) {
    SFG_HIP(ctx, hipSetDevice(ctx->device));
    if (nvec <= 0) return 0;
    if (level < 0 || level >= ctx->nq) SFG_FAIL(ctx, "encode_vectors: level out of range");
    EncTables *et = (EncTables *)ctx->enc_tables();
    const size_t n = SFG_SLOTS, lds_bytes = ENC_LDS_BYTES;
    void *p = nullptr;
    SFG_TRY(sfg_scratch(ctx, "enc.vectors", (size_t)nvec * n * 16, &p));
    double *dv = (double *)p; double *dpc = dv + (size_t)nvec * n;
    SFG_HIP(ctx, hipMemcpyAsync(dv, values_host, (size_t)nvec * n * 8, hipMemcpyHostToDevice, ctx->stream));
    SFG_HIP(ctx, hipMemsetAsync((unsigned long long *)ctx->tie_count_dev + 3, 0, 8, ctx->stream));
    hipLaunchKernelGGL(k_fft_encode<true>, dim3(nvec), dim3(512), lds_bytes, ctx->stream, (const void *)dv, 0, et->tb, et->tinv, dpc, (unsigned long long *)ctx->tie_count_dev, et->costab, -1, ctx->cfg.tie_band, enc_band_rel(ctx));
    SFG_HIP(ctx, hipGetLastError());
    SFG_TRY(launch_ntt_plain(ctx, dpc, (u64 *)pt_dev, (size_t)nvec, level + 1));
    SFG_HIP(ctx, hipStreamSynchronize(ctx->stream));
    return enc_domain_check(ctx, "encode_vectors");
}

extern "C" int sfg_ctx_encoder_near_ties(sfg_ctx *ctx, unsigned long long *count, int reset) {
    SFG_HIP(ctx, hipSetDevice(ctx->device));
    SFG_TRY(sfg_sync_all(ctx));
    unsigned long long c[2] = {0, 0};
    SFG_HIP(ctx, hipMemcpy(c, ctx->tie_count_dev, 16, hipMemcpyDeviceToHost));
    *count = c[0];
    if (reset) {
        if (c[1]) sfg_ptc_invalidate_all(ctx);
        SFG_HIP(ctx, hipMemset(ctx->tie_count_dev, 0, 32));
    }
    return 0;
}

int sfg_encoder_check(sfg_ctx *ctx) {
    unsigned long long c[2] = {0, 0};
    SFG_HIP(ctx, hipMemcpy(c, ctx->tie_count_dev, 16, hipMemcpyDeviceToHost));
    if (c[1]) sfg_ptc_invalidate_all(ctx);
    if (c[1]) SFG_FAIL(ctx, "encoder: %llu coefficient(s) within 2^-50 of a rounding tie - the double-double encoder cannot prove them rounded as the reference's 256-bit "
                            "EncoderBig rounds; re-derive the products of this context since the last reset with a big-float encoder (sfg_ctx_encoder_near_ties resets)", c[1]);
    return 0;
}
extern "C" int sfg_ctx_encoder_resolved(sfg_ctx *ctx, unsigned long long *count) {
    SFG_HIP(ctx, hipSetDevice(ctx->device));
    SFG_TRY(sfg_sync_all(ctx));
    SFG_HIP(ctx, hipMemcpy(count, (unsigned long long *)ctx->tie_count_dev + 2, 8, hipMemcpyDeviceToHost));
    return 0;
}
extern "C" int sfg_ctx_encoder_unprovable(sfg_ctx *ctx, unsigned long long *count) {
    SFG_HIP(ctx, hipSetDevice(ctx->device));
    SFG_HIP(ctx, hipStreamSynchronize(ctx->stream));
    SFG_HIP(ctx, hipMemcpy(count, (unsigned long long *)ctx->tie_count_dev + 1, 8, hipMemcpyDeviceToHost));
    return 0;
}
extern "C" int sfg_ctx_encoder_inject_unsafe_for_test(sfg_ctx *ctx, unsigned long long n) {
    if (!ctx->test_hooks) SFG_FAIL(ctx, "sfg_ctx_encoder_inject_unsafe_for_test: test hook, enabled only in a process that set the test switch before creating the context");
    SFG_HIP(ctx, hipSetDevice(ctx->device));
    unsigned long long c[2] = {0, n};
    SFG_HIP(ctx, hipMemcpy((unsigned long long *)ctx->tie_count_dev + 1, c + 1, 8, hipMemcpyHostToDevice));
    return 0;
}
```

Measured before the change: 6223 billion.

## Encode genotype diagonals with plain fp64 FFT plus error-bounded tie fallback

```diff
diff --git a/include/sfgwas_hip.h b/include/sfgwas_hip.h
--- a/include/sfgwas_hip.h
+++ b/include/sfgwas_hip.h
@@ -61,6 +61,7 @@
 int sfg_ctx_encoder_near_ties(sfg_ctx *ctx, unsigned long long *count, int reset);
 int sfg_ctx_encoder_resolved(sfg_ctx *ctx, unsigned long long *count);
 int sfg_ctx_encoder_unprovable(sfg_ctx *ctx, unsigned long long *count);
+int sfg_ctx_encoder_fast_stats_for_test(sfg_ctx *ctx, unsigned long long *same_lane, unsigned long long *redone);
 int sfg_ctx_encoder_inject_unsafe_for_test(sfg_ctx *ctx, unsigned long long n);
 int sfg_encode_vectors_dev(sfg_ctx *ctx, const double *values_host, int nvec, int level, uint64_t *pt_dev);
 
diff --git a/sfgwas_amd/capi.py b/sfgwas_amd/capi.py
--- a/sfgwas_amd/capi.py
+++ b/sfgwas_amd/capi.py
@@ -7,7 +7,7 @@
 AB_LIB_PATH = os.path.join(_HERE, "lib_ab", "libsfgwas_hip.so")
 DEPLOYMENT_SWITCHES = {"SFG_MM_GROUP", "SFG_MM_ACC_BUDGET_MB", "SFG_ASSOC_ROTCACHE_MB", "SFG_KSW_BUDGET_MB", "SFG_ENC_BATCH", "SFG_UPLOAD_BLOCKING",
                        "SFG_MGPU_TRANSPORT", "SFG_MGPU_CACHE_GB", "SFG_RCCL_LIB", "SFG_ENABLE_TEST_HOOKS",
-                       "SFG_TEST_SCRATCH_OOM", "SFG_TEST_TIE_BAND_LOG2", "SFG_MGPU_FORCE_COLLECTIVES"}
+                       "SFG_TEST_SCRATCH_OOM", "SFG_TEST_TIE_BAND_LOG2", "SFG_TEST_ENC_DD", "SFG_TEST_ENC_BAND_MULT_LOG2", "SFG_MGPU_FORCE_COLLECTIVES"}
 
 
 def ab_lib():
@@ -66,6 +66,7 @@
         "sfg_ctx_encoder_inject_unsafe_for_test": (i, [vp, C.c_ulonglong]),
         "sfg_ctx_encoder_resolved": (i, [vp, C.POINTER(C.c_ulonglong)]),
         "sfg_ctx_encoder_unprovable": (i, [vp, C.POINTER(C.c_ulonglong)]),
+        "sfg_ctx_encoder_fast_stats_for_test": (i, [vp, C.POINTER(C.c_ulonglong), C.POINTER(C.c_ulonglong)]),
         "sfg_ctx_load_rotkey": (i, [vp, u64, u64p, i]),
         "sfg_ctx_load_secret_key": (i, [vp, u64p, i]),
         "sfg_ctx_load_public_key": (i, [vp, u64p, i]),
diff --git a/sfgwas_amd/csrc/common.hpp b/sfgwas_amd/csrc/common.hpp
--- a/sfgwas_amd/csrc/common.hpp
+++ b/sfgwas_amd/csrc/common.hpp
@@ -58,6 +58,8 @@
     bool test_hooks = false;
     std::string test_scratch_oom;
     double tie_band = 0x1p-50;
+    bool enc_dd = false;
+    double enc_band_mult = 1.0;
     bool mac_i8_big = true;
     bool mac_reg = false;
     bool mac_bc = true;
diff --git a/sfgwas_amd/csrc/ctx.hip b/sfgwas_amd/csrc/ctx.hip
--- a/sfgwas_amd/csrc/ctx.hip
+++ b/sfgwas_amd/csrc/ctx.hip
@@ -47,6 +47,8 @@
     if (c.test_hooks) {
         if (const char *e = env("SFG_TEST_SCRATCH_OOM")) c.test_scratch_oom = e;
         if (const char *e = env("SFG_TEST_TIE_BAND_LOG2")) c.tie_band = ldexp(1.0, atoi(e));
+        if (const char *e = env("SFG_TEST_ENC_DD")) c.enc_dd = atoi(e) == 1;
+        if (const char *e = env("SFG_TEST_ENC_BAND_MULT_LOG2")) c.enc_band_mult = ldexp(1.0, std::max(0, atoi(e)));
     }
 #ifdef SFG_AB
     ab_read_config(c);
@@ -71,7 +73,7 @@
     for (int i = 0; i < 4; i++) if (hipEventCreateWithFlags(&ctx->ev_pipe[i], hipEventDisableTiming) != hipSuccess) return "hipEventCreate failed";
     ctx->pin_bytes = 64u << 20;
     if (hipHostMalloc((void **)&ctx->pin, ctx->pin_bytes, hipHostMallocDefault) != hipSuccess) return "hipHostMalloc failed";
-    if (hipMalloc(&ctx->tie_count_dev, 32) != hipSuccess || hipMemset(ctx->tie_count_dev, 0, 32) != hipSuccess) return "hipMalloc failed";
+    if (hipMalloc(&ctx->tie_count_dev, 48) != hipSuccess || hipMemset(ctx->tie_count_dev, 0, 48) != hipSuccess) return "hipMalloc failed";
     return nullptr;
 }
 
diff --git a/sfgwas_amd/csrc/ddfft.hpp b/sfgwas_amd/csrc/ddfft.hpp
--- a/sfgwas_amd/csrc/ddfft.hpp
+++ b/sfgwas_amd/csrc/ddfft.hpp
@@ -104,17 +104,26 @@
     lo = fma(bh, x.lo, lo); lo = fma(bl, x.hi, lo);
     return dd_quick(s.hi, s.lo + lo);
 }
+template <bool GRID> __device__ __forceinline__ double fx_add(double a, double b) { return a + b; }
+template <bool GRID> __device__ __forceinline__ double fx_sub(double a, double b) { return a - b; }
+template <bool GRID> __device__ __forceinline__ double fx_mul(double a, double b) { return a * b; }
+template <bool GRID> __device__ __forceinline__ double fx_dot2(double a, double w, double b, double x, double sgn) { return fma(a, w, (sgn * b) * x); }
+__host__ __device__ static inline double dd_neg(double a) { return -a; }
+template <typename T> __device__ __forceinline__ T fx_const(double hi, double lo);
+template <> __device__ __forceinline__ dd fx_const<dd>(double hi, double lo) { return dd_make(hi, lo); }
+template <> __device__ __forceinline__ double fx_const<double>(double hi, double) { return hi; }
 #ifndef SFG_ENC_DIAG
 #define SFG_ENC_DIAG 0
 #endif
-__device__ __forceinline__ void tw_at(const double4 *tab, int idx, dd &wr, dd &wi) {
-    if (SFG_ENC_DIAG & 1) { wr = dd_make(0.7 + idx * 1e-9, 1e-18); wi = dd_make(0.3 - idx * 1e-9, 2e-18); return; }
-    const double4 w = tab[idx];
-    wr = dd_make(w.x, w.y); wi = dd_make(w.z, w.w);
+template <typename T> __device__ __forceinline__ void tw_at(const double4 *tab, int idx, T &wr, T &wi) {
+    if (SFG_ENC_DIAG & 1) { wr = fx_const<T>(0.7 + idx * 1e-9, 1e-18); wi = fx_const<T>(0.3 - idx * 1e-9, 2e-18); return; }
+    if constexpr (std::is_same<T, double>::value) { wr = tab[idx].x; wi = tab[idx].z; }
+    else { const double4 w = tab[idx]; wr = dd_make(w.x, w.y); wi = dd_make(w.z, w.w); }
 }
-template <int S, bool GRID>
-__device__ __forceinline__ void dif_radix8(dd (&xr)[8], dd (&xi)[8], const double4 *tab, int t) {
-    const dd rs = dd_make(7.071067811865475727e-01, -4.833646656726456726e-17);
+template <int S, bool GRID, typename T>
+__device__ __forceinline__ void dif_radix8(T (&xr)[8], T (&xi)[8], const double4 *tab, int t) {
+    using dd = T;
+    const dd rs = fx_const<T>(7.071067811865475727e-01, -4.833646656726456726e-17);
     dd ur[4], ui[4], dr[4], di[4];
 #pragma unroll
     for (int i = 0; i < 4; i++) {
diff --git a/sfgwas_amd/csrc/encode.hip b/sfgwas_amd/csrc/encode.hip
--- a/sfgwas_amd/csrc/encode.hip
+++ b/sfgwas_amd/csrc/encode.hip
@@ -178,47 +178,92 @@
     return b + (up ? 1.0 : 0.0) - (dn ? 1.0 : 0.0);
 }
 
-__device__ __noinline__ bool enc_tie_resolve(const int8_t *row, const uint16_t *tinv, int nrot, const double2 *costab, int sexp, int j, double *out) {
-    const int n = SFG_SLOTS;
-    __int128 sa = 0, sb = 0, sc = 0;
-    for (int m = 0; m < n; m++) {
-        int t = (int)tinv[m] - nrot; t += t < 0 ? n : 0;
-        const int v = (int)row[t];
-        if (!v) continue;
-        unsigned k = ((4u * (unsigned)m + 1u) * (unsigned)j) & 32767u;
-        if (k > 16384u) k = 32768u - k;
-        const bool neg = k > 8192u; if (neg) k = 16384u - k;
-        const double2 cv = costab[k];
-        const double x = cv.x * 0x1p20, a = __builtin_rint(x), r1 = x - a;
-        const double y = r1 * 0x1p40, bq = __builtin_rint(y), r2 = y - bq;
-        const double cq = __builtin_rint(r2 * 0x1p40 + cv.y * 0x1p100);
-        const long long sv = neg ? -(long long)v : (long long)v;
-        sa += (__int128)(sv * (long long)a); sb += (__int128)(sv * (long long)bq); sc += (__int128)(sv * (long long)cq);
-    }
-    const __int128 T = (sa << 80) + (sb << 40) + sc;
-    const int sh = 100 - sexp;
-    const __int128 q = T >> sh, rem = T - (q << sh), half = (__int128)1 << (sh - 1);
-    const __int128 dist = rem > half ? rem - half : half - rem;
-    if (dist <= ((__int128)1 << (sh - 62))) return false;
-    *out = (double)((long long)q + (rem > half ? 1 : 0));
-    return true;
+constexpr double enc_fast_c() {
+    const double add = 1.0, rot = 2.0 + 0.7072, tw = 2.2361 + 0.7072;
+    const double pass = 3 * add + rot + tw, last = 3 * add + rot;
+    const double Z = 3 * pass + last;
+    return (1.41422 * Z + 2 * (1 + tw)) * 1.02;
+}
+constexpr double ENC_FAST_C = enc_fast_c();
+constexpr int ENC_LIST = 64;
+struct EncAux { int count; int list[ENC_LIST]; long long part[2][8][3]; double red[8]; };
+static double enc_fast_rel(const sfg_ctx *ctx, int sexp) { return std::ldexp(ENC_FAST_C, sexp - 53) * ctx->cfg.enc_band_mult; }
+
+__device__ __noinline__ void enc_resolve_coop(const int8_t *row, const uint16_t *tinv, int nrot, const double2 *costab, int sexp, EncAux *aux, int nlist, double *pc,
+                                               unsigned long long *tie_count, bool audit) {
+    const int n = SFG_SLOTS, tid = threadIdx.x, lane = tid & 63, wv = tid >> 6;
+    unsigned near = 0, unproven = 0, resolved = 0;
+    for (int e = 0; e < nlist; e++) {
+        const int j = aux->list[e];
+        long long sa = 0, sb = 0, sc = 0;
+        for (int i = 0; i < 16; i++) {
+            const int m = tid + 512 * i;
+            int t = (int)tinv[m] - nrot; t += t < 0 ? n : 0;
+            const int v = (int)row[t];
+            if (!v) continue;
+            unsigned k = ((4u * (unsigned)m + 1u) * (unsigned)j) & 32767u;
+            if (k > 16384u) k = 32768u - k;
+            const bool neg = k > 8192u; if (neg) k = 16384u - k;
+            const double2 cv = costab[k];
+            const double x = cv.x * 0x1p20, a = __builtin_rint(x), r1 = x - a;
+            const double y = r1 * 0x1p40, bq = __builtin_rint(y), r2 = y - bq;
+            const double cq = __builtin_rint(r2 * 0x1p40 + cv.y * 0x1p100);
+            const long long sv = neg ? -(long long)v : (long long)v;
+            sa += sv * (long long)a; sb += sv * (long long)bq; sc += sv * (long long)cq;
+        }
+#pragma unroll
+        for (int o = 32; o > 0; o >>= 1) { sa += __shfl_xor(sa, o); sb += __shfl_xor(sb, o); sc += __shfl_xor(sc, o); }
+        long long *part = &aux->part[e & 1][0][0];
+        if (lane == 0) { part[3 * wv] = sa; part[3 * wv + 1] = sb; part[3 * wv + 2] = sc; }
+        __syncthreads();
+        if (tid == 0) {
+            __int128 ta = 0, tb = 0, tc = 0;
+            for (int w = 0; w < 8; w++) { ta += part[3 * w]; tb += part[3 * w + 1]; tc += part[3 * w + 2]; }
+            const __int128 T = (ta << 80) + (tb << 40) + tc;
+            const int sh = 100 - sexp;
+            const __int128 q = T >> sh, rem = T - (q << sh), half = (__int128)1 << (sh - 1);
+            const __int128 dist = rem > half ? rem - half : half - rem;
+            if (audit && dist < ((__int128)1 << (sh - 40))) near++;
+            if (dist <= ((__int128)1 << (sh > 62 ? sh - 62 : 0))) unproven++;
+            else { pc[j] = (double)((long long)q + (rem > half ? 1 : 0)); resolved++; }
+        }
+    }
+    if (tid == 0) {
+        if (near) atomicAdd(tie_count, (unsigned long long)near);
+        if (unproven) atomicAdd(tie_count + 1, (unsigned long long)unproven);
+        if (resolved) atomicAdd(tie_count + 2, (unsigned long long)resolved);
+    }
+}
+
+__device__ __forceinline__ double fast_round(double x, bool &inside, double band) {
+    const double nn = __builtin_rint(x), diff = x - nn;
+    inside = !(__builtin_fabs(__builtin_fabs(diff) - 0.5) > band);
+    return nn;
 }
 
 constexpr unsigned long long ENC_DOM_NONFINITE = 1, ENC_DOM_RANGE = 2;
-constexpr size_t ENC_LDS_BYTES = (size_t)2 * ENC_H * 8;
-template <bool F64IN>
-__global__ void __launch_bounds__(512, 4) k_fft_encode(const void *Dv, int shift0, const double4 *tb, const uint16_t *tinv,
-                                                      double *pc_out, unsigned long long *tie_count, const double2 *costab, int sexp, double band, double band_rel) {
+constexpr size_t ENC_IMAGE_BYTES = (size_t)2 * ENC_H * 8;
+constexpr size_t ENC_LDS_BYTES = ENC_IMAGE_BYTES + 1024;
+static_assert(sizeof(EncAux) <= 1024, "EncAux outgrew its LDS");
+template <bool F64IN, typename T>
+__device__ __forceinline__ bool enc_plaintext(const void *Dv, int shift0, const double4 *tb, const uint16_t *tinv, double *pc_out, unsigned long long *tie_count,
+                                              const double2 *costab, int sexp, double band, double band_rel, double fast_rel, double *lds) {
+    constexpr bool FAST = std::is_same<T, double>::value;
+    static_assert(!(FAST && F64IN), "the plain-fp64 path encodes genotype rows only");
+    using dd = T;
+    auto mk = [](double h) { return fx_const<T>(h, 0.0); };
     unsigned near_tie = 0;
-    extern __shared__ double lds[];
     double *RE = lds, *IM = lds + ENC_H;
+    EncAux *aux = reinterpret_cast<EncAux *>(lds + 2 * ENC_H);
     const int n = SFG_SLOTS, h = ENC_H, tid = threadIdx.x;
     const int shift = shift0 + blockIdx.x;
     const int nrot = F64IN ? 0 : SFG_D * (shift / SFG_D);
     const int8_t *row = (const int8_t *)Dv + (size_t)shift * n;
     const double *rowd = (const double *)Dv + (size_t)shift * n;
     int8_t *rowl = reinterpret_cast<int8_t *>(lds);
+    if (!FAST) __syncthreads();
     if (!F64IN) reinterpret_cast<uint4 *>(rowl)[tid] = reinterpret_cast<const uint4 *>(row)[tid];
+    if (tid == 0) aux->count = 0;
     __syncthreads();
     dd xr[8], xi[8], yr[8], yi[8];
     auto exchange = [&](dd (&sr)[8], dd (&si)[8], dd (&dr)[8], dd (&di)[8], auto widx, auto ridx, auto wave, bool entry_barrier) {
@@ -226,29 +271,42 @@
         auto sync = [&]() { if (WAVE) __builtin_amdgcn_fence(__ATOMIC_ACQ_REL, "wavefront"); else __syncthreads(); };
         if (SFG_ENC_DIAG & 4) { for (int k = 0; k < 8; k++) { dr[k] = sr[k]; di[k] = si[k]; } return; }
         if (entry_barrier) __syncthreads(); else sync();
-#pragma unroll
-        for (int k = 0; k < 8; k++) { const int p = padj(widx(k)); RE[p] = sr[k].hi; IM[p] = si[k].hi; }
-        sync();
-#pragma unroll
-        for (int k = 0; k < 8; k++) { const int p = padj(ridx(k)); dr[k].hi = RE[p]; di[k].hi = IM[p]; }
-        sync();
-#pragma unroll
-        for (int k = 0; k < 8; k++) { const int p = padj(widx(k)); RE[p] = sr[k].lo; IM[p] = si[k].lo; }
-        sync();
-#pragma unroll
-        for (int k = 0; k < 8; k++) { const int p = padj(ridx(k)); dr[k].lo = RE[p]; di[k].lo = IM[p]; }
+        if constexpr (FAST) {
+#pragma unroll
+            for (int k = 0; k < 8; k++) { const int p = padj(widx(k)); RE[p] = sr[k]; IM[p] = si[k]; }
+            sync();
+#pragma unroll
+            for (int k = 0; k < 8; k++) { const int p = padj(ridx(k)); dr[k] = RE[p]; di[k] = IM[p]; }
+        } else {
+#pragma unroll
+            for (int k = 0; k < 8; k++) { const int p = padj(widx(k)); RE[p] = sr[k].hi; IM[p] = si[k].hi; }
+            sync();
+#pragma unroll
+            for (int k = 0; k < 8; k++) { const int p = padj(ridx(k)); dr[k].hi = RE[p]; di[k].hi = IM[p]; }
+            sync();
+#pragma unroll
+            for (int k = 0; k < 8; k++) { const int p = padj(widx(k)); RE[p] = sr[k].lo; IM[p] = si[k].lo; }
+            sync();
+#pragma unroll
+            for (int k = 0; k < 8; k++) { const int p = padj(ridx(k)); dr[k].lo = RE[p]; di[k].lo = IM[p]; }
+        }
     };
     const std::false_type wg_wide; const std::true_type wave_local;
+    int sabs = 0;
 #pragma unroll
     for (int a = 0; a < 8; a++) {
         const int m = a * 512 + tid;
         int t0 = (int)tinv[2 * m] - nrot, t1 = (int)tinv[2 * m + 1] - nrot;
         t0 += t0 < 0 ? n : 0; t1 += t1 < 0 ? n : 0;
-        if (F64IN) { xr[a] = dd_make(rowd[t0], 0.0); xi[a] = dd_make(rowd[t1], 0.0); }
-        else { xr[a] = dd_make((double)rowl[t0], 0.0); xi[a] = dd_make((double)rowl[t1], 0.0); }
+        if (F64IN) { xr[a] = mk(rowd[t0]); xi[a] = mk(rowd[t1]); }
+        else {
+            const int v0 = rowl[t0], v1 = rowl[t1];
+            xr[a] = mk((double)v0); xi[a] = mk((double)v1);
+            if (FAST) sabs += (v0 < 0 ? -v0 : v0) + (v1 < 0 ? -v1 : v1);
+        }
     }
     bool out_of_domain = false;
-    if (F64IN) {
+    if constexpr (F64IN) {
         double s = 0.0;
 #pragma unroll
         for (int a = 0; a < 8; a++) s += __builtin_fabs(xr[a].hi) + __builtin_fabs(xi[a].hi);
@@ -261,6 +319,16 @@
         for (int w = 0; w < 8; w++) s += lds[w];
         if (!__builtin_isfinite(s)) { if (tid == 0) atomicOr(tie_count + 3, ENC_DOM_NONFINITE); }
         else band = __builtin_fmax(band, s * band_rel);
+    }
+    if constexpr (FAST) {
+#pragma unroll
+        for (int o = 32; o > 0; o >>= 1) sabs += __shfl_xor(sabs, o);
+        if ((tid & 63) == 0) aux->red[tid >> 6] = (double)sabs;
+        __syncthreads();
+        double s = 0.0;
+#pragma unroll
+        for (int w = 0; w < 8; w++) s += aux->red[w];
+        band = __builtin_fmax(band, fma(s, fast_rel, 0x1p-40));
     }
     dif_radix8<512, !F64IN>(xr, xi, tb + ENC_TB_P512, tid);
     {
@@ -278,47 +346,67 @@
     dd Ar[5], Ai[5], Br[5], Bi[5];
     const int npair = tid == 0 ? 5 : 4;
     __syncthreads();
-#pragma unroll
-    for (int d4 = 0; d4 < 8; d4++) { const int p = padj_fin((int)((__brev((unsigned)d4) >> 29) << 9) | cbase); RE[p] = yr[d4].hi; IM[p] = yi[d4].hi; }
-    __syncthreads();
-#pragma unroll
-    for (int i = 0; i < 5; i++) if (i < npair) {
-        const int c = tid + 512 * i, pa = padj_fin(c), pb = padj_fin((h - c) & (h - 1));
-        Ar[i].hi = RE[pa]; Ai[i].hi = IM[pa]; Br[i].hi = RE[pb]; Bi[i].hi = -IM[pb];
-    }
-    __syncthreads();
-#pragma unroll
-    for (int d4 = 0; d4 < 8; d4++) { const int p = padj_fin((int)((__brev((unsigned)d4) >> 29) << 9) | cbase); RE[p] = yr[d4].lo; IM[p] = yi[d4].lo; }
-    __syncthreads();
-#pragma unroll
-    for (int i = 0; i < 5; i++) if (i < npair) {
-        const int c = tid + 512 * i, pa = padj_fin(c), pb = padj_fin((h - c) & (h - 1));
-        Ar[i].lo = RE[pa]; Ai[i].lo = IM[pa]; Br[i].lo = RE[pb]; Bi[i].lo = -IM[pb];
-    }
-    int tie_j = -1; unsigned tie_n = 0;
-    auto note = [&](int j) { tie_j = j; tie_n++; };
+    if constexpr (FAST) {
+#pragma unroll
+        for (int d4 = 0; d4 < 8; d4++) { const int p = padj_fin((int)((__brev((unsigned)d4) >> 29) << 9) | cbase); RE[p] = yr[d4]; IM[p] = yi[d4]; }
+        __syncthreads();
+#pragma unroll
+        for (int i = 0; i < 5; i++) if (i < npair) {
+            const int c = tid + 512 * i, pa = padj_fin(c), pb = padj_fin((h - c) & (h - 1));
+            Ar[i] = RE[pa]; Ai[i] = IM[pa]; Br[i] = RE[pb]; Bi[i] = -IM[pb];
+        }
+    } else {
+#pragma unroll
+        for (int d4 = 0; d4 < 8; d4++) { const int p = padj_fin((int)((__brev((unsigned)d4) >> 29) << 9) | cbase); RE[p] = yr[d4].hi; IM[p] = yi[d4].hi; }
+        __syncthreads();
+#pragma unroll
+        for (int i = 0; i < 5; i++) if (i < npair) {
+            const int c = tid + 512 * i, pa = padj_fin(c), pb = padj_fin((h - c) & (h - 1));
+            Ar[i].hi = RE[pa]; Ai[i].hi = IM[pa]; Br[i].hi = RE[pb]; Bi[i].hi = -IM[pb];
+        }
+        __syncthreads();
+#pragma unroll
+        for (int d4 = 0; d4 < 8; d4++) { const int p = padj_fin((int)((__brev((unsigned)d4) >> 29) << 9) | cbase); RE[p] = yr[d4].lo; IM[p] = yi[d4].lo; }
+        __syncthreads();
+#pragma unroll
+        for (int i = 0; i < 5; i++) if (i < npair) {
+            const int c = tid + 512 * i, pa = padj_fin(c), pb = padj_fin((h - c) & (h - 1));
+            Ar[i].lo = RE[pa]; Ai[i].lo = IM[pa]; Br[i].lo = RE[pb]; Bi[i].lo = -IM[pb];
+        }
+    }
+    unsigned tie_n = 0;
+    auto note = [&](int j) {
+        tie_n++;
+        if (!F64IN) { const int slot = atomicAdd(&aux->count, 1); if (slot < ENC_LIST) aux->list[slot] = j; }
+    };
+    auto round_c = [&](dd w, bool &in) -> double {
+        if constexpr (FAST) return fast_round(w, in, band);
+        else return dd_round_away<F64IN>(w, near_tie, band, in);
+    };
+    auto mag = [](dd w) -> double { if constexpr (FAST) return w; else return w.hi; };
     auto recomb = [&](int c, dd Ar, dd Ai, dd Br, dd Bi) {
         constexpr bool GRID = !F64IN;
-        auto radd = [](dd a, dd b) { return GRID ? dd_make(a.hi + b.hi, a.lo + b.lo) : dd_add(a, b); };
-        auto rsub = [](dd a, dd b) { return GRID ? dd_make(a.hi - b.hi, a.lo - b.lo) : dd_sub(a, b); };
-        auto half = [](dd a) { return dd_make(a.hi * 0.5, a.lo * 0.5); };
-        if (SFG_ENC_DIAG & 2) { pc[c] = Ar.hi; if (c > 0) pc[n - c] = Ai.hi; if (c < h / 2) { pc[h - c] = Br.hi; pc[n - (h - c)] = Bi.hi; } return; }
+        auto radd = [](dd a, dd b) { if constexpr (FAST) return a + b; else return GRID ? dd_make(a.hi + b.hi, a.lo + b.lo) : dd_add(a, b); };
+        auto rsub = [](dd a, dd b) { if constexpr (FAST) return a - b; else return GRID ? dd_make(a.hi - b.hi, a.lo - b.lo) : dd_sub(a, b); };
+        auto half = [](dd a) { if constexpr (FAST) return a * 0.5; else return dd_make(a.hi * 0.5, a.lo * 0.5); };
+        auto dot_raw = [](dd a, dd w, dd b, dd x, double sgn) { if constexpr (FAST) return fx_dot2<true>(a, w, b, x, sgn); else return dd_dot2_raw(a, w, b, x, sgn); };
+        if (SFG_ENC_DIAG & 2) { pc[c] = mag(Ar); if (c > 0) pc[n - c] = mag(Ai); if (c < h / 2) { pc[h - c] = mag(Br); pc[n - (h - c)] = mag(Bi); } return; }
         const bool nt = SFG_ENC_DIAG & 16;
         const double4 wo = nt ? make_double4(0.7 + c * 1e-9, 1e-18, 0.3, 1e-18) : tb[ENC_TB_RW + c];
         const double4 zc = nt ? make_double4(0.6 + c * 1e-9, 1e-18, 0.4, 1e-18) : tb[ENC_TB_RZ + c];
         dd Xr = half(radd(Ar, Br)), Xi = half(radd(Ai, Bi));
         dd Dr = rsub(Ar, Br), Di = rsub(Ai, Bi);
         dd Or = Di, Oi = dd_neg(Dr);
-        dd wor = dd_make(wo.x, wo.y), woi = dd_make(wo.z, wo.w);
+        dd wor = fx_const<T>(wo.x, wo.y), woi = fx_const<T>(wo.z, wo.w);
         dd Yr = fx_dot2<GRID>(Or, wor, Oi, woi, -1.0), Yi = fx_dot2<GRID>(Or, woi, Oi, wor, 1.0);
         {
             dd Wr = radd(Xr, Yr), Wi = radd(Xi, Yi);
-            dd zr = dd_make(zc.x, zc.y), zi = dd_make(zc.z, zc.w);
-            dd wr = dd_dot2_raw(Wr, zr, Wi, zi, -1.0), wi = dd_dot2_raw(Wr, zi, Wi, zr, 1.0);
+            dd zr = fx_const<T>(zc.x, zc.y), zi = fx_const<T>(zc.z, zc.w);
+            dd wr = dot_raw(Wr, zr, Wi, zi, -1.0), wi = dot_raw(Wr, zi, Wi, zr, 1.0);
             bool in0, in1 = false;
-            pc[c] = dd_round_away<F64IN>(wr, near_tie, band, in0);
-            if (c > 0) pc[n - c] = -dd_round_away<F64IN>(wi, near_tie, band, in1);
-            if (F64IN) out_of_domain |= !(__builtin_fabs(wr.hi) < 0x1p53) | !(__builtin_fabs(wi.hi) < 0x1p53);
+            pc[c] = round_c(wr, in0);
+            if (c > 0) pc[n - c] = -round_c(wi, in1);
+            if (F64IN) { const double m0 = mag(wr), m1 = mag(wi); out_of_domain |= !(__builtin_fabs(m0) < 0x1p53) | !(__builtin_fabs(m1) < 0x1p53); }
             if (in0) note(c);
             if (in1) note(n - c);
         }
@@ -326,12 +414,12 @@
             const int cc = h - c;
             const double4 zh = nt ? make_double4(0.5 + c * 1e-9, 1e-18, 0.45, 1e-18) : tb[ENC_TB_RZ2 + c];
             dd Wr = rsub(Xr, Yr), Wi = dd_neg(rsub(Xi, Yi));
-            dd zr = dd_make(zh.x, zh.y), zi = dd_make(zh.z, zh.w);
-            dd wr = dd_dot2_raw(Wr, zr, Wi, zi, -1.0), wi = dd_dot2_raw(Wr, zi, Wi, zr, 1.0);
+            dd zr = fx_const<T>(zh.x, zh.y), zi = fx_const<T>(zh.z, zh.w);
+            dd wr = dot_raw(Wr, zr, Wi, zi, -1.0), wi = dot_raw(Wr, zi, Wi, zr, 1.0);
             bool in0, in1 = false;
-            pc[cc] = dd_round_away<F64IN>(wr, near_tie, band, in0);
-            if (cc < h) pc[n - cc] = -dd_round_away<F64IN>(wi, near_tie, band, in1);
-            if (F64IN) out_of_domain |= !(__builtin_fabs(wr.hi) < 0x1p53) | !(__builtin_fabs(wi.hi) < 0x1p53);
+            pc[cc] = round_c(wr, in0);
+            if (cc < h) pc[n - cc] = -round_c(wi, in1);
+            if (F64IN) { const double m0 = mag(wr), m1 = mag(wi); out_of_domain |= !(__builtin_fabs(m0) < 0x1p53) | !(__builtin_fabs(m1) < 0x1p53); }
             if (in0) note(cc);
             if (in1) note(n - cc);
         }
@@ -341,19 +429,42 @@
     if (tid == 0) recomb(h / 2, Ar[4], Ai[4], Br[4], Bi[4]);
     if (F64IN && __syncthreads_or(out_of_domain ? 1 : 0)) {
         if (tid == 0) atomicOr(tie_count + 3, ENC_DOM_RANGE);
-        return;
-    }
-    if (tie_n) {
-        unsigned unproven = tie_n - 1, resolved = 0;
-        double v;
-#ifndef SFG_ENC_NO_RESOLVE
-        if (!F64IN && sexp >= 0 && enc_tie_resolve(row, tinv, nrot, costab, sexp, tie_j, &v)) { pc[tie_j] = v; resolved = 1; } else
+        return false;
+    }
+    if (near_tie) atomicAdd(tie_count, (unsigned long long)near_tie);
+    if constexpr (F64IN) {
+        if (tie_n) atomicAdd(tie_count + 1, (unsigned long long)tie_n);
+        return false;
+    } else {
+        __syncthreads();
+        const int nflag = aux->count;
+        if (nflag == 0) return false;
+        if (FAST && nflag > ENC_LIST) { if (tid == 0) atomicAdd(tie_count + 5, 1ULL); return true; }
+        if (tie_n > 1) atomicAdd(tie_count + 4, (unsigned long long)(tie_n - 1));
+        const int nlist = nflag < ENC_LIST ? nflag : ENC_LIST;
+        bool resolve = sexp >= 0;
+#ifdef SFG_ENC_NO_RESOLVE
+        resolve = false;
 #endif
-            unproven++;
-        if (resolved) atomicAdd(tie_count + 2, 1ULL);
-        if (unproven) atomicAdd(tie_count + 1, (unsigned long long)unproven);
-    }
-    if (near_tie) atomicAdd(tie_count, (unsigned long long)near_tie);
+        if (resolve) enc_resolve_coop(row, tinv, nrot, costab, sexp, aux, nlist, pc, tie_count, FAST);
+        const int left = resolve ? nflag - nlist : nflag;
+        if (left && tid == 0) atomicAdd(tie_count + 1, (unsigned long long)left);
+        return false;
+    }
+}
+
+__device__ __noinline__ void enc_plaintext_dd_redo(const void *Dv, int shift0, const double4 *tb, const uint16_t *tinv, double *pc_out, unsigned long long *tie_count,
+                                                    const double2 *costab, int sexp, double band, double *lds) {
+    enc_plaintext<false, dd>(Dv, shift0, tb, tinv, pc_out, tie_count, costab, sexp, band, 0.0, 0.0, lds);
+}
+template <bool F64IN, bool FAST>
+__global__ void __launch_bounds__(512, 4) k_fft_encode(const void *Dv, int shift0, const double4 *tb, const uint16_t *tinv,
+                                                      double *pc_out, unsigned long long *tie_count, const double2 *costab, int sexp, double band, double band_rel, double fast_rel) {
+    extern __shared__ double lds[];
+    if constexpr (FAST) {
+        if (enc_plaintext<false, double>(Dv, shift0, tb, tinv, pc_out, tie_count, costab, sexp, band, band_rel, fast_rel, lds))
+            enc_plaintext_dd_redo(Dv, shift0, tb, tinv, pc_out, tie_count, costab, sexp, band, lds);
+    } else enc_plaintext<F64IN, dd>(Dv, shift0, tb, tinv, pc_out, tie_count, costab, sexp, band, band_rel, fast_rel, lds);
 }
 
 static double enc_band_rel(const sfg_ctx *ctx) { return std::ldexp(ctx->sh->scale / (double)SFG_SLOTS, -88); }
@@ -369,8 +480,9 @@
     return sfg_scratch(ctx, "enc.pc", nplain * SFG_SLOTS * sizeof(double), (void **)pc);
 }
 int encode_set_attrs(sfg_ctx *ctx) {
-    SFG_HIP(ctx, hipFuncSetAttribute((const void *)k_fft_encode<false>, hipFuncAttributeMaxDynamicSharedMemorySize, (int)ENC_LDS_BYTES));
-    SFG_HIP(ctx, hipFuncSetAttribute((const void *)k_fft_encode<true>, hipFuncAttributeMaxDynamicSharedMemorySize, (int)ENC_LDS_BYTES));
+    SFG_HIP(ctx, hipFuncSetAttribute((const void *)k_fft_encode<false, true>, hipFuncAttributeMaxDynamicSharedMemorySize, (int)ENC_LDS_BYTES));
+    SFG_HIP(ctx, hipFuncSetAttribute((const void *)k_fft_encode<false, false>, hipFuncAttributeMaxDynamicSharedMemorySize, (int)ENC_LDS_BYTES));
+    SFG_HIP(ctx, hipFuncSetAttribute((const void *)k_fft_encode<true, false>, hipFuncAttributeMaxDynamicSharedMemorySize, (int)ENC_LDS_BYTES));
     return 0;
 }
 
@@ -394,7 +506,8 @@
         if (cmode == 1) pc = pcache->slot + (size_t)(shift0 + s0) * SFG_SLOTS;
         if (cmode <= 1) {
             PhaseTimer t(ctx, "encode", false);
-            hipLaunchKernelGGL(k_fft_encode<false>, dim3(nb), dim3(512), lds_bytes, ctx->stream, (const void *)D, shift0 + s0, et->tb, et->tinv, pc, (unsigned long long *)ctx->tie_count_dev, et->costab, et->sexp, ctx->cfg.tie_band, 0.0);
+            auto kern = (et->sexp < 0 || ctx->cfg.enc_dd) ? k_fft_encode<false, false> : k_fft_encode<false, true>;
+            hipLaunchKernelGGL(kern, dim3(nb), dim3(512), lds_bytes, ctx->stream, (const void *)D, shift0 + s0, et->tb, et->tinv, pc, (unsigned long long *)ctx->tie_count_dev, et->costab, et->sexp, ctx->cfg.tie_band, 0.0, enc_fast_rel(ctx, et->sexp));
             SFG_HIP(ctx, hipGetLastError());
         }
         if (cmode == 2) pc = pcache->slot + (size_t)(shift0 + s0) * SFG_SLOTS;
@@ -453,7 +566,7 @@
     if (hipMemcpyAsync(dv, values_host, (size_t)nvec * n * 8, hipMemcpyHostToDevice, ctx->stream) != hipSuccess) rc = 1;
     if (!rc && hipMemsetAsync((unsigned long long *)ctx->tie_count_dev + 3, 0, 8, ctx->stream) != hipSuccess) rc = 1;
     if (!rc) {
-        hipLaunchKernelGGL(k_fft_encode<true>, dim3(nvec), dim3(512), lds_bytes, ctx->stream, (const void *)dv, 0, et->tb, et->tinv, dpc, (unsigned long long *)ctx->tie_count_dev, et->costab, -1, ctx->cfg.tie_band, enc_band_rel(ctx));
+        hipLaunchKernelGGL((k_fft_encode<true, false>), dim3(nvec), dim3(512), lds_bytes, ctx->stream, (const void *)dv, 0, et->tb, et->tinv, dpc, (unsigned long long *)ctx->tie_count_dev, et->costab, -1, ctx->cfg.tie_band, enc_band_rel(ctx), 0.0);
         if (hipGetLastError() != hipSuccess) rc = 1;
     }
     if (!rc && hipMemcpyAsync(pc.data(), dpc, (size_t)nvec * n * 8, hipMemcpyDeviceToHost, ctx->stream) != hipSuccess) rc = 1;
@@ -480,7 +593,7 @@
     double *dv = (double *)p; double *dpc = dv + (size_t)nvec * n;
     SFG_HIP(ctx, hipMemcpyAsync(dv, values_host, (size_t)nvec * n * 8, hipMemcpyHostToDevice, ctx->stream));
     SFG_HIP(ctx, hipMemsetAsync((unsigned long long *)ctx->tie_count_dev + 3, 0, 8, ctx->stream));
-    hipLaunchKernelGGL(k_fft_encode<true>, dim3(nvec), dim3(512), lds_bytes, ctx->stream, (const void *)dv, 0, et->tb, et->tinv, dpc, (unsigned long long *)ctx->tie_count_dev, et->costab, -1, ctx->cfg.tie_band, enc_band_rel(ctx));
+    hipLaunchKernelGGL((k_fft_encode<true, false>), dim3(nvec), dim3(512), lds_bytes, ctx->stream, (const void *)dv, 0, et->tb, et->tinv, dpc, (unsigned long long *)ctx->tie_count_dev, et->costab, -1, ctx->cfg.tie_band, enc_band_rel(ctx), 0.0);
     SFG_HIP(ctx, hipGetLastError());
     SFG_TRY(launch_ntt_plain(ctx, dpc, (u64 *)pt_dev, (size_t)nvec, level + 1));
     SFG_HIP(ctx, hipStreamSynchronize(ctx->stream));
@@ -495,7 +608,7 @@
     *count = c[0];
     if (reset) {
         if (c[1]) sfg_ptc_invalidate_all(ctx);
-        SFG_HIP(ctx, hipMemset(ctx->tie_count_dev, 0, 32));
+        SFG_HIP(ctx, hipMemset(ctx->tie_count_dev, 0, 48));
     }
     return 0;
 }
@@ -520,6 +633,15 @@
     SFG_HIP(ctx, hipMemcpy(count, (unsigned long long *)ctx->tie_count_dev + 1, 8, hipMemcpyDeviceToHost));
     return 0;
 }
+extern "C" int sfg_ctx_encoder_fast_stats_for_test(sfg_ctx *ctx, unsigned long long *same_lane, unsigned long long *redone) {
+    if (!ctx->test_hooks) SFG_FAIL(ctx, "sfg_ctx_encoder_fast_stats_for_test: test hook, enabled only in a process that set the test switch before creating the context");
+    SFG_HIP(ctx, hipSetDevice(ctx->device));
+    SFG_TRY(sfg_sync_all(ctx));
+    unsigned long long c[2] = {0, 0};
+    SFG_HIP(ctx, hipMemcpy(c, (unsigned long long *)ctx->tie_count_dev + 4, 16, hipMemcpyDeviceToHost));
+    *same_lane = c[0]; *redone = c[1];
+    return 0;
+}
 extern "C" int sfg_ctx_encoder_inject_unsafe_for_test(sfg_ctx *ctx, unsigned long long n) {
     if (!ctx->test_hooks) SFG_FAIL(ctx, "sfg_ctx_encoder_inject_unsafe_for_test: test hook, enabled only in a process that set the test switch before creating the context");
     SFG_HIP(ctx, hipSetDevice(ctx->device));
```

After: 6007 billion. 0.965x the previous value.
